# go-distributed/gossip_simulator

Hardware: AMD Instinct MI355X
Metric: gossip messages delivered/sec (node) at N=1e9; rounds-to-coverage parity (higher is better)
Workload: dtype u32

## Files before the change

gossip_simulator_amd/csrc/gs_ctx.cpp:

```cpp
#include "gs_ctx.h"

namespace gs {

namespace {

uint32_t ring_slots(const gs_params& p) { return p.delay_high > 2 ? (uint32_t)p.delay_high : 2u; }

uint32_t ceil_log2(uint64_t x) {
  uint32_t b = 0;
  while ((1ull << b) < x) ++b;
  return b;
}

int check_params(const gs_params* p, bool rumor_trials, bool median_trials, std::string& why) {
  if (!p) { why = "params is NULL"; return GS_EINVAL; }
  if (p->n == 0) { why = "n must be >= 1 (simulator.go:240 panics on rand.Intn(0))"; return GS_EINVAL; }
  if (p->n > 0x7FFFFFFFull) { why = "n must be < 2^31"; return GS_EINVAL; }
  if (p->delay_high <= p->delay_low) {
    why = "delayhigh must exceed delaylow (simulator.go:167 panics on rand.Intn(<=0))";
    return GS_EINVAL;
  }
  if (p->fanout < 0 || p->fanin < 0 || p->fanout > 255 || p->fanin > 255) {
    why = "fanout/fanin must be in [0, 255]";
    return GS_EINVAL;
  }
  if (ring_slots(*p) > 4096) { why = "delayhigh must be <= 4096"; return GS_EINVAL; }
  if (p->model > GS_MODEL_MEDIAN) {
    why = "model must be GS_MODEL_FLOOD, GS_MODEL_PUSHPULL, GS_MODEL_RUMOR or GS_MODEL_MEDIAN";
    return GS_EINVAL;
  }
  if (p->model == GS_MODEL_MEDIAN && (p->rumor_k < 1 || p->rumor_k > 127)) {
    why = "GS_MODEL_MEDIAN needs 1 <= rumor_k <= 127, not " + std::to_string(p->rumor_k);
    return GS_EINVAL;
  }
  if (p->model == GS_MODEL_MEDIAN && p->trials > 1 && !median_trials) {
    why = "GS_MODEL_MEDIAN with trials > 1: the median-counter model runs one trial per context";
    return GS_EINVAL;
  }
  if (p->model == GS_MODEL_RUMOR && (p->rumor_k < 1 || p->rumor_k > 255)) {
    why = "GS_MODEL_RUMOR needs 1 <= rumor_k <= 255, not " + std::to_string(p->rumor_k);
    return GS_EINVAL;
  }
  if (p->model == GS_MODEL_RUMOR && (p->rumor_mode & ~(GS_RUMOR_BLIND | GS_RUMOR_COIN | GS_RUMOR_PULL))) {
    why = "GS_MODEL_RUMOR: rumor_mode " + std::to_string(p->rumor_mode) +
          " has a bit that is none of GS_RUMOR_BLIND, GS_RUMOR_COIN, GS_RUMOR_PULL";
    return GS_EINVAL;
  }
  if (p->model == GS_MODEL_RUMOR && p->trials > 1 && !rumor_trials) {
    why = "GS_MODEL_RUMOR with trials > 1: the rumor model runs one trial per context (gs_create_trials makes a batch)";
    return GS_EINVAL;
  }
  if (p->trials > 1 && ((uint64_t)p->trials << std::max<uint32_t>(kFineLog, ceil_log2(p->n))) > 0x7FFFFFFFull) {
    why = "trials x 2^ceil(log2 n) must be < 2^31 (batch fewer trials per context)";
    return GS_EINVAL;
  }
  return GS_OK;
}

bool alloc_trial_rows(gs_ctx* c, size_t tb, size_t cb) {
  return dev_malloc((void**)&c->bt.d_tstat, tb) == hipSuccess &&
         hipHostMalloc((void**)&c->bt.h_tstat, tb) == hipSuccess && grow(c->bt.chk, cb);
}

void release_trials(gs_ctx* c) {
  if (c->bt.d_tstat) (void)dev_free(c->bt.d_tstat);
  if (c->bt.h_tstat) (void)hipHostFree(c->bt.h_tstat);
  release(c->bt.chk);
}

int alloc_window(gs_ctx* c) {
  const DevState& s = c->st;
  WinState& w = c->ws;
  w.n = s.n;
  w.W = s.W;
  w.nfine = (uint32_t)((s.n + kFineNodes - 1) >> kFineLog);
  w.ncoarse = (w.nfine + 255) / 256;
  w.R = s.R;
  w.delay_low = s.delay_low;
  w.delay_span = s.delay_span;
  w.kd = s.kd;
  w.kc = s.kc;
  w.key = s.key;
  w.base = (uint32_t)c->lo;
  w.tlog = c->tlog;
  w.tmask = c->tlog >= 32 ? ~0u : (1u << c->tlog) - 1;
  w.tnodes = c->trials > 1 && c->tlog <= kCoarseShift && !c->shard ? (uint32_t)c->p.n : 0u;
  w.G = c->G;
  w.rank = c->rank;
  w.seg_per = (uint32_t)c->seg_per;
  w.csub = kCoarseSub;
  w.noxcd = getenv("GS_PART2_NOXCD") ? 1u : 0u;
  {
    const char* xp = getenv("GS_XPAIR");
    w.nopair = xp && atoi(xp) == 0 ? 1u : 0u;
  }
  w.ccap_end = nullptr;
  w.csrc = nullptr;
  if (c->shard) {
    w.owner = 1;
    w.obins = 256 / c->G;
    w.oseg_q = (uint32_t)(c->seg_per >> kFineLog);
    w.oseg_magic = 0xFFFFFFFFu / w.oseg_q;
    if (dev_malloc(&c->wn.d_rtab, kRtabWords * 8) != hipSuccess ||
        hipHostMalloc((void**)&c->wn.h_rtab, kRtabWords * 8) != hipSuccess)
      return fail(c, GS_ENOMEM, "cannot allocate the shard's receive layout");
  }
  auto al = [](size_t b) { return (b + 255) & ~(size_t)255; };
  const size_t units = (size_t)kMaxWindow * w.nfine + 1;
  const size_t b_fc = al((size_t)w.R * w.nfine * 4), b_units = al(units * 8),
               b_small = al(kRegions * 8) * 2 + al((kRegions + 1) * 8) + al((kRegions + 1) * 4) + al(kMaxWindow * 8),
               b_fhist = al(((size_t)w.ncoarse * 256 + 1) * 8), b_fbase = al(((size_t)w.nfine + 1) * 8),
               b_ffill = al((size_t)w.nfine * 8),
               b_sst = al((size_t)kStatShards * kMaxWindow * kStatFields * 8),
               b_rlcnt = al((size_t)w.nfine * 4) + al(((size_t)w.nfine + 2) * 4),
               b_tsum = al((size_t)w.ncoarse * kMaxWindow * 8) + al(((size_t)w.ncoarse + 1) * 8);
  const size_t total = b_fc + 2 * b_units + b_small + b_fhist + b_fbase + b_ffill + b_sst + b_rlcnt + b_tsum;
  if (dev_malloc(&c->wn.d_win, total) != hipSuccess)
    return fail(c, GS_ENOMEM, "cannot allocate window-engine buffers");
  const size_t flist = (size_t)w.R * w.nfine * kFineNodes * 2;
  if (dev_malloc(&c->wn.d_flist, flist) != hipSuccess)
    return fail(c, GS_ENOMEM, "cannot allocate " + std::to_string(flist >> 20) + " MiB of fire lists");
  char* q = (char*)c->wn.d_win;
  w.fcount = (uint32_t*)q; q += b_fc;
  w.usize = (unsigned long long*)q; q += b_units;
  w.unit_off = (unsigned long long*)q; q += b_units;
  w.chist = (unsigned long long*)q; q += al(kRegions * 8);
  w.cfill = (unsigned long long*)q; q += al(kRegions * 8);
  w.ccap = (unsigned long long*)q; q += al((kRegions + 1) * 8);
  w.tprefix = (uint32_t*)q; q += al((kRegions + 1) * 4);
  w.tfires = (unsigned long long*)q;
  q = (char*)c->wn.d_win + b_fc + 2 * b_units + b_small;
  w.fhist = (unsigned long long*)q; q += b_fhist;
  w.fstart = (unsigned long long*)q; q += b_fbase;
  w.ffill = (unsigned long long*)q; q += b_ffill;
  w.sstats = (unsigned long long*)q; q += b_sst;
  w.rlcnt = (uint32_t*)q; q += al((size_t)w.nfine * 4);
  w.lgl = (uint32_t*)q; q += al(((size_t)w.nfine + 2) * 4);
  w.tsum = (unsigned long long*)q; q += al((size_t)w.ncoarse * kMaxWindow * 8);
  w.toff = (unsigned long long*)q; q += al(((size_t)w.ncoarse + 1) * 8);
  if (dev_malloc(&c->wn.d_rlmsg, (size_t)w.nfine * kRolledCap * 4) != hipSuccess)
    return fail(c, GS_ENOMEM, "cannot allocate the rolled-receipt lists");
  w.rlmsg = (uint32_t*)c->wn.d_rlmsg;
  w.dbg = nullptr;
  if (getenv("GS_STAMPS") && dev_malloc(&w.dbg, kDbgWords * 8) == hipSuccess)
    (void)hipMemset(w.dbg, 0, kDbgWords * 8);
  w.flist = (uint16_t*)c->wn.d_flist;
  c->wn.fcount_bytes = (size_t)w.R * w.nfine * 4;
  if (hipMemsetAsync(c->wn.d_win, 0, total, c->stream) != hipSuccess)
    return fail(c, GS_EDEVICE, "memset of window buffers failed");
  c->wn.misc_words = std::max<size_t>(4096, (size_t)c->G * kMaxWindow + 64);
  if (hipHostMalloc((void**)&c->wn.h_cap, (kRegions + 1) * 8) != hipSuccess ||
      hipHostMalloc((void**)&c->wn.h_misc, c->wn.misc_words * 8) != hipSuccess ||
      hipHostMalloc((void**)&c->wn.h_err, 64) != hipSuccess)
    return fail(c, GS_ENOMEM, "cannot allocate pinned window buffers");
  if (c->trials > 1) {
    if (!alloc_trial_rows(c, (size_t)c->trials * kMaxWindow * kTStatFields * 4, 0))
      return fail(c, GS_ENOMEM, "cannot allocate per-trial counters");
    w.tstat = c->bt.d_tstat;
  }
  return GS_OK;
}

void release_window(gs_ctx* c) {
  WinEngine& e = c->wn;
  for (void* p : {e.d_win, e.d_flist, e.d_rlmsg, (void*)e.d_rtab, (void*)c->ws.dbg})
    if (p) (void)dev_free(p);
  for (Buf* b : {&e.gmap, &e.cmsg, &e.fmsg, &e.tmp}) release(*b);
  for (void* p : {(void*)e.h_cap, (void*)e.h_misc, (void*)e.h_err, (void*)e.h_rtab})
    if (p) (void)hipHostFree(p);
}

int ctx_setup(gs_ctx* c, const gs_params* params, int device, bool shard, uint32_t G, uint32_t rank,
              std::string& why) {
  c->p = *params;
  c->p.device = device;
  c->dev = device;
  int ndev = 0;
  if (hipGetDeviceCount(&ndev) != hipSuccess || ndev <= 0) {
    why = "no HIP device visible (libgossip_hip needs an MI355X)";
    return GS_EDEVICE;
  }
  if (c->dev < 0 || c->dev >= ndev) {
    why = "device " + std::to_string(c->dev) + " out of range (" + std::to_string(ndev) + " visible)";
    return GS_EDEVICE;
  }
  hipDeviceProp_t prop;
  if (hipSetDevice(c->dev) != hipSuccess || hipGetDeviceProperties(&prop, c->dev) != hipSuccess ||
      strncmp(prop.gcnArchName, "gfx950", 6) != 0) {
    why = "device " + std::to_string(c->dev) + " is not gfx950";
    return GS_EDEVICE;
  }
  if (hipStreamCreateWithFlags(&c->own, hipStreamNonBlocking) != hipSuccess) {
    why = "cannot create a stream";
    return GS_EDEVICE;
  }
  c->stream = c->own;
  DevState& s = c->st;
  const uint32_t stride0 = (uint32_t)std::max(c->p.fanout, c->p.fanin);
  c->pp = c->p.model == GS_MODEL_PUSHPULL && !c->rset;
  c->rumor = c->p.model == GS_MODEL_RUMOR;
  c->median = c->p.model == GS_MODEL_MEDIAN;
  c->pp_l2_only = (c->p.flags & GS_FLAG_PP_L2_ONLY) != 0;
  c->trials = std::max<uint32_t>(1, c->p.trials);
  c->ntot = c->p.n;
  if (c->trials > 1) {
    c->tlog = std::max<uint32_t>(kFineLog, ceil_log2(c->p.n));
    c->ntot = (uint64_t)c->trials << c->tlog;
  }
  c->shard = shard;
  c->G = G;
  c->rank = rank;
  if (shard && c->rumor) {
    why = "GS_MODEL_RUMOR runs on one device: no node-range shards";
    return GS_EINVAL;
  }
  if (shard && c->median) {
    why = "GS_MODEL_MEDIAN runs on one device: no node-range shards";
    return GS_EINVAL;
  }
  if (shard) {
    if (c->pp && !pp_rslot_packed(stride0)) {
      why = "push-pull node-range shards need rows of at most 16 slots (bottom-up rounds)";
      return GS_EINVAL;
    }
    c->seg_per = (((c->p.n + G - 1) / G) + kFineNodes - 1) & ~(uint64_t)(kFineNodes - 1);
    if ((uint64_t)(G - 1) * c->seg_per >= c->p.n) {
      why = "n = " + std::to_string(c->p.n) + " is too small for " + std::to_string(G) +
            " shards of whole 16384-node buckets";
      return GS_EINVAL;
    }
    c->pp_shard = c->pp;
    c->rs.segw = c->seg_per / 64;
    c->lo = rank * c->seg_per;
    c->hi = std::min<uint64_t>(c->lo + c->seg_per, c->p.n);
    c->ntot = c->hi - c->lo;
  }
  s.lo = 0;
  s.hi = (uint32_t)c->ntot;
  s.n = c->ntot;
  s.W = (s.n + 63) / 64;
  s.C = (uint32_t)((s.n + (1ull << kChunkNodesLog) - 1) >> kChunkNodesLog);
  s.CS = (s.C + kShards - 1) / kShards;
  s.chunk_lo = 0;
  s.chunk_hi = s.C;
  s.sharded = 0;
  s.R = ring_slots(c->p);
  s.delay_low = c->p.delay_low;
  s.delay_span = (uint32_t)(c->p.delay_high - c->p.delay_low);
  s.kd = gs_threshold(c->p.drop_rate);
  s.kc = gs_threshold(c->p.crash_rate);
  s.key = Key{(uint32_t)c->p.seed, (uint32_t)(c->p.seed >> 32), c->p.trial};
  c->win = !c->pp && !c->rumor && !c->median && !c->rset && s.R <= kWinMaxRing && !(c->p.flags & GS_FLAG_TICK_ENGINE) && stride0 <= kWinMaxStride &&
           s.n <= (1ull << (kCoarseShift + 8));
  if (((c->trials > 1 && !c->ppt && !c->rmt && !c->mdt) || (shard && !c->pp)) && !c->win) {
    why = "batched trials and node-range shards run on the window engine (delayhigh <= 256, "
          "fanout/fanin <= 32, no GS_FLAG_TICK_ENGINE, at most 2^30 nodes per context or shard)";
    return GS_EINVAL;
  }
  static_assert(kSrcShift + 8 == 64, "8-bit source index in the receive layout");
  if (shard && !c->pp && (G > 255 || ((c->seg_per + (1ull << kCoarseShift) - 1) >> kCoarseShift) > 256 / G)) {
    why = "flood node-range shards: each of the G <= 255 shards' ranges must fit 256 / G bins of 2^22 nodes "
          "(n up to about 2^30)";
    return GS_EINVAL;
  }
  auto al = [](size_t b) { return (b + 255) & ~(size_t)255; };
  const bool tick = !c->win && !c->pp && !c->rumor && !c->median && !c->rset;
  const size_t b_sum = c->pp && !c->ppt ? al(pp_summary_total_words(s.W) * 8) : 0;
  const size_t b_next = (c->pp && !c->ppt) || (c->rumor && !c->rmt) ? al(s.W * 8) + b_sum : 0;
  const size_t b_bits = al(s.W * 8), b_ring = tick ? al((size_t)s.R * s.W * 8) : 0,
               b_cflag = tick ? al((size_t)s.R * s.C * 4) : 0,
               b_clist = tick ? al((size_t)s.R * kShards * s.CS * 4) : 0,
               b_ccount = tick ? al((size_t)s.R * kShards * kCounterStride * 4) : 0,
               b_stats = al((size_t)kStatSlots * kStatFields * 8);
  const size_t b_roll = c->win ? b_bits : 0;
  const size_t total = 2 * b_bits + b_roll + b_next + b_ring + b_cflag + b_clist + b_ccount + b_stats + 256;
  c->state_bytes = total;
  if (dev_malloc(&c->d_state, total) != hipSuccess) {
    why = "cannot allocate " + std::to_string(total) + " bytes of device state";
    return GS_ENOMEM;
  }
  char* q = (char*)c->d_state;
  s.recv = (unsigned long long*)q; q += b_bits;
  s.crash = (unsigned long long*)q; q += b_bits;
  s.rollw = b_roll ? (uint32_t*)q : nullptr; q += b_roll;
  c->d_next = b_next ? (unsigned long long*)q : nullptr;
  c->d_ppsum = b_sum ? (unsigned long long*)(q + al(s.W * 8)) : nullptr;
  q += b_next;
  s.ring = (unsigned long long*)q; q += b_ring;
  s.cflag = (uint32_t*)q; q += b_cflag;
  s.clist = (uint32_t*)q; q += b_clist;
  s.ccount = (uint32_t*)q; q += b_ccount;
  s.stats = (unsigned long long*)q; q += b_stats;
  c->d_err = (uint32_t*)q;
  c->d_flag = c->d_err + 1;
  s.err = c->d_err;
  s.grecv = s.recv;
  s.gcrash = s.crash;
  s.gbase = 0;
  if (tick && s.kc > 0 && dev_malloc(&c->d_cnt, s.n * 4) != hipSuccess) {
    why = "cannot allocate arrival counters";
// ... 430 lines not shown
```

gossip_simulator_amd/csrc/gs_internal.h:

```cpp
#pragma once
#include <stdint.h>
#include <hip/hip_runtime.h>

#include <algorithm>
#include <vector>

#include "gs_devmem.h"
#include "gs_rng.h"

namespace gs {

inline uint32_t grid_for(uint64_t items, uint32_t per_block, uint32_t cap) {
  return (uint32_t)std::min<uint64_t>((items + per_block - 1) / per_block, cap);
}

constexpr uint32_t kWave = 64;
constexpr uint32_t kChunkNodesLog = 12;
constexpr uint32_t kChunkWords = 64;
constexpr uint32_t kShards = 32;
constexpr uint32_t kCounterStride = 16;
constexpr uint32_t kStatFields = 8;
constexpr uint32_t kStatSlots = 4096;
constexpr uint32_t kListCap = 1024;
constexpr uint32_t kTickBlock = 256;
constexpr uint32_t kTickGridMax = 2048;

enum Stat : uint32_t {
  ST_FIRED = 0, ST_SENT = 1, ST_MSGS = 2, ST_RECV = 3, ST_CRASH = 4, ST_SCHED = 5,
  ST_ERR = 6, ST_RSVD = 7
};

enum Mode : int {
  MODE_FLOOD = 0,
  MODE_COUNT = 1,
  MODE_RESOLVE = 2
};

struct DevState {
  const uint8_t* deg;
  const uint32_t* ids;
  unsigned long long* recv;
  unsigned long long* crash;
  uint32_t* rollw;
  uint32_t* cnt;
  unsigned long long* ring;
  uint32_t* cflag;
  uint32_t* clist;
  uint32_t* ccount;
  unsigned long long* stats;
  uint32_t* err;
  unsigned long long* grecv;
  unsigned long long* gcrash;
  uint64_t gbase;
  uint64_t n, W;
  uint32_t C, CS, R, stride;
  uint32_t stride_magic;
  int32_t delay_low;
  uint32_t delay_span;
  int32_t kd, kc;
  int32_t check_crashed;
  int32_t sharded;
  uint32_t lo, hi;
  uint32_t chunk_lo, chunk_hi;
  Key key;
};

constexpr uint32_t kFineLog = 14;
constexpr uint32_t kFineNodes = 1u << kFineLog;
constexpr uint32_t kCoarseShift = kFineLog + 8;
constexpr uint32_t kMaxWindow = 16;
constexpr uint32_t kCoarseSub = 8;
constexpr uint32_t kRegions = 256 * kCoarseSub;
constexpr uint32_t kWinMaxRing = 256;
constexpr uint32_t kWinMaxStride = 32;
constexpr uint32_t kEmptyMsg = 0xFFFFFFFFu;
constexpr uint32_t kSrcShift = 56;
constexpr unsigned long long kSrcMask = (1ull << kSrcShift) - 1;
#ifndef GS_PART_TILE
#define GS_PART_TILE 16384
#endif
constexpr uint32_t kPartTile = GS_PART_TILE;
constexpr uint32_t kRolledCap = 1024;
constexpr uint32_t kBitTicks = 10;
constexpr uint32_t kXRoundNodes = 2048;
constexpr uint32_t kWinSlotsPerBucket = 1u << 16;

struct WinCtl {
  uint32_t t, L, tnext, tend;
  uint32_t poll, pbase, stop, lmax;
  unsigned long long Tn, T;
  unsigned long long recv, crashed, pending, cover, max_ticks;
  unsigned long long cmsg_cap, fmsg_cap;
  unsigned long long xs_cap, xr_cap;
};
constexpr uint32_t kStageWords = 8 + 16 * 8;

struct WinState {
  const uint8_t* deg;
  const uint32_t* ids;
  unsigned long long* recv;
  unsigned long long* crash;
  uint32_t* rollw;
  uint32_t* rlmsg;
  uint32_t* rlcnt;
  uint32_t* lgl;
  unsigned long long* stats;
  uint32_t* err;
  uint32_t* fcount;
  uint16_t* flist;
  unsigned long long* usize;
  unsigned long long* unit_off;
  unsigned long long* tfires;
  uint32_t* gmap;
  const uint32_t* pk;
  uint32_t noxcd;
  uint32_t nopair;
  uint32_t* cmsg;
  uint32_t* fmsg;
  unsigned long long* chist;
  unsigned long long* ccap;
  const unsigned long long* ccap_end;
  unsigned long long* cfill;
  uint32_t* tprefix;
  unsigned long long* fhist;
  unsigned long long* fstart;
  unsigned long long* ffill;
  unsigned long long* tsum;
  unsigned long long* toff;
  unsigned long long* sstats;
  unsigned long long* dbg;
  uint32_t* tstat;
  uint32_t tofs;
  WinCtl* ctl;
  unsigned long long* stage;
  uint32_t lstride;
  uint32_t slots;
  uint32_t csub;
  const uint32_t* const* csrc;
  uint32_t owner;
  uint32_t obins;
  uint32_t oseg_q, oseg_magic;
  uint32_t abort_on_err;
  uint32_t G, rank;
  uint32_t seg_per;
  uint32_t dd;
  uint32_t guard;
  uint32_t solo;
  unsigned long long* gcnt;
  unsigned long long* glay;
  unsigned long long* wstat;
  uint64_t nglob;
  uint64_t n, W;
  uint32_t nfine, ncoarse, R, stride, stride_magic;
  int32_t delay_low;
  uint32_t delay_span;
  int32_t kd, kc;
  uint32_t base;
  uint32_t tlog, tmask;
  uint32_t tnodes;
  Key key;
};
constexpr uint32_t kStatShards = 32;
constexpr uint32_t kStampPhases = 10;
constexpr uint32_t kXStamp0 = 2 * kStampPhases;
constexpr uint32_t kDbgWords = kXStamp0 + 8;
enum TStat : uint32_t { TS_FIRED = 0, TS_SENT = 1, TS_DEAD = 2, TS_RECV = 3, TS_CRASH = 4, TS_HOT = 5, TS_MSGS = 6 };
constexpr uint32_t kTStatFields = 8;

__host__ __device__ __forceinline__ void node_key(uint32_t tlog, uint32_t tmask, const Key& key,
                                                  uint64_t g, uint32_t kind, uint32_t& node,
                                                  uint32_t& c3) {
  node = (uint32_t)(g & tmask);
  c3 = ctr3(kind, key.trial + (uint32_t)(g >> tlog));
}

constexpr uint32_t kErrArrivals = 4;
constexpr uint32_t kErrCoarse = 8;
constexpr uint32_t kErrFine = 16;
constexpr uint32_t kErrAbort = 32;
constexpr uint32_t kErrNoMem = 64;
constexpr uint32_t kDDRow = kRegions + 4;
constexpr uint32_t kDDWStat = kMaxWindow * kStatFields + 8;
constexpr size_t kRtabWords = 4 * (kRegions + 1) + 260;
constexpr size_t kRtabTotal = kRtabWords - 1;

hipError_t win_units(const WinState& w, uint32_t t0, uint32_t L, hipStream_t s);
hipError_t win_cut(const WinState& w, unsigned long long budget, hipStream_t s);
hipError_t win_unitscan(const WinState& w, hipStream_t s);
hipError_t win_close(const WinState& w, uint32_t slot, hipStream_t s);
hipError_t win_scan_units(const WinState& w, uint32_t L, void* tmp, size_t& tmp_bytes, hipStream_t s);
hipError_t win_groupmap(const WinState& w, uint32_t L, hipStream_t s);
hipError_t win_expand(const WinState& w, uint32_t t0, uint32_t L, uint64_t Tn, int mode,
                      hipStream_t s);
uint32_t win_expand_geometry(const WinState& w, uint64_t Tn, uint32_t* per_round, uint32_t* bsz,
                             uint32_t* npt);
hipError_t win_plan(const WinState& w, bool exact, hipStream_t s);
hipError_t win_scan_fine(const WinState& w, void* tmp, size_t& tmp_bytes, hipStream_t s);
hipError_t win_part2(const WinState& w, uint64_t T, bool scatter, hipStream_t s);
hipError_t win_resolve(const WinState& w, uint32_t t0, uint32_t L, hipStream_t s);
hipError_t win_pack_rows(const uint32_t* ids, uint64_t n, uint32_t* pk, hipStream_t s);
hipError_t win_seal_rows(const uint8_t* deg, uint32_t* ids, uint64_t n, uint32_t stride,
                         hipStream_t s);
hipError_t win_stats_reduce(const WinState& w, uint32_t t0, uint32_t L, hipStream_t s);
hipError_t win_consume_sh(const WinState& w, uint32_t t0, uint32_t L, hipStream_t s);
hipError_t win_rtab(const WinState& w, unsigned long long* rtab, const unsigned long long* const* ccaps,
                    const uint32_t* const* src, uint32_t nsrc, uint32_t travels, hipStream_t s);
hipError_t win_fine_redo(const WinState& w, uint64_t T, hipStream_t s);
hipError_t win_stats_dd(const WinState& w, uint32_t slot, hipStream_t s);
struct WinGroup {
  const WinState* ws;
  const WinState* wr;
  const WinState* wg;
  uint32_t M;
  uint32_t nfine_max;
  uint32_t ncoarse_max;
  uint32_t slots_max;
};
hipError_t win_units_g(const WinGroup& g, uint32_t L, hipStream_t s);
hipError_t win_cut_g(const WinGroup& g, unsigned long long budget, hipStream_t s);
hipError_t win_unitscan_g(const WinGroup& g, hipStream_t s);
hipError_t win_rtab_g(const WinGroup& g, const unsigned long long* const* ccaps, const uint32_t* const* src,
                      uint32_t nsrc, hipStream_t s);
hipError_t win_recv_g(const WinGroup& g, uint64_t T, hipStream_t s);
hipError_t win_stats_dd_g(const WinGroup& g, uint32_t slot, hipStream_t s);
hipError_t win_expand_g(const WinGroup& g, uint32_t L, hipStream_t s);
hipError_t win_resolve_g(const WinGroup& g, uint32_t L, hipStream_t s);
hipError_t win_close_dd(const WinState& w, const unsigned long long* const* wstats, WinCtl* const* ctls,
                        uint32_t n, uint32_t slot, hipStream_t s);
hipError_t win_pack(const WinState& w, const unsigned long long* poff, uint32_t nreg, uint32_t* out, hipStream_t s);
hipError_t win_schedule(const WinState& w, uint32_t node, uint32_t tick, uint32_t trials, uint32_t n,
                        hipStream_t s, uint32_t* started = nullptr);

inline uint64_t pp_summary_words(uint64_t W) { return (W + 63) / 64; }
inline uint64_t pp_summary2_words(uint64_t W) { return (pp_summary_words(W) + 63) / 64; }
inline uint64_t pp_summary_total_words(uint64_t W) { return 2 * pp_summary_words(W) + 2 * pp_summary2_words(W); }
enum PPMode : uint32_t { PP_DENSE = 0, PP_EARLY = 1, PP_BOTTOM = 2, PP_ANSWER = 3 };
__host__ __device__ inline bool pp_rslot_packed(uint32_t stride) { return stride <= 16; }
constexpr uint32_t kPPSegs = 256;
struct PPCtl {
  unsigned long long ninf;
  unsigned long long thr;
  unsigned long long bthr;
  unsigned long long athr;
  unsigned long long ncallers;
  unsigned long long nlive0;
  unsigned long long seg_cap;
  uint32_t nseg;
  uint32_t mode;
  uint32_t early_ok;
  uint32_t ovf;
  uint32_t nearly, nbottom;
  uint32_t nanswer, pad_;
  unsigned long long segcnt[kPPSegs];
  unsigned long long seglen[kPPSegs];
  unsigned long long segpre[kPPSegs + 1];
};
struct PPSparse {
  PPCtl* ctl;
  uint32_t* ilist;
  const unsigned long long* rend;
  const uint16_t* rend16;
  const unsigned long long* rbase;
  const uint32_t* rsrc;
  const uint8_t* rslot;
  const uint8_t* fmask;
  const unsigned long long* fany;
  const uint32_t* rfail;
  uint32_t* dset;
  unsigned long long* dcnt;
  uint64_t dcap, ccap, fcap;
  uint32_t nodeg;
  uint32_t pullfirst;
  uint32_t word_maxi;
  uint32_t word_maxu;
  uint32_t words;
};
constexpr uint32_t kPPDLists = 512;
constexpr uint32_t kPPDRegions = 2048;
hipError_t pp_round(const DevState& s, unsigned long long* next, unsigned long long* sum, uint32_t t,
                    bool l2_only, const PPSparse& sp, hipStream_t st);
hipError_t pp_live_edges(const DevState& s, uint32_t* out, hipStream_t st);
hipError_t pp_commit(const DevState& s, const unsigned long long* next, uint32_t t, const PPSparse& sp,
                     hipStream_t st);
hipError_t pp_seed(const DevState& s, unsigned long long* next, uint32_t node, uint32_t* flag,
                   const PPSparse& sp, unsigned long long thr, unsigned long long bthr, unsigned long long athr,
                   const unsigned long long* callers, hipStream_t st);
size_t pp_rev_scan_bytes(uint64_t n);
hipError_t pp_rev_build(const DevState& s, unsigned long long* rend, uint32_t* rsrc, uint8_t* rslot, void* tmp,
                        size_t tmp_bytes, hipStream_t st);
hipError_t pp_rev_compact(const unsigned long long* rend, uint64_t n, uint16_t* rend16, unsigned long long* rbase,
                          uint32_t* ovf, hipStream_t st);
hipError_t pp_rev_build_part(const DevState& s, unsigned long long* rend, uint32_t* rsrc, uint8_t* rslot,
                             hipStream_t st, uint32_t* passes_out);
hipError_t pp_fmask_build(const DevState& s, const unsigned long long* rend, const uint32_t* rsrc,
                          const uint8_t* rslot, uint8_t* fmask, hipStream_t st);
size_t pp_rev_range_scan_bytes(uint64_t n);
hipError_t pp_rev_count_range(const uint8_t* deg, const uint32_t* ids, uint64_t nfull, uint32_t stride, uint64_t lo,
                              uint64_t hi, unsigned long long* rend, void* tmp, size_t tmp_bytes, hipStream_t st);
hipError_t pp_rev_fill_range(const uint8_t* deg, const uint32_t* ids, uint64_t nfull, uint32_t stride, uint64_t lo,
                             uint64_t hi, unsigned long long* rend, uint32_t* rsrc, uint8_t* rslot, hipStream_t st);
hipError_t pp_fmask_rows(const DevState& s, uint8_t* fmask, hipStream_t st);
hipError_t pp_fmask_any(const uint8_t* fmask, uint64_t n, unsigned long long* fany, hipStream_t st);
hipError_t pp_rfail_build(const DevState& s, const unsigned long long* rend, const uint32_t* rsrc,
                          const uint8_t* rslot, uint32_t* rfail, hipStream_t st);
hipError_t pp_round_shard(const DevState& s, unsigned long long* next, unsigned long long* gnext, uint32_t t,
                          const PPSparse& sp, uint32_t mode, hipStream_t st);
hipError_t pp_count(const unsigned long long* words, uint64_t nwords, unsigned long long* out, hipStream_t st);
hipError_t pp_or_slices(unsigned long long* dst, const unsigned long long* src, uint32_t nslices, uint64_t words,
                        hipStream_t st);

struct PptState {
  const uint8_t* deg;
  const uint32_t* ids;
  unsigned long long* recv;
  const unsigned long long* crash;
  uint32_t* tstat;
  uint32_t n, trials, tlog, stride;
  uint32_t block, lds_bytes;
  uint32_t lds_masked;
  int32_t kd;
  Key key;
};
hipError_t ppt_lds_limit(int device, bool masked, uint64_t* limit, const char** where = nullptr);
hipError_t ppt_prepare(int device, bool masked, uint32_t lds_bytes);
hipError_t ppt_seed(const PptState& s, uint32_t node, uint32_t* started, hipStream_t st);
hipError_t ppt_rounds(const PptState& s, uint32_t t0, uint32_t rounds, hipStream_t st);
hipError_t ppt_stalled(const PptState& s, const uint8_t* need, uint32_t* live, hipStream_t st);

enum RumorAcc : uint32_t { RA_FIRED = 0, RA_SENT = 1, RA_MSGS = 2, RA_NEW = 3 };
constexpr uint32_t kRumorCovered = 1, kRumorQuiescent = 2;
constexpr uint32_t kRumorBlind = 1, kRumorCoin = 2, kRumorPull = 4;
struct RumorCtl {
  unsigned long long wlen;
  unsigned long long pad0_[31];
  unsigned long long acc[4];
  unsigned long long pad1_[28];
  unsigned long long rlen;
  unsigned long long received;
  unsigned long long cover;
  unsigned long long peak;
  uint32_t stop, pad2_;
  unsigned long long pad3_[27];
};
static_assert(sizeof(RumorCtl) == 3 * 256, "RumorCtl: three 256-byte blocks");
struct RumorState {
  RumorCtl* ctl;
  unsigned long long* next;
  uint8_t* miss;
  uint32_t k;
  uint32_t mode;
  unsigned long long* hot;
  unsigned long long* served;
  unsigned long long* vain;
};
uint32_t rumor_grid(uint64_t n, uint32_t want);
hipError_t rumor_seed(const DevState& s, const RumorState& r, uint32_t* list0, uint32_t node, unsigned long long cover,
                      hipStream_t st);
hipError_t rumor_round(const DevState& s, const RumorState& r, const uint32_t* rlist, uint32_t* wlist, uint32_t t,
                       uint32_t grid, hipStream_t st);
hipError_t rumor_commit(const DevState& s, const RumorState& r, uint32_t t, hipStream_t st);
hipError_t rumor_removed(const RumorState& r, const uint32_t* rlist, unsigned long long* out, uint32_t grid,
                         hipStream_t st);
hipError_t rumor_pull_seed(const DevState& s, const RumorState& r, uint32_t node, unsigned long long cover,
                           hipStream_t st);
hipError_t rumor_pull_round(const DevState& s, const RumorState& r, uint32_t t, uint32_t grid, hipStream_t st);
hipError_t rumor_pull_commit(const DevState& s, const RumorState& r, uint32_t t, hipStream_t st);
hipError_t rumor_pull_removed(const DevState& s, const RumorState& r, unsigned long long* out, hipStream_t st);

struct RmtState {
// ... 69 lines not shown
```

gossip_simulator_amd/csrc/gs_shards.cpp:

```cpp
#include "gs_ctx.h"

namespace gs {

namespace {

int sync_all(const std::vector<gs_ctx*>& ms) {
  for (gs_ctx* m : ms) {
    CK(m, hipSetDevice(m->dev));
    CK(m, hipStreamSynchronize(m->stream));
  }
  return GS_OK;
}

int mark_nomem(gs_ctx* m, const std::string& what) {
  uint32_t e = 0;
  CK(m, hipMemcpyAsync(&e, m->d_err, 4, hipMemcpyDeviceToHost, m->stream));
  CK(m, hipStreamSynchronize(m->stream));
  e |= kErrNoMem;
  CK(m, hipMemcpyAsync(m->d_err, &e, 4, hipMemcpyHostToDevice, m->stream));
  CK(m, hipStreamSynchronize(m->stream));
  m->err = what;
  return GS_OK;
}

// ... 575 lines not shown
  CK(c, hipMemcpyAsync(dbuf, c->xc.h_xbuf, count * 8, hipMemcpyHostToDevice, c->stream));
  CK(c, hipStreamSynchronize(c->stream));
  return GS_OK;
}

int rank_sum(gs_ctx* c, unsigned long long* v) {
  unsigned long long* d = c->xc.d_gcounts;
  CK(c, hipMemcpyAsync(d, v, 8, hipMemcpyHostToDevice, c->stream));
  if (int rc = x_all_reduce(c, d, 1)) return abort_rank(c, rc);
  CK(c, hipMemcpyAsync(v, d, 8, hipMemcpyDeviceToHost, c->stream));
  CK(c, hipStreamSynchronize(c->stream));
  return GS_OK;
}

int abort_rank(gs_ctx* c, int rc) {
  if (rc && is_rank(c)) c->aborted = true;
  if (rc && c->xc.comm && rccl().ok && rccl().comm_abort) {
    (void)rccl().comm_abort(c->xc.comm);
    c->xc.comm = nullptr;
  }
  return rc;
}

bool dd_ok(const gs_ctx* acc, const std::vector<gs_ctx*>& ms) {
  if ((acc->p.flags & GS_FLAG_TIMING) || getenv("GS_SYNC_WINDOWS") || shard_serial()) return false;
  const gs_ctx* m0 = ms[0];
  if (m0->pp || !m0->win || !m0->shard) return false;
  if (acc->group) return !acc->gtrials && acc->gr.devs.size() == 1;
  return is_rank(acc);
}

int dd_run(gs_ctx* acc, const std::vector<gs_ctx*>& ms, uint64_t tend, uint32_t poll, uint64_t max_ticks,
           const OnTick& on_tick, uint32_t* stop, bool* fallback) {
  *stop = 0;
  *fallback = false;
  RC(dd_setup(acc, ms));
  gs_ctx* m0 = ms[0];
  const uint32_t G = m0->G, M = (uint32_t)ms.size();
  const bool rank = is_rank(m0), travel = rank && G > 1;
  const bool solo = !rank && G == 1 && M == 1;
  const size_t K1 = kRegions + 1;
  hipStream_t st = m0->stream;
  CK(acc, hipSetDevice(m0->dev));
  for (gs_ctx* m : ms)
    if (m != m0) CK(acc, hipStreamSynchronize(m->stream));
  const uint32_t Lmax = std::min<uint32_t>(std::max<int32_t>(m0->p.delay_low, 1), kBitTicks);
  const uint64_t N = m0->p.n;
  const unsigned long long budget = ((N + kFineNodes - 1) >> kFineLog) * (unsigned long long)kWinSlotsPerBucket;
  const uint32_t B8 = m0->ws.obins * kCoarseSub, nreg = G * B8;
  bool ok = true;
  for (gs_ctx* m : ms)
    ok = ok && grow(m->wn.gmap, ((m->ntot + 1 + 63) / 64 + 1) * 4) && grow(m->wn.cmsg, 64) && grow(m->wn.fmsg, 64);
  if (rank) RC(agree_ok(m0, ok, "cannot allocate the window message buffers"));
  else if (!ok) return fail(acc, GS_ENOMEM, "cannot allocate the window message buffers");
  void** hp = acc->dd.h_ptrs;
  const uint32_t nsrc = rank ? 2u : M + 1;
  void** d_ccaps = acc->dd.ptrs;
  void** d_src = acc->dd.ptrs + M;
  void** d_wst = acc->dd.ptrs + 2 * M + 1;
  void** d_ctls = acc->dd.ptrs + 3 * M + 1;
  for (uint32_t i = 0; i < M; ++i) {
    hp[i] = ms[i]->ws.ccap;
    hp[2 * M + 1 + i] = acc->dd.wstat + (size_t)i * kDDWStat;
    hp[3 * M + 1 + i] = acc->dd.ctl + i;
  }
  if (rank) {
    hp[M] = m0->xc.xrecv.p;
    hp[M + 1] = m0->wn.cmsg.p;
  } else {
    for (uint32_t i = 0; i < M; ++i) hp[M + i] = ms[i]->wn.cmsg.p;
    hp[2 * M] = nullptr;
  }
  CK(acc, hipMemcpyAsync(acc->dd.ptrs, hp, (size_t)(4 * M + 2) * sizeof(void*), hipMemcpyHostToDevice, st));
  std::vector<WinCtl> hc(M);
  for (uint32_t i = 0; i < M; ++i) {
    WinCtl& h = hc[i];
    h = WinCtl{};
    h.tnext = (uint32_t)(acc->t + 1);
    h.tend = (uint32_t)std::min<uint64_t>(tend, 0xFFFFFFFFull);
    h.poll = poll;
    h.pbase = (uint32_t)acc->t;
    h.lmax = Lmax;
    h.recv = acc->recv;
    h.crashed = acc->crashed;
    h.pending = acc->pending;
    h.cover = cover_threshold(N);
    h.max_ticks = max_ticks;
    h.cmsg_cap = buf_cap(ms[i]->wn.cmsg);
    h.fmsg_cap = buf_cap(ms[i]->wn.fmsg);
    h.xs_cap = buf_cap(ms[i]->xc.xsend);
    h.xr_cap = buf_cap(ms[i]->xc.xrecv);
  }
  CK(acc, hipMemcpyAsync(acc->dd.ctl, hc.data(), (size_t)M * sizeof(WinCtl), hipMemcpyHostToDevice, st));
  CK(acc, hipMemsetAsync(acc->dd.gcnt, 0, (size_t)G * kMaxWindow * 8, st));
  std::vector<WinState> ws(M), wr(M);
  std::vector<uint64_t> tn_bound(M);
  for (uint32_t i = 0; i < M; ++i) {
    gs_ctx* m = ms[i];
    WinState w = m->ws;
    w.ctl = acc->dd.ctl + i;
    w.stage = acc->aw.d_stage;
    w.lstride = Lmax;
    w.dd = 1;
    w.guard = 0;
    w.abort_on_err = 0;
    w.gcnt = acc->dd.gcnt;
    w.glay = acc->dd.glay;
    w.tfires = acc->dd.gcnt + (size_t)m->rank * kMaxWindow;
    w.cfill = acc->dd.glay + (size_t)m->rank * kDDRow;
    w.wstat = acc->dd.wstat + (size_t)i * kDDWStat;
    w.nglob = N;
    w.solo = solo ? 1u : 0u;
    w.gmap = (uint32_t*)m->wn.gmap.p;
    w.cmsg = (uint32_t*)m->wn.cmsg.p;
    w.fmsg = (uint32_t*)m->wn.fmsg.p;
    ws[i] = w;
    if (solo) {
      wr[i] = w;
      tn_bound[i] = std::min<uint64_t>(m->ntot + 1, 4096ull * 1024);
      continue;
    }
    WinState r = w;
    r.cmsg = nullptr;
    r.csrc = (const uint32_t* const*)(m->wn.d_rtab + 4 * K1);
    r.ccap = m->wn.d_rtab;
    r.ccap_end = m->wn.d_rtab + K1;
    r.cfill = m->wn.d_rtab + 2 * K1;
    r.csub = G * kCoarseSub;
    wr[i] = r;
    tn_bound[i] = std::min<uint64_t>(m->ntot + 1, 4096ull * 1024);
  }
  const uint64_t T_bound = 2048ull * 16384;
  static const bool group_env = [] { const char* e = getenv("GS_DD_GROUP"); return !(e && atoi(e) == 0); }();
  const bool grouped = !rank && M > 1 && group_env;
  std::vector<WinState> wall;
  WinGroup grp{};
  if (grouped) {
    wall.reserve(3 * M);
    wall.insert(wall.end(), ws.begin(), ws.end());
    wall.insert(wall.end(), wr.begin(), wr.end());
    for (uint32_t i = 0; i < M; ++i) {
      wall.push_back(wr[i]);
      wall.back().guard = 1;
    }
    CK(acc, hipMemcpyAsync(acc->dd.wsm, wall.data(), wall.size() * sizeof(WinState), hipMemcpyHostToDevice, st));
    grp.ws = acc->dd.wsm;
    grp.wr = acc->dd.wsm + M;
    grp.wg = acc->dd.wsm + 2 * M;
    grp.M = M;
    for (uint32_t i = 0; i < M; ++i) {
      grp.nfine_max = std::max(grp.nfine_max, ws[i].nfine);
      grp.ncoarse_max = std::max(grp.ncoarse_max, ws[i].ncoarse);
      grp.slots_max = std::max(grp.slots_max, ws[i].slots);
    }
  }
  auto bsize = [&](uint32_t s, uint32_t d) {
    unsigned long long a = 0;
    for (uint32_t r = d * B8; r < (d + 1) * B8; ++r) a += acc->dd.h_lay[(size_t)s * kDDRow + r];
    return a;
  };
  auto enqueue = [&](uint32_t slot, bool* aborted) -> int {
    *aborted = false;
    if (grouped) {
      CK(acc, win_units_g(grp, Lmax, st));
      CK(acc, win_cut_g(grp, budget, st));
      CK(acc, win_unitscan_g(grp, st));
    } else {
      for (uint32_t i = 0; i < M; ++i) CK(acc, win_units(ws[i], 0, Lmax, st));
      if (rank) RC(x_all_gather(m0, acc->dd.gcnt, kMaxWindow * 8));
      for (uint32_t i = 0; i < M; ++i) CK(acc, win_cut(ws[i], budget, st));
      for (uint32_t i = 0; i < M; ++i) CK(acc, win_unitscan(ws[i], st));
    }
    if (grouped) CK(acc, win_expand_g(grp, Lmax, st));
    for (uint32_t i = 0; i < M && !grouped; ++i) CK(acc, win_expand(ws[i], 0, Lmax, tn_bound[i], 1, st));
    if (rank) RC(x_all_gather(m0, acc->dd.glay, kDDRow * 8));
    if (grouped)
      CK(acc, win_rtab_g(grp, (const unsigned long long* const*)d_ccaps, (const uint32_t* const*)d_src, nsrc, st));
    for (uint32_t i = 0; i < M && !solo && !grouped; ++i)
      CK(acc, win_rtab(ws[i], ms[i]->wn.d_rtab, (const unsigned long long* const*)d_ccaps, (const uint32_t* const*)d_src,
                       nsrc, rank ? 1u : 0u, st));
    if (travel) {
      gs_ctx* m = m0;
      const uint32_t me = m->rank;
      CK(acc, hipMemcpyAsync(acc->dd.h_lay, acc->dd.glay, (size_t)G * kDDRow * 8, hipMemcpyDeviceToHost, st));
      CK(acc, hipMemcpyAsync(m->wn.h_err, m->d_err, 4, hipMemcpyDeviceToHost, st));
      CK(acc, hipMemcpyAsync(m->wn.h_misc, acc->dd.ctl, 32, hipMemcpyDeviceToHost, st));
      CK(acc, hipStreamSynchronize(st));
      const uint32_t* hc0 = (const uint32_t*)m->wn.h_misc;
      if (*m->wn.h_err & kErrAbort) { *aborted = true; return 1; }
      if (hc0[1] == 0 || hc0[6]) return 1;
      std::vector<unsigned long long> ptot(G, 0), rsum(G, 0);
      for (uint32_t s = 0; s < G; ++s)
        for (uint32_t d = 0; d < G; ++d)
          if (s != d) {
            const unsigned long long b = bsize(s, d);
            ptot[s] += b;
            rsum[d] += b;
          }
      bool any_grow = false;
      for (uint32_t s = 0; s < G; ++s) {
        const unsigned long long* row = acc->dd.h_lay + (size_t)s * kDDRow;
        if (ptot[s] > row[kRegions + 2] || rsum[s] > row[kRegions + 3]) any_grow = true;
      }
      if (any_grow) {
        const void* old_recv = m->xc.xrecv.p;
        const bool ok = grow(m->xc.xsend, (ptot[me] + 16) * 4) && grow(m->xc.xrecv, (rsum[me] + 16) * 4);
        unsigned long long* d = m->xc.d_gcounts + (size_t)G * kMaxWindow;
        m->wn.h_misc[8] = ok ? 0ull : 1ull;
        CK(acc, hipMemcpyAsync(d, &m->wn.h_misc[8], 8, hipMemcpyHostToDevice, st));
        RC(x_all_reduce(m, d, 1));
        CK(acc, hipMemcpyAsync(&m->wn.h_misc[9], d, 8, hipMemcpyDeviceToHost, st));
        CK(acc, hipStreamSynchronize(st));
        if (m->wn.h_misc[9]) return fail(acc, GS_ENOMEM, "a rank cannot allocate its exchange buffers");
        WinCtl* c = acc->dd.ctl;
        m->wn.h_misc[10] = buf_cap(m->xc.xsend);
        m->wn.h_misc[11] = buf_cap(m->xc.xrecv);
        CK(acc, hipMemcpyAsync(&c->xs_cap, &m->wn.h_misc[10], 16, hipMemcpyHostToDevice, st));
        if (m->xc.xrecv.p != old_recv) {
          m->wn.h_misc[12] = (unsigned long long)(uintptr_t)m->xc.xrecv.p;
          CK(acc, hipMemcpyAsync(m->wn.d_rtab + 4 * K1, &m->wn.h_misc[12], 8, hipMemcpyHostToDevice, st));
          hp[M] = m->xc.xrecv.p;
          CK(acc, hipMemcpyAsync(&d_src[0], &hp[M], sizeof(void*), hipMemcpyHostToDevice, st));
        }
        CK(acc, hipStreamSynchronize(st));
      }
      CK(acc, win_pack(ws[0], m->wn.d_rtab + 3 * K1, nreg, (uint32_t*)m->xc.xsend.p, st));
      auto bstart = [&](uint32_t s, uint32_t d) {
        unsigned long long a = 0;
        for (uint32_t d2 = 0; d2 < d; ++d2)
          if (d2 != s) a += bsize(s, d2);
        return a;
      };
      std::vector<unsigned long long> in(G, 0);
      unsigned long long rs = 0;
      for (uint32_t s = 0; s < G; ++s)
        if (s != me) { in[s] = rs; rs += bsize(s, me); }
      uint32_t* xs = (uint32_t*)m->xc.xsend.p;
      uint32_t* xr = (uint32_t*)m->xc.xrecv.p;
      if (m->xc.comm) {
        const Rccl& r = rccl();
        NCK(acc, r.group_start());
        for (uint32_t p = 0; p < G; ++p) {
          if (p == me) continue;
          if (bsize(me, p)) NCK(acc, r.send(xs + bstart(me, p), bsize(me, p), ncclUint32, (int)p, m->xc.comm, st));
          if (bsize(p, me)) NCK(acc, r.recv(xr + in[p], bsize(p, me), ncclUint32, (int)p, m->xc.comm, st));
        }
        NCK(acc, r.group_end());
      } else {
        std::vector<size_t> sb(G, 0), rb(G, 0);
        for (uint32_t p = 0; p < G; ++p)
          if (p != me) { sb[p] = bsize(me, p) * 4; rb[p] = bsize(p, me) * 4; }
        RC(agree_ok(m, grow_pinned(m, (ptot[me] + rs) * 4 + 16), "cannot allocate exchange staging"));
        char* hs = m->xc.h_xbuf;
        char* hr = m->xc.h_xbuf + ptot[me] * 4;
        CK(acc, hipMemcpyAsync(hs, xs, ptot[me] * 4, hipMemcpyDeviceToHost, st));
        CK(acc, hipStreamSynchronize(st));
        if (m->xc.hx.all_to_allv(m->xc.hx.user, hs, sb.data(), hr, rb.data()))
          return fail(acc, GS_EDEVICE, "the exchange's all_to_allv callback failed");
        CK(acc, hipMemcpyAsync(xr, hr, rs * 4, hipMemcpyHostToDevice, st));
        CK(acc, hipStreamSynchronize(st));
      }
    }
    if (grouped) {
      CK(acc, win_recv_g(grp, T_bound, st));
      CK(acc, win_resolve_g(grp, Lmax, st));
      CK(acc, win_stats_dd_g(grp, slot, st));
    } else {
      for (uint32_t i = 0; i < M; ++i) {
        CK(acc, win_plan(wr[i], false, st));
        CK(acc, win_part2(wr[i], T_bound, true, st));
        if (!solo) CK(acc, win_fine_redo(wr[i], T_bound, st));
        CK(acc, win_resolve(wr[i], 0, Lmax, st));
        CK(acc, win_stats_dd(ws[i], slot, st));
      }
    }
    if (rank) RC(x_all_reduce(m0, acc->dd.wstat, kDDWStat));
    if (!solo)
      CK(acc, win_close_dd(ws[0], (const unsigned long long* const*)d_wst, (WinCtl* const*)d_ctls, M, slot, st));
    CK(acc, hipEventRecord(acc->aw.wev[slot], st));
    return 0;
  };
  bool eoverflow = false;
  auto absorb = [&](uint32_t slot, int* what) -> int {
    CK(acc, hipEventSynchronize(acc->aw.wev[slot]));
    const unsigned long long* sg = acc->aw.h_stage + (size_t)slot * kStageWords;
    const uint32_t t0 = (uint32_t)sg[0], L = (uint32_t)sg[1];
    *what = 0;
    if (sg[3] & kErrAbort) {
      if (dd_log()) fprintf(stderr, "[dd] window at t0=%u aborted: redone host-driven\n", t0);
      ++m0->timing.dd_fallbacks;
      *fallback = true;
      *what = 1;
      return GS_OK;
    }
    if (dd_log()) fprintf(stderr, "[dd] t0=%u L=%u stop=%llu redos=%llu\n", t0, L, sg[2], sg[4]);
    m0->timing.exact_redos += sg[4];
    for (uint32_t k = 0; k < L; ++k) on_tick((uint64_t)t0 + k, sg + 8 + (size_t)k * kStatFields);
    if (sg[3] & kErrArrivals) eoverflow = true;
    if (sg[2]) *stop = (uint32_t)sg[2];
    if (sg[2] || L == 0 || (uint64_t)t0 + L >= tend || eoverflow) *what = 1;
    return GS_OK;
  };
  bool ab = false;
  int e0 = 0;
  RC((e0 = enqueue(0, &ab), e0 < 0 ? e0 : 0));
  if (e0 == 1) {
// ... 79 lines not shown
```

gossip_simulator_amd/csrc/gs_win_dev.h:

```cpp
#pragma once
#include <cstdlib>

#include "gossip.h"
#include "gs_internal.h"
#include "gs_wave.h"

namespace gs {
namespace {

constexpr uint32_t kExpandBlock = 256;
constexpr uint32_t kExpandBlock6 = 512;
constexpr uint32_t kExpandNpt = 4;
constexpr uint32_t kResolveBlock = 512;
#ifndef GS_RESOLVE_WAVES
#define GS_RESOLVE_WAVES 4
#endif
constexpr uint32_t kRoll0Coarse = kCoarseShift + 4;
constexpr uint32_t kRoll0Fine = kFineLog + 4;

inline uint32_t device_cus() {
  static const uint32_t cus = [] {
    int dev = 0, v = 0;
    if (hipGetDevice(&dev) == hipSuccess &&
        hipDeviceGetAttribute(&v, hipDeviceAttributeMultiprocessorCount, dev) == hipSuccess && v > 0)
      return (uint32_t)v;
    return 256u;
  }();
  return cus;
}

__device__ __forceinline__ uint32_t stop_bits(const WinState& w) {
  return w.dd && !w.solo ? kErrAbort : (kErrCoarse | kErrFine | kErrAbort);
}
__device__ __forceinline__ bool win_abort(const WinState& w) {
  return (*w.err & stop_bits(w)) != 0;
}
struct CtlView {
  uint32_t t, L, tnext, tend, poll, pbase, stop, lmax, err;
};
__device__ __forceinline__ CtlView ctl_view(const WinState& w) {
  static_assert(offsetof(WinCtl, t) == 0 && offsetof(WinCtl, lmax) == 28, "WinCtl's first 32 bytes");
  const uint4* p = reinterpret_cast<const uint4*>(w.ctl);
  const uint4 a = p[0], b = p[1];
  const uint32_t e = *w.err;
  return CtlView{a.x, a.y, a.z, a.w, b.x, b.y, b.z, b.w, e};
}
__device__ __forceinline__ uint32_t win_open(const WinState& w, uint32_t& t) {
  const CtlView c = ctl_view(w);
  t = c.tnext;
  const bool dead = (c.err & stop_bits(w)) || c.stop || t >= c.tend;
  uint32_t Lw = min(c.lmax, c.tend - t);
  if (c.poll) {
    const uint32_t P = c.pbase + c.poll * ((t - c.pbase + c.poll - 1) / c.poll);
    Lw = min(Lw, P - t + 1);
  }
  return dead ? 0u : Lw;
}
__device__ __forceinline__ uint32_t win_live(const WinState& w, uint32_t& t0, uint32_t L) {
  if (!w.ctl) return w.abort_on_err && win_abort(w) ? 0u : L;
  const CtlView c = ctl_view(w);
  t0 = c.t;
  const bool off = (c.err & stop_bits(w)) || (w.guard && !(c.err & kErrFine));
  return off ? 0u : c.L;
}

__device__ __forceinline__ unsigned long long* shard_row(const WinState& w, uint32_t k) {
  return w.sstats + ((size_t)(blockIdx.x & (kStatShards - 1)) * kMaxWindow + k) * kStatFields;
}

constexpr uint32_t kCloseLanes = 8;
__device__ __forceinline__ unsigned long long stat_shard_sum(const WinState& w, uint32_t i, uint32_t part) {
  constexpr uint32_t kPer = kStatShards / kCloseLanes;
  unsigned long long x[kPer], sum = 0;
#pragma unroll
  for (uint32_t j = 0; j < kPer; ++j) x[j] = w.sstats[(size_t)(j * kCloseLanes + part) * kMaxWindow * kStatFields + i];
#pragma unroll
  for (uint32_t j = 0; j < kPer; ++j) {
    sum += x[j];
    if (x[j]) w.sstats[(size_t)(j * kCloseLanes + part) * kMaxWindow * kStatFields + i] = 0;
  }
#pragma unroll
  for (uint32_t o = 1; o < kCloseLanes; o <<= 1) sum += __shfl_xor(sum, o, 64);
  return sum;
}

__device__ __forceinline__ void block_scan256(uint32_t* cnt, uint32_t* off) {
  if (threadIdx.x < 64) {
    const uint32_t l = threadIdx.x;
    const uint32_t a = cnt[4 * l], b = cnt[4 * l + 1], c = cnt[4 * l + 2], d = cnt[4 * l + 3];
    const uint32_t sum = a + b + c + d;
    const uint32_t x = wave_inscan(sum);
    const uint32_t ex = x - sum;
    off[4 * l] = ex;
    off[4 * l + 1] = ex + a;
    off[4 * l + 2] = ex + a + b;
    off[4 * l + 3] = ex + a + b + c;
    if (l == 63) off[256] = x;
  }
}

__device__ __forceinline__ unsigned long long region_end(const WinState& w, uint32_t r) {
  return w.ccap_end ? w.ccap_end[r] : w.ccap[r + 1];
}
__device__ __forceinline__ unsigned long long region_fill(const WinState& w, uint32_t r) {
  const unsigned long long room = region_end(w, r) - w.ccap[r];
  return w.cfill[r] < room ? w.cfill[r] : room;
}

__device__ __forceinline__ bool tiles_by_xcd(const WinState& w) {
  return w.csub == kCoarseSub && !w.csrc && !w.noxcd;
}
__device__ __forceinline__ uint32_t xcd_bin_pos(uint32_t c) { return (c & 7) * 32 + (c >> 3); }
__device__ __forceinline__ uint32_t xcd_bin_of(uint32_t pc) { return (pc & 31) * 8 + (pc >> 5); }

__device__ __forceinline__ uint32_t msg_loc(uint32_t m) { return m & (kFineNodes - 1); }
__device__ __forceinline__ uint32_t msg_tick(uint32_t m) { return (m >> kFineLog) & (kMaxWindow - 1); }

}
}
```

gossip_simulator_amd/csrc/gs_win_expand.hip:

```cpp
#include <algorithm>

#include "gs_win_dev.h"

namespace gs {
namespace {

__device__ __forceinline__ uint32_t unit_of_wave(const WinState& w, unsigned long long g0, unsigned long long g,
                                                 unsigned long long Tn, uint32_t units) {
  const unsigned long long q = g0 >> 6;
  uint32_t lo = w.gmap[q];
  uint32_t hi = ((q + 1) << 6) < Tn ? w.gmap[q + 1] : units - 1;
  if (lo == hi) return lo;
  while (lo < hi) {
    const uint32_t mid = (lo + hi + 1) >> 1;
    if (w.unit_off[mid] <= g) lo = mid; else hi = mid - 1;
  }
  return lo;
}

#ifdef GS_XSTAMPS
__device__ __forceinline__ void xstamp(const WinState& w, unsigned long long& last, uint32_t i) {
  if (w.dbg && threadIdx.x < 64) {
    __builtin_amdgcn_s_waitcnt(0);
    const unsigned long long t = __builtin_amdgcn_s_memtime();
// ... 18 lines not shown
  uint32_t ovf;
  unsigned long long acc[kMaxWindow][2];
};

__device__ __forceinline__ void tstat_add(uint32_t* tstat, uint32_t key, uint32_t fa, uint32_t a,
                                          uint32_t fb, uint32_t b) {
  bool pend = key != ~0u;
  for (unsigned long long bal = __ballot(pend); bal; bal = __ballot(pend)) {
    const uint32_t lead = (uint32_t)__builtin_ctzll(bal);
    const uint32_t k0 = __shfl(key, lead, 64);
    const bool mine = pend && key == k0;
    const uint32_t sa = wave_sum(mine ? a : 0u), sb = wave_sum(mine ? b : 0u);
    if ((threadIdx.x & 63) == lead) {
      if (sa) atomicAdd(&tstat[(size_t)k0 * kTStatFields + fa], sa);
      if (sb) atomicAdd(&tstat[(size_t)k0 * kTStatFields + fb], sb);
    }
    pend = pend && !mine;
  }
}

__device__ __forceinline__ uint64_t pk_byte(uint32_t v) {
  const uint32_t line = (uint32_t)(((uint64_t)v * 0xCCCCCCCDull) >> 34);
  return (uint64_t)line * 128 + (v - line * 5) * 24;
}

__device__ __forceinline__ uint32_t dpp_swap_pair(uint32_t v) {
  return (uint32_t)__builtin_amdgcn_mov_dpp((int)v, 0xB1, 0xF, 0xF, false);
}
template <uint32_t MAXS>
__device__ __forceinline__ void decode_pk_row(uint4 x, uint4 y, bool o8, uint32_t (&mm)[MAXS]) {
  mm[0] = o8 ? x.z : x.x;
  mm[1] = o8 ? x.w : x.y;
  mm[2] = o8 ? y.x : x.z;
  mm[3] = o8 ? y.y : x.w;
  mm[4 % MAXS] = o8 ? y.z : y.x;
  if (MAXS > 5) mm[5 % MAXS] = o8 ? y.w : y.y;
}
template <uint32_t MAXS, uint32_t NPT>
__device__ __forceinline__ void load_rows_pk_pairs(const WinState& w, const uint32_t (&vv)[NPT], const bool (&wlive)[NPT],
                                                   uint32_t (&mm)[NPT][MAXS]) {
  const uint32_t odd = threadIdx.x & 1;
  const uint4* pk = reinterpret_cast<const uint4*>(w.pk);
  uint4 s0[NPT], s1[NPT];
  uint32_t o8[NPT];
#pragma unroll
  for (uint32_t q = 0; q < NPT; ++q) {
    if (!wlive[q]) continue;
    const uint64_t b = vv[q] != ~0u ? pk_byte(vv[q]) : 0ull;
    o8[q] = (uint32_t)b & 8u;
    const uint32_t mine = (uint32_t)(b >> 4), other = dpp_swap_pair(mine);
    const uint32_t ev = odd ? other : mine, od = odd ? mine : other;
    s0[q] = pk[(size_t)ev + odd];
    s1[q] = pk[(size_t)od + odd];
  }
#pragma unroll
  for (uint32_t q = 0; q < NPT; ++q) {
    if (!wlive[q]) continue;
    const uint4 send = odd ? s0[q] : s1[q];
    uint4 got;
    got.x = dpp_swap_pair(send.x);
    got.y = dpp_swap_pair(send.y);
    got.z = dpp_swap_pair(send.z);
    got.w = dpp_swap_pair(send.w);
    if (vv[q] != ~0u) decode_pk_row<MAXS>(odd ? got : s0[q], odd ? s1[q] : got, o8[q] != 0, mm[q]);
  }
}

template <uint32_t MAXS>
__device__ __forceinline__ void load_row(const WinState& w, uint32_t v, uint32_t (&mm)[MAXS]) {
  const uint32_t S = w.stride;
  if (MAXS >= 5 && MAXS <= 6 && w.pk) {
    const uint64_t b = pk_byte(v);
    const uint4* p = reinterpret_cast<const uint4*>(reinterpret_cast<const char*>(w.pk) + (b & ~15ull));
    decode_pk_row<MAXS>(p[0], p[1], (b & 8) != 0, mm);
    return;
  }
  if ((S & 3) == 0 && S >= 8 && MAXS >= 5 && MAXS <= 8) {
    const uint4 a = reinterpret_cast<const uint4*>(w.ids + (size_t)v * S)[0];
    mm[0] = a.x; mm[1] = a.y; mm[2] = a.z; mm[3] = a.w;
    if (MAXS > 4 && MAXS <= 6) {
      const uint2 b = reinterpret_cast<const uint2*>(w.ids + (size_t)v * S)[2];
      mm[4 % MAXS] = b.x;
      if (MAXS > 5) mm[5 % MAXS] = b.y;
    } else if (MAXS > 6) {
      const uint4 b = reinterpret_cast<const uint4*>(w.ids + (size_t)v * S)[1];
      mm[4 % MAXS] = b.x; mm[5 % MAXS] = b.y; mm[6 % MAXS] = b.z; mm[7 % MAXS] = b.w;
    }
  } else if ((S & 3) == 0 && MAXS > 8) {
    const uint4* row = reinterpret_cast<const uint4*>(w.ids + (size_t)v * S);
#pragma unroll
    for (uint32_t j = 0; j < MAXS; j += 4) {
      const uint4 x = j < S ? row[j / 4] : make_uint4(kEmptyMsg, kEmptyMsg, kEmptyMsg, kEmptyMsg);
      mm[j] = x.x;
      if (j + 1 < MAXS) mm[j + 1] = x.y;
      if (j + 2 < MAXS) mm[j + 2] = x.z;
      if (j + 3 < MAXS) mm[j + 3] = x.w;
    }
  } else if ((S & 1) == 0) {
    const uint2* row = reinterpret_cast<const uint2*>(w.ids + (size_t)v * S);
#pragma unroll
    for (uint32_t j = 0; j < MAXS; j += 2) {
      const uint2 x = 2 * j < 2 * S ? row[j / 2] : make_uint2(kEmptyMsg, kEmptyMsg);
      mm[j] = x.x;
      if (j + 1 < MAXS) mm[j + 1] = x.y;
    }
  } else {
    const uint32_t* row = w.ids + (size_t)v * S;
#pragma unroll
    for (uint32_t j = 0; j < MAXS; ++j) mm[j] = j < S ? row[j] : kEmptyMsg;
  }
}

__device__ __forceinline__ uint32_t coarse_bin(const WinState& w, uint32_t& t) {
  if (!w.owner) {
    const uint32_t b = t >> kCoarseShift;
    t &= (1u << kCoarseShift) - 1;
    return b;
  }
  const uint32_t q = t >> kFineLog;
  uint32_t d = __umulhi(q, w.oseg_magic);
  if ((d + 1) * w.oseg_q <= q) ++d;
  const uint32_t off = t - d * w.seg_per;
  t = off & ((1u << kCoarseShift) - 1);
  return d * w.obins + (off >> kCoarseShift);
}

__device__ __forceinline__ void xcd_rounds(unsigned long long rounds, unsigned long long& beg,
                                           unsigned long long& end, unsigned long long& step) {
  const uint32_t B = gridDim.x;
  if ((B & 7) == 0) {
    const unsigned long long per = (rounds + 7) >> 3, x = blockIdx.x & 7;
    beg = x * per + (blockIdx.x >> 3);
    end = (x + 1) * per < rounds ? (x + 1) * per : rounds;
    step = B >> 3;
  } else {
    beg = blockIdx.x;
    end = rounds;
    step = B;
  }
}

template <bool WRITE, uint32_t MAXS, uint32_t NPT, uint32_t B>
__device__ __forceinline__ void expand_body(const WinState& w, uint32_t t0, uint32_t L, unsigned long long Tn,
                                            int add_stats) {
  __shared__ ExpandLds<B * NPT * MAXS> sm;
  const uint32_t tid = threadIdx.x;
  uint32_t Ls = L;
  if (w.ctl) {
    L = win_live(w, t0, 0);
    if (!L) return;
    Tn = w.ctl->Tn;
    Ls = w.lstride;
  }
  const uint32_t units = Ls * w.nfine;
  constexpr uint32_t per_round = B * NPT;
  if (tid < kMaxWindow * 2) (&sm.acc[0][0])[tid] = 0;
  static_assert(B % 256 == 0, "thread b < 256 owns coarse bin b");
  const bool binner = tid < 256;
  const uint32_t reg = (tid & 255) * kCoarseSub + (blockIdx.x & (kCoarseSub - 1));
  const unsigned long long cbase = w.ccap[reg], cend = w.ccap[reg + 1];
  if (binner) sm.cend[tid] = cend;
  const unsigned long long rounds = (Tn + per_round - 1) / per_round;
  unsigned long long rbeg, rend, rstep;
  xcd_rounds(rounds, rbeg, rend, rstep);
  uint32_t accp[kBitTicks];
#pragma unroll
  for (uint32_t kx = 0; kx < kBitTicks; ++kx) accp[kx] = 0;
#ifdef GS_XSTAMPS
  unsigned long long xlast = 0;
  XSTAMP(0);
#endif
  for (unsigned long long rd = rbeg; rd < rend; rd += rstep) {
    if (binner) sm.cnt[tid] = 0;
    __syncthreads();
    if (tid == 0) sm.ovf = 0;
    XSTAMP(6);
    uint32_t mm[NPT][MAXS], mt[NPT][MAXS];
    uint32_t vv[NPT], kk[NPT];
    bool wlive[NPT];
#pragma unroll
    for (uint32_t q = 0; q < NPT; ++q) {
      const unsigned long long g0 = rd * per_round + q * B + __builtin_amdgcn_readfirstlane(tid & ~63u);
      const unsigned long long g = g0 + (tid & 63);
      vv[q] = ~0u;
      kk[q] = 0;
      wlive[q] = g0 < Tn;
      if (g0 < Tn) {
        const uint32_t u = unit_of_wave(w, g0, g < Tn ? g : Tn - 1, Tn, units);
        if (g < Tn) {
        const uint32_t f = u / Ls, k = u - f * Ls;
        const uint32_t s = (t0 + k) % w.R;
        const uint32_t i = (uint32_t)(g - w.unit_off[u]);
        vv[q] = (f << kFineLog) + w.flist[((size_t)s * w.nfine + f) * kFineNodes + i];
        kk[q] = k;
        }
      }
    }
    XSTAMP(1);
#pragma unroll
    for (uint32_t q = 0; q < NPT; ++q) {
#pragma unroll
      for (uint32_t j = 0; j < MAXS; ++j) { mm[q][j] = kEmptyMsg; mt[q][j] = ~0u; }
    }
    if (MAXS >= 5 && MAXS <= 6 && w.pk && !w.nopair) {
      load_rows_pk_pairs<MAXS, NPT>(w, vv, wlive, mm);
    } else {
#pragma unroll
      for (uint32_t q = 0; q < NPT; ++q)
        if (vv[q] != ~0u) load_row<MAXS>(w, vv[q], mm[q]);
    }
    XSTAMP(2);
    uint32_t sentq[NPT];
#pragma unroll
    for (uint32_t q = 0; q < NPT; ++q) {
      sentq[q] = 0;
      if (vv[q] == ~0u) continue;
      const uint32_t v = vv[q], k = kk[q], t = t0 + k;
      uint32_t vn, c3drop;
      node_key(w.tlog, w.tmask, w.key, (uint64_t)w.base + v, K_DROP, vn, c3drop);
      uint32_t sent = 0;
#pragma unroll
      for (uint32_t jg = 0; jg < (MAXS + 3) / 4; ++jg) {
        if (mm[q][jg * 4] == kEmptyMsg) break;
        const u32x4 r = philox(vn, t, jg, c3drop, w.key.k0, w.key.k1);
#pragma unroll
        for (uint32_t jj = 0; jj < 4; ++jj) {
          const uint32_t j = jg * 4 + jj;
          if (j >= MAXS) break;
          uint32_t dropd, crashd;
          drop_crash(lane_of(r, jj), dropd, crashd);
          if (mm[q][j] != kEmptyMsg && (int32_t)dropd >= w.kd) {
            uint32_t loc = mm[q][j];
            const uint32_t bin = coarse_bin(w, loc);
            const uint32_t roll0 = (int32_t)crashd < w.kc;
            mt[q][j] = bin | (atomicAdd(&sm.cnt[bin], 1u) << 8);
            mm[q][j] = loc | (k << kCoarseShift) | (roll0 << kRoll0Coarse);
            ++sent;
          }
        }
      }
      sentq[q] = sent;
#pragma unroll
      for (uint32_t kx = 0; kx < kBitTicks; ++kx)
        if (kx == k) accp[kx] += 1u | (sent << 16);
    }
    if (WRITE && add_stats && w.tstat) {
#pragma unroll
      for (uint32_t q = 0; q < NPT; ++q) {
        const uint32_t key = vv[q] == ~0u ? ~0u : (uint32_t)((uint64_t)vv[q] >> w.tlog) * kMaxWindow + w.tofs + kk[q];
        tstat_add(w.tstat, key, TS_FIRED, 1u, TS_SENT, sentq[q]);
      }
    }
    XSTAMP(3);
    __syncthreads();
    if (!WRITE) {
      if (binner && sm.cnt[tid]) atomicAdd(&w.chist[reg], (unsigned long long)sm.cnt[tid]);
      continue;
    }
    block_scan256(sm.cnt, sm.off);
    const uint32_t mycnt = binner ? sm.cnt[tid] : 0u;
    unsigned long long at = 0;
    if (mycnt) at = atomicAdd(&w.cfill[reg], (unsigned long long)mycnt);
    __syncthreads();
#pragma unroll
    for (uint32_t q = 0; q < NPT; ++q)
#pragma unroll
      for (uint32_t j = 0; j < MAXS; ++j)
        if (mt[q][j] != ~0u) {
          const uint32_t bin = mt[q][j] & 255, p = sm.off[bin] + (mt[q][j] >> 8);
          sm.sorted[p] = mm[q][j];
          sm.sbin[p] = (uint8_t)bin;
        }
    if (mycnt) {
      if (at + mycnt > cend - cbase) {
        atomicOr(w.err, kErrCoarse);
        if (w.dd) atomicOr(reinterpret_cast<unsigned int*>(&w.cfill[kRegions]), kErrCoarse);
        sm.ovf = 1;
      }
      sm.gbase[tid] = cbase + at - sm.off[tid];
    }
    XSTAMP(4);
    __syncthreads();
    XSTAMP(5);
    const uint32_t total = sm.off[256];
    if (!sm.ovf) {
      for (uint32_t p = tid; p < total; p += B) w.cmsg[sm.gbase[sm.sbin[p]] + p] = sm.sorted[p];
    } else {
      for (uint32_t p = tid; p < total; p += B) {
        const uint32_t b = sm.sbin[p];
        const unsigned long long pos = sm.gbase[b] + p;
        if (pos < sm.cend[b]) w.cmsg[pos] = sm.sorted[p];
      }
    }
  }
  if (!WRITE || !add_stats) return;
#pragma unroll
  for (uint32_t kx = 0; kx < kBitTicks; ++kx) {
    if (kx >= L) continue;
    const uint32_t fired = wave_sum(accp[kx] & 0xFFFFu), sent = wave_sum(accp[kx] >> 16);
    if ((tid & 63) == 0) {
      if (fired) atomicAdd(&sm.acc[kx][0], (unsigned long long)fired);
      if (sent) atomicAdd(&sm.acc[kx][1], (unsigned long long)sent);
    }
  }
  __syncthreads();
  if (tid < L * 2) {
    const uint32_t k = tid >> 1, fld = tid & 1;
    const unsigned long long v = sm.acc[k][fld];
    unsigned long long* row = shard_row(w, k);
    if (v) atomicAdd(&row[fld ? ST_SENT : ST_FIRED], v);
    if (v && fld) atomicAdd(&row[ST_MSGS], v);
  }
}
template <bool WRITE, uint32_t MAXS, uint32_t NPT, uint32_t B = kExpandBlock>
__global__ __launch_bounds__(B) void k_expand(const WinState w, uint32_t t0, uint32_t L, unsigned long long Tn,
                                              int add_stats) {
  expand_body<WRITE, MAXS, NPT, B>(w, t0, L, Tn, add_stats);
}
template <bool WRITE, uint32_t MAXS, uint32_t NPT, uint32_t B = kExpandBlock>
__global__ __launch_bounds__(B) void k_expand_m(const WinState* __restrict__ ws, uint32_t L, int add_stats) {
  expand_body<WRITE, MAXS, NPT, B>(ws[blockIdx.y], 0u, L, 0ull, add_stats);
}

__global__ void k_pack_rows(const uint32_t* ids, uint64_t n, uint32_t* pk) {
  for (uint64_t v = (uint64_t)blockIdx.x * blockDim.x + threadIdx.x; v < n;
       v += (uint64_t)gridDim.x * blockDim.x) {
    const uint4 a = reinterpret_cast<const uint4*>(ids + v * 8)[0];
    const uint2 b = reinterpret_cast<const uint2*>(ids + v * 8)[2];
    uint2* d = reinterpret_cast<uint2*>(reinterpret_cast<char*>(pk) + pk_byte((uint32_t)v));
    d[0] = make_uint2(a.x, a.y);
    d[1] = make_uint2(a.z, a.w);
    d[2] = b;
  }
}

__global__ void k_seal_rows(const uint8_t* deg, uint32_t* ids, uint64_t n, uint32_t stride) {
  for (uint64_t v = (uint64_t)blockIdx.x * blockDim.x + threadIdx.x; v < n;
       v += (uint64_t)gridDim.x * blockDim.x) {
    const uint32_t d = deg[v];
    for (uint32_t j = d; j < stride; ++j) ids[v * stride + j] = kEmptyMsg;
  }
}

}

uint32_t win_expand_geometry(const WinState& w, uint64_t Tn, uint32_t* per_round_out, uint32_t* bsz_out,
// ... 71 lines not shown
```

gossip_simulator_amd/csrc/gs_win_resolve.hip:

```cpp
#include <algorithm>

#include "gs_win_dev.h"

namespace gs {
namespace {

constexpr uint32_t kResolveMaxBuckets = 256;
constexpr uint32_t kSmallMax = 256;
#ifndef GS_SMALL_BLOCK
#define GS_SMALL_BLOCK 512
#endif
constexpr uint32_t kSmallBlock = GS_SMALL_BLOCK;
#ifndef GS_ROLLED_BLOCK
#define GS_ROLLED_BLOCK 256
#endif
constexpr uint32_t kRolledBlock = GS_ROLLED_BLOCK;

constexpr uint32_t kBitWords = kFineNodes / 32;
struct ResolveLds {
  union {
    struct {
      uint32_t b1[kBitTicks][kBitWords];
      uint2 cr0[kBitWords];
    };
    struct {
      uint32_t cnt[kFineNodes];
      uint32_t recv[kBitWords];
      uint32_t crash[kBitWords];
      uint32_t nrecv[kBitWords];
      uint32_t ncrash[kBitWords];
    };
  };
  uint32_t fc[kWinMaxRing];
  uint32_t st[kMaxWindow][4];
  uint32_t dead[kMaxWindow];
  uint32_t blist[kResolveMaxBuckets];
  unsigned long long bstart[kResolveMaxBuckets];
  uint32_t bcnt[kResolveMaxBuckets];
  uint32_t ndup;
  uint32_t ninf;
  uint32_t err;
  uint32_t nb;
  uint32_t cls;
  unsigned long long stamp[2][kStampPhases];
  unsigned long long tlast;
};
static_assert(kBitTicks <= kMaxWindow, "window ticks fit the message format");
static_assert(sizeof(uint32_t) * kFineNodes <= sizeof(((ResolveLds*)0)->cnt), "the infection list fits");

template <class Lds>
__device__ __forceinline__ void stamp(const WinState& w, Lds& sm, uint32_t i) {
  if (w.dbg && threadIdx.x == 0) {
    const unsigned long long t = __builtin_amdgcn_s_memtime();
    if (i) sm.stamp[sm.cls][i] += t - sm.tlast;
    sm.tlast = t;
  }
}

#if defined(GS_RESOLVE_PROBE) && GS_RESOLVE_PROBE == 1
#define GS_RESOLVE_CR0(loc) make_uint2(0u, 0u)
#else
#define GS_RESOLVE_CR0(loc) sm.cr0[(loc) >> 5]
#endif


__device__ __forceinline__ void resolve_node(const WinState& w, ResolveLds& sm, uint32_t f,
                                             uint32_t loc, uint32_t kk, uint32_t ones, uint32_t t,
                                             uint32_t& cm, uint32_t& cr, uint32_t& cc, uint32_t& cs) {
  const uint32_t bit = 1u << (loc & 31), wi = loc >> 5;
  if (sm.crash[wi] & bit) return;
  const uint64_t g = (uint64_t)w.base + (f << kFineLog) + loc;
  uint32_t u, c3order;
  node_key(w.tlog, w.tmask, w.key, g, K_ORDER, u, c3order);
  const uint32_t pos = ones ? first_crash(u, t, kk, ones, c3order, w.key.k0, w.key.k1) : kk + 1;
  cm += pos <= kk ? pos : kk;
  if (pos > 1 && !(sm.recv[wi] & bit)) {
    atomicOr(&sm.recv[wi], bit);
    ++cr;
    uint32_t c3delay;
    node_key(w.tlog, w.tmask, w.key, g, K_DELAY, u, c3delay);
    const uint32_t off = fire_offset(w.delay_low, w.delay_span,
                                     philox(u, t, 0, c3delay, w.key.k0, w.key.k1).x);
    const uint32_t s = (t + off) % w.R;
    const uint32_t at = atomicAdd(&sm.fc[s], 1u);
    w.flist[((size_t)s * w.nfine + f) * kFineNodes + at] = (uint16_t)loc;
    ++cs;
  }
  if (pos <= kk) {
    atomicOr(&sm.crash[wi], bit);
    ++cc;
  }
}

template <class Src>
__device__ __forceinline__ void resolve_tick(const WinState& w, ResolveLds& sm, uint32_t f,
                                             const Src& src, uint32_t lo, uint32_t hi, uint32_t k,
                                             uint32_t t) {
  const uint32_t tid = threadIdx.x;
  for (uint32_t p = lo + tid; p < hi; p += kResolveBlock) {
    const uint32_t m = src[p];
    if (msg_tick(m) != k) continue;
    const uint32_t old = atomicAdd(&sm.cnt[msg_loc(m)], 1u + (((m >> kRoll0Fine) & 1u) << 16));
    if ((old & 0xFFFFu) == 0xFFFFu) sm.err = 1;
  }
  __syncthreads();
  uint32_t arr = 0, cm = 0, cr = 0, cc = 0, cs = 0;
  for (uint32_t p = lo + tid; p < hi; p += kResolveBlock) {
    const uint32_t m = src[p];
    if (msg_tick(m) != k) continue;
    const uint32_t loc = msg_loc(m);
    const uint32_t kk = atomicExch(&sm.cnt[loc], 0u);
    arr += kk & 0xFFFFu;
    if (kk) resolve_node(w, sm, f, loc, kk & 0xFFFFu, kk >> 16, t, cm, cr, cc, cs);
  }
  if (arr != cm) atomicAdd(&sm.st[k][0], arr - cm);
  if (cr) atomicAdd(&sm.st[k][1], cr);
  if (cc) atomicAdd(&sm.st[k][2], cc);
  (void)cs;
  __syncthreads();
}

template <class Lds>
__device__ __forceinline__ void flush_counts(const WinState& w, Lds& sm, uint32_t (&acc_ni)[kBitTicks / 2],
                                             uint32_t L, uint32_t trial) {
#pragma unroll
  for (uint32_t k = 0; k < kBitTicks; ++k) {
    if (k >= L) continue;
    const uint32_t sr = wave_sum((acc_ni[k / 2] >> (16 * (k & 1))) & 0xFFFFu);
    if (lane_id() == 0 && sr) atomicAdd(&sm.st[k][1], sr);
  }
#pragma unroll
  for (uint32_t k = 0; k < kBitTicks / 2; ++k) acc_ni[k] = 0;
  __syncthreads();
  const uint32_t tid = threadIdx.x;
  if (tid < L * 3) {
    const uint32_t k = tid / 3, fld = tid - k * 3;
    const uint32_t v = sm.st[k][fld];
    unsigned long long* row = shard_row(w, k);
    if (v && fld == 0) atomicAdd(&row[ST_MSGS], 0ull - (unsigned long long)v);
    if (v && fld == 1) {
      atomicAdd(&row[ST_RECV], (unsigned long long)v);
      atomicAdd(&row[ST_SCHED], (unsigned long long)v);
    }
    if (v && fld == 2) atomicAdd(&row[ST_CRASH], (unsigned long long)v);
    if (v && trial != ~0u) atomicAdd(&w.tstat[((size_t)trial * kMaxWindow + w.tofs + k) * kTStatFields + TS_DEAD + fld], v);
    sm.st[k][fld] = 0;
  }
  __syncthreads();
}

__device__ __forceinline__ void resolve_body(const WinState& w, uint32_t t0, uint32_t L) {
  __shared__ ResolveLds sm;
  const uint32_t tid = threadIdx.x, G = gridDim.x;
  L = win_live(w, t0, L);
  if (!L) return;
  static_assert(kBitWords == kResolveBlock, "one bit word per thread");
  static_assert(kWinMaxRing <= kResolveBlock, "one ring slot per thread");
  if (tid < kMaxWindow * 4) (&sm.st[0][0])[tid] = 0;
  if (tid == 0) { sm.nb = 0; sm.cls = 0; }
  if (tid < 2 * kStampPhases) (&sm.stamp[0][0])[tid] = 0;
  __syncthreads();
  {
    const uint32_t f = blockIdx.x + tid * G;
    const unsigned long long fl = tid < kResolveMaxBuckets && f < w.nfine ? w.ffill[f] : 0ull;
    const bool ne = fl > kSmallMax;
    const uint32_t at = wave_append(&sm.nb, ne);
    if (ne) {
      sm.blist[at] = f;
      sm.bstart[at] = w.fstart[f];
      sm.bcnt[at] = (uint32_t)fl;
    }
  }
  __syncthreads();
  const uint32_t nb = sm.nb;
  stamp(w, sm, 0);
  uint32_t fB = 0, MB = 0;
  unsigned long long mbB = 0;
  auto next_bucket = [&](uint32_t j) { fB = sm.blist[j]; mbB = sm.bstart[j]; MB = sm.bcnt[j]; };
  if (nb > 0) next_bucket(0);
  uint32_t* rwg = (uint32_t*)w.recv;
  uint32_t* cwg = (uint32_t*)w.crash;
  uint32_t acc_ni[kBitTicks / 2];
#pragma unroll
  for (uint32_t k = 0; k < kBitTicks / 2; ++k) acc_ni[k] = 0;
  static_assert(kBitTicks % 2 == 0 && 32 * kResolveMaxBuckets < 65536, "two 16-bit counts per register");
  constexpr uint32_t kU = 8;
  constexpr uint32_t kBatch = kResolveBlock * kU;
  auto ld = [&](const uint32_t* gm, uint32_t M, uint32_t p0, uint32_t (&m)[kU]) {
#pragma unroll
    for (uint32_t u = 0; u < kU; ++u) {
      const uint32_t p = p0 + u * kResolveBlock + tid;
      m[u] = *reinterpret_cast<const uint32_t*>(reinterpret_cast<const char*>(gm) + ((p < M ? p : M - 1) << 2));
    }
  };
  uint32_t pm[kU], p_recv0 = 0, p_crash0 = 0, p_roll0 = 0, p_fcv = 0;
  bool p_in = false;
  auto prefetch = [&](uint32_t f, uint32_t M, unsigned long long mb) {
    const uint64_t wi = ((uint64_t)(f << kFineLog) >> 5) + tid;
    const bool in = wi < w.W * 2;
    const uint64_t wc = in ? wi : w.W * 2 - 1;
    p_in = in;
    p_recv0 = rwg[wc];
    p_crash0 = cwg[wc];
    p_roll0 = w.rollw[wc];
    p_fcv = w.fcount[(size_t)(tid < w.R ? tid : 0u) * w.nfine + f];
    ld(w.fmsg + mb, M, 0, pm);
  };
  if (nb > 0) prefetch(fB, MB, mbB);
  for (uint32_t i = 0; i < nb; ++i) {
    const uint32_t f = fB, M = MB;
    const unsigned long long mb = mbB;
    const uint32_t node0 = f << kFineLog;
    const uint64_t wi = ((uint64_t)node0 >> 5) + tid;
    uint32_t knode0, c3order;
    node_key(w.tlog, w.tmask, w.key, (uint64_t)w.base + node0, K_ORDER, knode0, c3order);
    const uint32_t c3delay = (c3order & 0xFFFFFFu) | (K_DELAY << 24);
    const bool in = wi < w.W * 2;
    const uint32_t recv0 = p_in ? p_recv0 : 0u, crash0 = p_in ? p_crash0 : 0u, roll0 = p_in ? p_roll0 : 0u;
    const uint32_t fcv = tid < w.R ? p_fcv : 0u;
    if (i + 1 < nb) next_bucket(i + 1);
    if (roll0) w.rollw[wi] = 0u;
    const uint32_t rollw = roll0 & ~crash0;
#pragma unroll
    for (uint32_t k = 0; k < kBitTicks; ++k)
      if (k < L) sm.b1[k][tid] = 0;
    sm.cr0[tid] = make_uint2(crash0, rollw);
    if (tid < w.R) sm.fc[tid] = fcv;
    if (tid < kMaxWindow) sm.dead[tid] = 0;
    if (tid == 0) { sm.ndup = 0; sm.ninf = 0; sm.err = M >= (1u << 28) ? 3 : 0; sm.cls = M >= 1024 ? 1 : 0; }
    __syncthreads();
    stamp(w, sm, 1);
    const uint32_t* gm = w.fmsg + mb;
    unsigned long long dlo = 0, dhi = 0;
    auto flush_dead = [&]() {
      while (dlo) {
        const uint32_t b = __builtin_ctzll(dlo) >> 3;
        atomicAdd(&sm.dead[b], (uint32_t)(dlo >> (8 * b)) & 255u);
        dlo &= ~(255ull << (8 * b));
      }
      while (dhi) {
        const uint32_t b = __builtin_ctzll(dhi) >> 3;
        atomicAdd(&sm.dead[8 + b], (uint32_t)(dhi >> (8 * b)) & 255u);
        dhi &= ~(255ull << (8 * b));
      }
    };
#define GS_RESOLVE_BATCH(m, VALID)                                                                \
    {                                                                                             \
      uint2 sp[kU];                                                                               \
      _Pragma("unroll") for (uint32_t u = 0; u < kU; ++u) {                                       \
        sp[u] = make_uint2(0, 0);                                                                 \
        if (VALID) {                                                                              \
          const uint32_t loc = msg_loc(m[u]);                                                     \
          atomicOr(&sm.b1[msg_tick(m[u])][loc >> 5], 1u << (loc & 31));          \
          sp[u] = GS_RESOLVE_CR0(loc);                                                            \
        }                                                                                         \
      }                                                                                           \
      uint32_t dm = 0;                                  \
      _Pragma("unroll") for (uint32_t u = 0; u < kU; ++u) {                                       \
        const uint32_t sh = msg_loc(m[u]) & 31, k = msg_tick(m[u]);                               \
        if ((sp[u].x >> sh) & 1u) {            \
          if (k < 8) dlo += 1ull << (8 * k);                                                      \
          else dhi += 1ull << (8 * (k - 8));                                                      \
        }                                                                                         \
        if ((sp[u].y >> sh) & 1u) dm |= 1u << u;                                                  \
      }                                                                                           \
      if (nbat % 31 == 30) flush_dead();                                                          \
      const uint32_t nd = __popc(dm);                                                             \
      if (__ballot(nd != 0)) {                                                                    \
        uint32_t pre = 0, tot = 0;                                  \
        _Pragma("unroll") for (uint32_t bb = 0; bb < 4; ++bb) {                                   \
          const unsigned long long bal = __ballot((nd >> bb) & 1u);                               \
          pre += lanes_below(bal) << bb;                                                                \
          tot += (uint32_t)__popcll(bal) << bb;                                                   \
        }                                                                                         \
        uint32_t base = 0;                                                                        \
        if (lane_id() == 0) base = atomicAdd(&sm.ndup, tot);                                      \
        uint32_t at = __builtin_amdgcn_readfirstlane(base) + pre;                                 \
        _Pragma("unroll") for (uint32_t u = 0; u < kU; ++u) if ((dm >> u) & 1u) {                 \
          if (at < kRolledCap) w.rlmsg[(size_t)f * kRolledCap + at] = m[u] & ((1u << 19) - 1);    \
          else sm.err = 3;                                                                        \
          ++at;                                                                                   \
        }                                                                                         \
      }                                                                                           \
    }
    {
      uint32_t m[kU];
#pragma unroll
      for (uint32_t u = 0; u < kU; ++u) m[u] = pm[u];
      for (uint32_t p0 = 0, nbat = 0; p0 < (sm.err == 3 ? 0u : M); p0 += kBatch, ++nbat) {
        uint32_t mn[kU];
        if (p0 + kBatch < M) ld(gm, M, p0 + kBatch, mn);
        GS_RESOLVE_BATCH(m, p0 + u * kResolveBlock + tid < M)
#pragma unroll
        for (uint32_t u = 0; u < kU; ++u) m[u] = mn[u];
      }
    }
#undef GS_RESOLVE_BATCH
    flush_dead();
    stamp(w, sm, 2);
    __syncthreads();
    if (i + 1 < nb) prefetch(fB, MB, mbB);
    if (tid == 0) w.rlcnt[f] = sm.err == 3 ? 0u : min(sm.ndup, kRolledCap);
    stamp(w, sm, 3);
    uint32_t rw = recv0, cw = crash0;
    if (sm.err != 3) {
      if (tid < L && sm.dead[tid]) atomicAdd(&sm.st[tid][0], sm.dead[tid]);
      uint32_t infk[kBitTicks], ninf = 0;
      const uint32_t plain = ~(crash0 | rollw);
#pragma unroll
      for (uint32_t k = 0; k < kBitTicks; ++k) {
        infk[k] = 0;
        if (k >= L) continue;
        const uint32_t infS = sm.b1[k][tid] & plain & ~rw;
        rw |= infS;
        infk[k] = infS;
      }
      stamp(w, sm, 4);
#pragma unroll
      for (uint32_t k = 0; k < kBitTicks; ++k) {
        const uint32_t ni = __popc(infk[k]);
        acc_ni[k / 2] += ni << (16 * (k & 1));
        ninf += ni;
      }
      stamp(w, sm, 5);
      __syncthreads();
      stamp(w, sm, 6);
      auto bcast = [&](uint32_t x) {
        const uint32_t loc = msg_loc(x), t = t0 + msg_tick(x);
        const uint32_t off = fire_offset(w.delay_low, w.delay_span,
                                         philox(knode0 + loc, t, 0, c3delay, w.key.k0, w.key.k1).x);
        const uint32_t slot = (t + off) % w.R;
        const uint32_t pos = atomicAdd(&sm.fc[slot], 1u);
        w.flist[((size_t)slot * w.nfine + f) * kFineNodes + pos] = (uint16_t)loc;
      };
      uint32_t* inf = &sm.cnt[0];
      {
        uint32_t pre = 0, tot = 0;
#pragma unroll
        for (uint32_t b = 0; b < 9; ++b) {
          const unsigned long long bal = __ballot((ninf >> b) & 1u);
          pre += lanes_below(bal) << b;
          tot += (uint32_t)__popcll(bal) << b;
        }
        uint32_t base = 0;
        if (tot && lane_id() == 0) base = atomicAdd(&sm.ninf, tot);
        uint32_t at = __builtin_amdgcn_readfirstlane(base) + pre;
#pragma unroll
        for (uint32_t k = 0; k < kBitTicks; ++k)
          for (uint32_t x = k < L ? infk[k] : 0u; x; x &= x - 1)
            inf[at++] = (tid * 32 + __builtin_ctz(x)) | (k << kFineLog);
      }
      __syncthreads();
      stamp(w, sm, 7);
      const uint32_t ni_all = sm.ninf;
      for (uint32_t q = tid; q < ni_all; q += kResolveBlock) bcast(inf[q]);
    } else {
      __syncthreads();
      uint4* c4 = reinterpret_cast<uint4*>(sm.cnt);
      for (uint32_t q = tid; q < kFineNodes / 4; q += kResolveBlock) c4[q] = make_uint4(0, 0, 0, 0);
      sm.recv[tid] = recv0;
      sm.crash[tid] = crash0;
      sm.nrecv[tid] = 0;
      sm.ncrash[tid] = 0;
      __syncthreads();
      for (uint32_t k = 0; k < L; ++k) resolve_tick(w, sm, f, gm, 0, M, k, t0 + k);
      rw = sm.recv[tid] | sm.nrecv[tid];
      cw = sm.crash[tid] | sm.ncrash[tid];
      if (tid == 0 && sm.err == 1) atomicOr(w.err, kErrArrivals);
    }
    __syncthreads();
    stamp(w, sm, 8);
    if (in) {
      if (rw != recv0) rwg[wi] = rw;
      if (cw != crash0) cwg[wi] = cw;
    }
    if (tid < w.R) w.fcount[(size_t)tid * w.nfine + f] = sm.fc[tid];
    stamp(w, sm, 9);
    if (w.dbg && tid == 0) sm.stamp[sm.cls][0] += 1;
    if (w.tstat) flush_counts(w, sm, acc_ni, L, (uint32_t)(((uint64_t)w.base + node0) >> w.tlog));
  }
  if (w.dbg && tid < 2 * kStampPhases) atomicAdd(&w.dbg[tid], (&sm.stamp[0][0])[tid]);
  if (!w.tstat) flush_counts(w, sm, acc_ni, L, ~0u);
}
__global__ __launch_bounds__(kResolveBlock, GS_RESOLVE_WAVES) void k_resolve2(const WinState w, uint32_t t0, uint32_t L) {
  resolve_body(w, t0, L);
}
__global__ __launch_bounds__(kResolveBlock, GS_RESOLVE_WAVES) void k_resolve2_m(const WinState* __restrict__ ws,
                                                                                 uint32_t L) {
  resolve_body(ws[blockIdx.y], 0u, L);
}

constexpr uint32_t kInfCap = 6656;
constexpr uint32_t kResolveWaves3 = 6;
struct ResolveLds3 {
  uint32_t b1[kBitTicks][kBitWords];
  union {
    uint2 cr0[kBitWords];
    uint32_t inf[kInfCap];
  };
  uint32_t fc[kWinMaxRing];
  uint32_t st[kMaxWindow][4];
  uint32_t dead[kMaxWindow];
  uint32_t blist[kResolveMaxBuckets];
  unsigned long long bstart[kResolveMaxBuckets];
  uint32_t bcnt[kResolveMaxBuckets];
  uint32_t ndup;
  uint32_t ninf;
  uint32_t err;
  uint32_t nb;
  uint32_t cls;
  unsigned long long stamp[2][kStampPhases];
  unsigned long long tlast;
};
static_assert(sizeof(ResolveLds3) <= 53 * 1024, "three workgroups per CU");
static_assert(kBitTicks * 6 <= 64, "6-bit dead counts per tick in one register pair");

__device__ __forceinline__ void resolve3_body(const WinState& w, uint32_t t0, uint32_t L) {
  __shared__ ResolveLds3 sm;
  const uint32_t tid = threadIdx.x, G = gridDim.x;
  L = win_live(w, t0, L);
  if (!L) return;
  if (tid < kMaxWindow * 4) (&sm.st[0][0])[tid] = 0;
  if (tid == 0) { sm.nb = 0; sm.cls = 0; }
  if (tid < 2 * kStampPhases) (&sm.stamp[0][0])[tid] = 0;
  __syncthreads();
  {
    const uint32_t f = blockIdx.x + tid * G;
    const unsigned long long fl = tid < kResolveMaxBuckets && f < w.nfine ? w.ffill[f] : 0ull;
    const bool ne = fl > kSmallMax;
    const uint32_t at = wave_append(&sm.nb, ne);
    if (ne) {
      sm.blist[at] = f;
      sm.bstart[at] = w.fstart[f];
      sm.bcnt[at] = (uint32_t)fl;
    }
  }
  __syncthreads();
  const uint32_t nb = sm.nb;
  stamp(w, sm, 0);
  uint32_t* rwg = (uint32_t*)w.recv;
  uint32_t* cwg = (uint32_t*)w.crash;
  uint32_t acc_ni[kBitTicks / 2];
#pragma unroll
  for (uint32_t k = 0; k < kBitTicks / 2; ++k) acc_ni[k] = 0;
  constexpr uint32_t kU = 4;
  constexpr uint32_t kBatch = kResolveBlock * kU;
  auto ld = [&](const uint32_t* gm, uint32_t M, uint32_t p0, uint32_t (&m)[kU]) {
#pragma unroll
    for (uint32_t u = 0; u < kU; ++u) {
      const uint32_t p = p0 + u * kResolveBlock + tid;
      m[u] = *reinterpret_cast<const uint32_t*>(reinterpret_cast<const char*>(gm) + ((p < M ? p : M - 1) << 2));
    }
  };
  uint32_t pm[kU], p_recv0 = 0, p_crash0 = 0, p_roll0 = 0, p_fcv = 0;
  bool p_in = false;
  auto prefetch = [&](uint32_t j) {
    const uint32_t f = sm.blist[j];
    const uint64_t wi = ((uint64_t)(f << kFineLog) >> 5) + tid;
    const bool in = wi < w.W * 2;
    const uint64_t wc = in ? wi : w.W * 2 - 1;
    p_in = in;
    p_recv0 = rwg[wc];
    p_crash0 = cwg[wc];
    p_roll0 = w.rollw[wc];
    p_fcv = w.fcount[(size_t)(tid < w.R ? tid : 0u) * w.nfine + f];
    ld(w.fmsg + sm.bstart[j], sm.bcnt[j], 0, pm);
  };
  if (nb > 0) prefetch(0);
  for (uint32_t i = 0; i < nb; ++i) {
    const uint32_t f = sm.blist[i], M = sm.bcnt[i];
    const uint32_t* gm = w.fmsg + sm.bstart[i];
    uint32_t m[kU];
#pragma unroll
    for (uint32_t u = 0; u < kU; ++u) m[u] = pm[u];
    const uint32_t node0 = f << kFineLog;
    const uint64_t wi = ((uint64_t)node0 >> 5) + tid;
    const bool in = p_in;
    const uint32_t recv0 = in ? p_recv0 : 0u, crash0 = in ? p_crash0 : 0u, roll0 = in ? p_roll0 : 0u;
    if (roll0) w.rollw[wi] = 0u;
    const uint32_t rollw = roll0 & ~crash0;
#pragma unroll
    for (uint32_t k = 0; k < kBitTicks; ++k)
      if (k < L) sm.b1[k][tid] = 0;
    sm.cr0[tid] = make_uint2(crash0, rollw);
    if (tid < w.R) sm.fc[tid] = p_fcv;
    if (tid < kMaxWindow) sm.dead[tid] = 0;
    if (tid == 0) { sm.ndup = 0; sm.ninf = 0; sm.err = M >= (1u << 28) ? 3 : 0; sm.cls = M >= 1024 ? 1 : 0; }
    __syncthreads();
    stamp(w, sm, 1);
    unsigned long long dd = 0;
    auto flush_dead = [&]() {
      while (dd) {
        const uint32_t b = (uint32_t)__builtin_ctzll(dd) / 6;
        atomicAdd(&sm.dead[b], (uint32_t)(dd >> (6 * b)) & 63u);
        dd &= ~(63ull << (6 * b));
      }
    };
    for (uint32_t p0 = 0, nbat = 0; p0 < (sm.err == 3 ? 0u : M); p0 += kBatch, ++nbat) {
      uint32_t mn[kU];
      if (p0 + kBatch < M) ld(gm, M, p0 + kBatch, mn);
      uint2 sp[kU];
#pragma unroll
      for (uint32_t u = 0; u < kU; ++u) {
        const uint32_t loc = msg_loc(m[u]);
        atomicOr(&sm.b1[msg_tick(m[u])][loc >> 5], 1u << (loc & 31));
        sp[u] = GS_RESOLVE_CR0(loc);
      }
      uint32_t dm = 0;
#pragma unroll
      for (uint32_t u = 0; u < kU; ++u) {
        const uint32_t sh = msg_loc(m[u]) & 31, k = msg_tick(m[u]);
        const uint32_t valid = p0 + u * kResolveBlock + tid < M ? 1u : 0u;
        dd += (unsigned long long)((sp[u].x >> sh) & valid) << (6 * k);
        dm |= ((sp[u].y >> sh) & valid) << u;
      }
      if (nbat % 15 == 14) flush_dead();
      if (__ballot(dm != 0)) {
        const uint32_t nd = __popc(dm);
        uint32_t pre = 0, tot = 0;
#pragma unroll
        for (uint32_t bb = 0; bb < 3; ++bb) {
          const unsigned long long bal = __ballot((nd >> bb) & 1u);
          pre += lanes_below(bal) << bb;
          tot += (uint32_t)__popcll(bal) << bb;
        }
        uint32_t base = 0;
        if (lane_id() == 0) base = atomicAdd(&sm.ndup, tot);
        uint32_t at = __builtin_amdgcn_readfirstlane(base) + pre;
#pragma unroll
        for (uint32_t u = 0; u < kU; ++u) if ((dm >> u) & 1u) {
          if (at < kRolledCap) w.rlmsg[(size_t)f * kRolledCap + at] = m[u] & ((1u << 19) - 1);
          else sm.err = 3;
          ++at;
        }
      }
#pragma unroll
      for (uint32_t u = 0; u < kU; ++u) m[u] = mn[u];
    }
    flush_dead();
    stamp(w, sm, 2);
    __syncthreads();
    if (i + 1 < nb) prefetch(i + 1);
    const bool large = sm.err == 3;
    if (tid == 0) {
      w.rlcnt[f] = large ? 0u : sm.ndup;
      if (large) w.lgl[2 + atomicAdd(&w.lgl[0], 1u)] = f;
    }
    stamp(w, sm, 3);
    if (!large) {
      if (tid < L && sm.dead[tid]) atomicAdd(&sm.st[tid][0], sm.dead[tid]);
      const uint32_t plain = ~(crash0 | rollw);
      uint32_t rw = recv0, ninf = 0;
#pragma unroll
      for (uint32_t k = 0; k < kBitTicks; ++k) {
        if (k >= L) continue;
        const uint32_t infS = sm.b1[k][tid] & plain & ~rw;
        rw |= infS;
        const uint32_t ni = __popc(infS);
        acc_ni[k / 2] += ni << (16 * (k & 1));
        ninf += ni;
      }
      stamp(w, sm, 4);
      stamp(w, sm, 5);
      stamp(w, sm, 6);
      if (in && rw != recv0) rwg[wi] = rw;
      uint32_t at0;
      {
        uint32_t pre = 0, tot = 0;
#pragma unroll
        for (uint32_t b = 0; b < 9; ++b) {
          const unsigned long long bal = __ballot((ninf >> b) & 1u);
          pre += lanes_below(bal) << b;
          tot += (uint32_t)__popcll(bal) << b;
        }
        uint32_t base = 0;
        if (tot && lane_id() == 0) base = atomicAdd(&sm.ninf, tot);
        at0 = __builtin_amdgcn_readfirstlane(base) + pre;
      }
      for (uint32_t r0 = 0;; r0 += kInfCap) {
        uint32_t at = at0 - r0, r = recv0;
#pragma unroll
        for (uint32_t k = 0; k < kBitTicks; ++k) {
          if (k >= L) continue;
          uint32_t x = sm.b1[k][tid] & plain & ~r;
          r |= x;
          for (; x; x &= x - 1, ++at)
            if (at < kInfCap) sm.inf[at] = (tid * 32 + __builtin_ctz(x)) | (k << kFineLog);
        }
        __syncthreads();
        stamp(w, sm, 7);
        const uint32_t left = sm.ninf - r0;
        for (uint32_t q = tid; q < min(left, kInfCap); q += kResolveBlock) {
          const uint32_t x = sm.inf[q];
          const uint32_t loc = msg_loc(x), t = t0 + msg_tick(x);
          uint32_t knode0, c3order;
          node_key(w.tlog, w.tmask, w.key, (uint64_t)w.base + node0, K_ORDER, knode0, c3order);
          const uint32_t c3delay = (c3order & 0xFFFFFFu) | (K_DELAY << 24);
          const uint32_t off = fire_offset(w.delay_low, w.delay_span,
                                           philox(knode0 + loc, t, 0, c3delay, w.key.k0, w.key.k1).x);
          const uint32_t slot = (t + off) % w.R;
          const uint32_t pos = atomicAdd(&sm.fc[slot], 1u);
          w.flist[((size_t)slot * w.nfine + f) * kFineNodes + pos] = (uint16_t)loc;
        }
        if (left <= kInfCap) break;
        __syncthreads();
      }
    }
    __syncthreads();
    stamp(w, sm, 8);
    if (!large && tid < w.R) w.fcount[(size_t)tid * w.nfine + f] = sm.fc[tid];
    stamp(w, sm, 9);
    if (w.dbg && tid == 0) sm.stamp[sm.cls][0] += 1;
    if (w.tstat) flush_counts(w, sm, acc_ni, L, (uint32_t)(((uint64_t)w.base + node0) >> w.tlog));
  }
  if (w.dbg && tid < 2 * kStampPhases) atomicAdd(&w.dbg[tid], (&sm.stamp[0][0])[tid]);
  if (!w.tstat) flush_counts(w, sm, acc_ni, L, ~0u);
}
__global__ __launch_bounds__(kResolveBlock, kResolveWaves3) void k_resolve(const WinState w, uint32_t t0, uint32_t L) {
  resolve3_body(w, t0, L);
}
__global__ __launch_bounds__(kResolveBlock, kResolveWaves3) void k_resolve_m(const WinState* __restrict__ ws,
                                                                             uint32_t L) {
  resolve3_body(ws[blockIdx.y], 0u, L);
}

__device__ __forceinline__ void resolve_large_body(const WinState& w, uint32_t t0, uint32_t L) {
  __shared__ ResolveLds sm;
  const uint32_t n = w.lgl[0];
  if (!n) return;
  const uint32_t tid = threadIdx.x;
  L = win_live(w, t0, L);
  if (L) {
    if (tid < kMaxWindow * 4) (&sm.st[0][0])[tid] = 0;
    uint32_t acc_ni[kBitTicks / 2];
#pragma unroll
    for (uint32_t k = 0; k < kBitTicks / 2; ++k) acc_ni[k] = 0;
    uint32_t* rwg = (uint32_t*)w.recv;
    uint32_t* cwg = (uint32_t*)w.crash;
    for (uint32_t j = blockIdx.x; j < n; j += gridDim.x) {
      const uint32_t f = w.lgl[2 + j], M = (uint32_t)w.ffill[f];
      const uint32_t* gm = w.fmsg + w.fstart[f];
      const uint32_t node0 = f << kFineLog;
      const uint64_t wi = ((uint64_t)node0 >> 5) + tid;
      const bool in = wi < w.W * 2;
      const uint32_t recv0 = in ? rwg[wi] : 0u, crash0 = in ? cwg[wi] : 0u;
      uint4* c4 = reinterpret_cast<uint4*>(sm.cnt);
      for (uint32_t q = tid; q < kFineNodes / 4; q += kResolveBlock) c4[q] = make_uint4(0, 0, 0, 0);
      sm.recv[tid] = recv0;
      sm.crash[tid] = crash0;
      if (tid < w.R) sm.fc[tid] = w.fcount[(size_t)tid * w.nfine + f];
      if (tid == 0) sm.err = 0;
      __syncthreads();
      for (uint32_t k = 0; k < L; ++k) resolve_tick(w, sm, f, gm, 0, M, k, t0 + k);
      const uint32_t rw = sm.recv[tid], cw = sm.crash[tid];
      if (in) {
        if (rw != recv0) rwg[wi] = rw;
        if (cw != crash0) cwg[wi] = cw;
      }
      if (tid < w.R) w.fcount[(size_t)tid * w.nfine + f] = sm.fc[tid];
      if (tid == 0 && sm.err == 1) atomicOr(w.err, kErrArrivals);
      if (w.tstat) flush_counts(w, sm, acc_ni, L, (uint32_t)(((uint64_t)w.base + node0) >> w.tlog));
      else __syncthreads();
    }
    if (!w.tstat) flush_counts(w, sm, acc_ni, L, ~0u);
  }
  __syncthreads();
  if (tid == 0 && atomicAdd(&w.lgl[1], 1u) == gridDim.x - 1) {
    w.lgl[0] = 0;
    w.lgl[1] = 0;
  }
}
__global__ __launch_bounds__(kResolveBlock) void k_resolve_large(const WinState w, uint32_t t0, uint32_t L) {
  resolve_large_body(w, t0, L);
}
__global__ __launch_bounds__(kResolveBlock) void k_resolve_large_m(const WinState* __restrict__ ws, uint32_t L) {
  resolve_large_body(ws[blockIdx.y], 0u, L);
}

template <uint32_t E, bool ROLLED>
__device__ __forceinline__ void resolve_small_bucket(const WinState& w, uint32_t t0, uint32_t L, uint32_t f,
                                                     const uint32_t* gm, unsigned long long M,
                                                     uint32_t (*st)[kMaxWindow][4], uint32_t* skw,
                                                     uint32_t* fcw) {
  constexpr uint32_t N = 64 * E;
  const uint32_t lane = threadIdx.x & 63, wv = threadIdx.x >> 6;
  {
    const bool consume = !ROLLED && w.ctl;
    const uint32_t s0 = t0 % w.R;
    for (uint32_t s = lane; s < w.R; s += 64)
      fcw[s] = consume && (s + w.R - s0) % w.R < L ? 0u : w.fcount[(size_t)s * w.nfine + f];
    uint32_t knode0, c3order;
    node_key(w.tlog, w.tmask, w.key, (uint64_t)w.base + (f << kFineLog), K_ORDER, knode0, c3order);
    const uint32_t c3delay = (c3order & 0xFFFFFFu) | (K_DELAY << 24);
    uint32_t key[E];
#pragma unroll
    for (uint32_t r = 0; r < E; ++r) {
      const uint32_t i = lane * E + r;
      key[r] = ~0u;
      if (i < M) {
        const uint32_t m = gm[i];
        key[r] = (msg_loc(m) << 5) | (msg_tick(m) << 1) | ((m >> kRoll0Fine) & 1u);
        if (!ROLLED && ((m >> kRoll0Fine) & 1u)) w.rollw[((f << kFineLog) + msg_loc(m)) >> 5] = 0u;
      }
    }
#pragma unroll
    for (uint32_t k = 2; k <= N; k <<= 1)
#pragma unroll
      for (uint32_t j = k >> 1; j > 0; j >>= 1) {
        if (j >= E) {
#pragma unroll
          for (uint32_t r = 0; r < E; ++r) {
            const uint32_t i = lane * E + r;
            const uint32_t o = __shfl_xor(key[r], j / E, 64);
            const bool keep_min = ((i & j) == 0) == ((i & k) == 0);
            key[r] = keep_min ? min(key[r], o) : max(key[r], o);
          }
        } else {
#pragma unroll
          for (uint32_t r = 0; r < E; ++r) {
            if (r & j) continue;
            const bool up = ((lane * E + r) & k) == 0;
            const uint32_t a = key[r], b = key[r | j];
            key[r] = up ? min(a, b) : max(a, b);
            key[r | j] = up ? max(a, b) : min(a, b);
          }
        }
      }
#pragma unroll
    for (uint32_t r = 0; r < E; ++r) skw[lane * E + r] = key[r];
    wave_lds_sync();
    uint32_t* rwg = (uint32_t*)w.recv;
    uint32_t* cwg = (uint32_t*)w.crash;
    bool any_inf = false;
    uint32_t head = 0;
#pragma unroll
    for (uint32_t r = 0; r < E; ++r) {
      const uint32_t i = lane * E + r;
      if (key[r] != ~0u && !(i > 0 && (skw[i - 1] >> 5) == (key[r] >> 5))) head |= 1u << r;
    }
#pragma unroll 1
    for (uint32_t r = 0; r < E; ++r) {
      if (!((head >> r) & 1u)) continue;
      const uint32_t i = lane * E + r;
      const uint32_t loc = skw[i] >> 5;
      const uint32_t wi = ((f << kFineLog) + loc) >> 5, bit = 1u << (loc & 31), u = knode0 + loc;
      const uint32_t cw = cwg[wi];
      bool rv = (rwg[wi] & bit) != 0, cr = (cw & bit) != 0, inf = false;
      uint32_t tinf = 0;
      for (uint32_t q = i; q < N;) {
        const uint32_t e = skw[q];
        if ((e >> 5) != loc) break;
        const uint32_t k = (e >> 1) & (kMaxWindow - 1), t = t0 + k;
        uint32_t c = 0, ones = 0;
        for (; q < N && (skw[q] >> 1) == (e >> 1); ++q) {
          ++c;
          ones += skw[q] & 1u;
        }
        if (cr) {
          atomicAdd(&st[wv][k][0], c);
          continue;
        }
        const uint32_t g = ones ? first_crash(u, t, c, ones, c3order, w.key.k0, w.key.k1) : c + 1;
        if (g > 1 && !rv) {
          rv = inf = true;
          tinf = t;
          atomicAdd(&st[wv][k][1], 1u);
        }
        if (g <= c) {
          cr = true;
          atomicAdd(&st[wv][k][2], 1u);
          if (c > g) atomicAdd(&st[wv][k][0], c - g);
        }
      }
      if (cr && !(cw & bit)) atomicOr(&cwg[wi], bit);
      if (inf) {
        any_inf = true;
        atomicOr(&rwg[wi], bit);
        const uint32_t off = fire_offset(w.delay_low, w.delay_span,
                                         philox(u, tinf, 0, c3delay, w.key.k0, w.key.k1).x);
        const uint32_t slot = (tinf + off) % w.R;
        const uint32_t pos = atomicAdd(&fcw[slot], 1u);
        w.flist[((size_t)slot * w.nfine + f) * kFineNodes + pos] = (uint16_t)loc;
      }
    }
    wave_lds_sync();
    if (__ballot(any_inf)) {
      for (uint32_t s = lane; s < w.R; s += 64) w.fcount[(size_t)s * w.nfine + f] = fcw[s];
    } else if (consume && lane < L) {
      w.fcount[(size_t)((t0 + lane) % w.R) * w.nfine + f] = 0;
    }
    if (w.tstat) {
      wave_lds_sync();
      if (lane < L * 3) {
        const uint32_t k = lane / 3, fld = lane - k * 3;
        const uint32_t v = st[wv][k][fld];
        const uint32_t trial = (uint32_t)(((uint64_t)w.base + (f << kFineLog)) >> w.tlog);
        if (v) atomicAdd(&w.tstat[((size_t)trial * kMaxWindow + w.tofs + k) * kTStatFields + TS_DEAD + fld], v);
      }
    }
  }
}

template <bool ROLLED>
__device__ __forceinline__ void resolve_small_body(const WinState& w, uint32_t t0, uint32_t L) {
  constexpr uint32_t kWaves = (ROLLED ? kRolledBlock : kSmallBlock) / 64;
  constexpr uint32_t kEmax = ROLLED ? 16 : 4;
  __shared__ uint32_t st[kWaves][kMaxWindow][4];
  __shared__ uint32_t sk[kWaves][64 * kEmax];
  __shared__ uint32_t fcw[kWaves][kWinMaxRing];
  const uint32_t tid = threadIdx.x, wv = tid >> 6;
  static_assert(kWaves * kMaxWindow * 4 == kWaves * 64, "one counter per thread");
  static_assert(kRolledCap == 64 * 16, "the rolled bodies cover 1..kRolledCap");
  const uint32_t f = __builtin_amdgcn_readfirstlane(blockIdx.x * kWaves + wv);
  unsigned long long M = 0;
  const uint32_t* gm = nullptr;
  if (f < w.nfine) {
    if (ROLLED) {
      M = w.rlcnt[f];
      gm = w.rlmsg + (size_t)f * kRolledCap;
    } else {
      M = w.ffill[f];
      gm = w.fmsg + w.fstart[f];
    }
  }
  L = win_live(w, t0, L);
  if (!L) return;
  (&st[0][0][0])[tid] = 0;
  __syncthreads();
  if (M > 0 && M <= 64) resolve_small_bucket<1, ROLLED>(w, t0, L, f, gm, M, st, sk[wv], fcw[wv]);
  else if (M > 64 && M <= 256) resolve_small_bucket<4, ROLLED>(w, t0, L, f, gm, M, st, sk[wv], fcw[wv]);
  else if (ROLLED && M > 256 && M <= 512)
    resolve_small_bucket<ROLLED ? 8 : 1, ROLLED>(w, t0, L, f, gm, M, st, sk[wv], fcw[wv]);
  else if (ROLLED && M > 512 && M <= kRolledCap)
    resolve_small_bucket<ROLLED ? 16 : 1, ROLLED>(w, t0, L, f, gm, M, st, sk[wv], fcw[wv]);
  if (ROLLED && M && (threadIdx.x & 63) == 0) w.rlcnt[f] = 0;
  if (!ROLLED && w.ctl && !(M > 0 && M <= 256) && f < w.nfine && (threadIdx.x & 63) < L)
    w.fcount[(size_t)((t0 + (threadIdx.x & 63)) % w.R) * w.nfine + f] = 0;
  __syncthreads();
  if (tid < L * 3) {
    const uint32_t k = tid / 3, fld = tid - k * 3;
    uint32_t v = 0;
    for (uint32_t q = 0; q < kWaves; ++q) v += st[q][k][fld];
    unsigned long long* row = shard_row(w, k);
    if (v && fld == 0) atomicAdd(&row[ST_MSGS], 0ull - (unsigned long long)v);
    if (v && fld == 1) {
      atomicAdd(&row[ST_RECV], (unsigned long long)v);
      atomicAdd(&row[ST_SCHED], (unsigned long long)v);
    }
    if (v && fld == 2) atomicAdd(&row[ST_CRASH], (unsigned long long)v);
  }
}
template <bool ROLLED>
__global__ __launch_bounds__(ROLLED ? kRolledBlock : kSmallBlock) void k_resolve_small(const WinState w, uint32_t t0,
                                                                                       uint32_t L) {
  resolve_small_body<ROLLED>(w, t0, L);
}
template <bool ROLLED>
__global__ __launch_bounds__(ROLLED ? kRolledBlock : kSmallBlock) void k_resolve_small_m(
    const WinState* __restrict__ ws, uint32_t L) {
  resolve_small_body<ROLLED>(ws[blockIdx.y], 0u, L);
}

}

static bool resolve_occ3() {
  static const bool on = [] { const char* e = getenv("GS_RESOLVE_OCC3"); return !e || atoi(e) != 0; }();
  return on;
}

static uint32_t resolve_grid_env() {
  static const uint32_t g = [] { const char* e = getenv("GS_RESOLVE_GRID"); return e ? (uint32_t)std::max(atoi(e), 1) : 0u; }();
  return g;
}

hipError_t win_resolve(const WinState& w, uint32_t t0, uint32_t L, hipStream_t s) {
  const uint32_t cus = device_cus();
  const bool occ3 = resolve_occ3();
  static const uint32_t per_cu_env = [] { const char* e = getenv("GS_RESOLVE_PER_CU"); return e ? (uint32_t)std::max(atoi(e), 1) : 0u; }();
  const uint32_t per_cu = per_cu_env ? per_cu_env : occ3 ? 6u : 2u;
  uint32_t G = std::min<uint32_t>(w.nfine, resolve_grid_env() ? resolve_grid_env() : per_cu * cus);
  G = std::max<uint32_t>(G, (w.nfine + kResolveMaxBuckets - 1) / kResolveMaxBuckets);
  const uint32_t gs = (w.nfine + kSmallBlock / 64 - 1) / (kSmallBlock / 64);
  hipLaunchKernelGGL(k_resolve_small<false>, dim3(gs), dim3(kSmallBlock), 0, s, w, t0, L);
  static_assert(kSmallMax == 64 * 4, "the two bodies cover 1..kSmallMax");
  if (occ3) {
    hipLaunchKernelGGL(k_resolve, dim3(G), dim3(kResolveBlock), 0, s, w, t0, L);
    hipLaunchKernelGGL(k_resolve_large, dim3(std::min<uint32_t>(w.nfine, cus)), dim3(kResolveBlock), 0, s, w, t0, L);
  } else {
    hipLaunchKernelGGL(k_resolve2, dim3(G), dim3(kResolveBlock), 0, s, w, t0, L);
  }
  hipLaunchKernelGGL(k_resolve_small<true>, dim3((w.nfine + kRolledBlock / 64 - 1) / (kRolledBlock / 64)),
                     dim3(kRolledBlock), 0, s, w, t0, L);
  return hipGetLastError();
}

hipError_t win_resolve_g(const WinGroup& g, uint32_t L, hipStream_t s) {
  const uint32_t cus = device_cus();
  const bool occ3 = resolve_occ3();
  uint32_t G = std::min<uint32_t>(g.nfine_max,
                                  resolve_grid_env() ? resolve_grid_env() : ((occ3 ? 3 : 2) * cus + g.M - 1) / g.M);
  G = std::max<uint32_t>(G, (g.nfine_max + kResolveMaxBuckets - 1) / kResolveMaxBuckets);
  const uint32_t gs = (g.nfine_max + kSmallBlock / 64 - 1) / (kSmallBlock / 64);
  hipLaunchKernelGGL(k_resolve_small_m<false>, dim3(gs, g.M), dim3(kSmallBlock), 0, s, g.wr, L);
  if (occ3) {
    hipLaunchKernelGGL(k_resolve_m, dim3(G, g.M), dim3(kResolveBlock), 0, s, g.wr, L);
    hipLaunchKernelGGL(k_resolve_large_m, dim3(std::min<uint32_t>(g.nfine_max, (cus + g.M - 1) / g.M), g.M),
                       dim3(kResolveBlock), 0, s, g.wr, L);
  } else {
    hipLaunchKernelGGL(k_resolve2_m, dim3(G, g.M), dim3(kResolveBlock), 0, s, g.wr, L);
  }
  hipLaunchKernelGGL(k_resolve_small_m<true>, dim3((g.nfine_max + kRolledBlock / 64 - 1) / (kRolledBlock / 64), g.M),
                     dim3(kRolledBlock), 0, s, g.wr, L);
  return hipGetLastError();
}

}
```

gossip_simulator_amd/csrc/gs_win_shard.hip:

```cpp
#include "gs_win_dev.h"

namespace gs {
namespace {

__global__ void k_pack(const WinState w, const unsigned long long* poff, uint32_t nreg, uint32_t* out) {
  const uint32_t r = blockIdx.x;
  if (r >= nreg || poff[r] == ~0ull) return;
  if (w.dd && (*w.err & kErrAbort)) return;
  const unsigned long long f = region_fill(w, r);
  const uint32_t* src = w.cmsg + w.ccap[r];
  uint32_t* dst = out + poff[r];
  for (unsigned long long i = (unsigned long long)blockIdx.y * blockDim.x + threadIdx.x; i < f;
       i += (unsigned long long)gridDim.y * blockDim.x)
    dst[i] = src[i];
}

__global__ void k_consume_sh(const WinState w, uint32_t t0, uint32_t L) {
  for (uint32_t i = blockIdx.x * blockDim.x + threadIdx.x; i < L * w.nfine; i += gridDim.x * blockDim.x) {
    const uint32_t k = i / w.nfine, f = i - k * w.nfine;
    w.fcount[(size_t)((t0 + k) % w.R) * w.nfine + f] = 0;
  }
}


__device__ __forceinline__ void rtab_body(const WinState& w, unsigned long long* rtab,
                                          const unsigned long long* const* ccaps, const uint32_t* const* src,
                                          uint32_t nsrc, uint32_t travels) {
  __shared__ unsigned long long s_x[4];
  __shared__ unsigned long long s_R[256];
  __shared__ uint32_t s_abort;
  const uint32_t tid = threadIdx.x;
  uint32_t t0;
  if (!win_live(w, t0, 0)) return;
  const uint32_t G = w.G, me = w.rank, B8 = w.obins * kCoarseSub, nreg = G * B8;
  constexpr size_t K1 = kRegions + 1;
  static_assert(kRegions == 8 * 256, "eight regions per thread");
  if (nreg > kRegions) {
    if (tid == 0) atomicOr(w.err, kErrAbort);
    return;
  }
  unsigned long long *rcap = rtab, *rend = rtab + K1, *rfill = rtab + 2 * K1, *mypoff = rtab + 3 * K1;
  s_R[tid] = 0;
  if (tid == 0) s_abort = 0;
  __syncthreads();
  uint32_t fl = 0;
  for (uint32_t s = tid; s < G; s += 256) fl |= (uint32_t)w.glay[(size_t)s * kDDRow + kRegions];
  if (fl & (kErrCoarse | kErrAbort)) atomicOr(&s_abort, 1u);
  for (uint32_t s = 0; s < G; ++s) {
    const unsigned long long* row = w.glay + (size_t)s * kDDRow;
    for (uint32_t r = tid; r < nreg; r += 256) {
      const unsigned long long f = row[r];
      if (f) atomicAdd(&s_R[r / B8], f);
    }
  }
  __syncthreads();
  for (uint32_t d = tid; d < G; d += 256) {
    const unsigned long long lo = (unsigned long long)d * w.seg_per;
    const unsigned long long nd = min((unsigned long long)w.seg_per, (unsigned long long)w.nglob - lo);
    const unsigned long long ncd = (((nd + kFineNodes - 1) >> kFineLog) + 255) / 256;
    const unsigned long long R = s_R[d];
    if (R + R / 8 + ncd * 256 * 513 + 16 > w.glay[(size_t)d * kDDRow + kRegions + 1]) atomicOr(&s_abort, 2u);
  }
  __syncthreads();
  if (s_abort) {
    if (tid == 0) atomicOr(w.err, kErrAbort);
    return;
  }
  for (uint32_t rr = tid; rr < K1; rr += 256) {
    rcap[rr] = rend[rr] = rfill[rr] = 0;
    mypoff[rr] = ~0ull;
  }
  __syncthreads();
  const uint32_t in_src = travels ? 0u : G;
  const uint32_t per = (B8 + 255) / 256;
  unsigned long long in_s = 0, tot = 0;
  for (uint32_t s = 0; s < G; ++s) {
    const bool tr = travels && s != me;
    const unsigned long long* row = w.glay + (size_t)s * kDDRow + (size_t)me * B8;
    const unsigned long long* cc = ccaps[travels ? 0u : s] + (size_t)me * B8;
    unsigned long long f[8], sum = 0;
#pragma unroll
    for (uint32_t j = 0; j < 8; ++j) {
      const uint32_t i = tid * per + j;
      f[j] = j < per && i < B8 ? row[i] : 0ull;
      sum += f[j];
    }
    unsigned long long btot;
    unsigned long long off = block_exscan_u64<4>(sum, s_x, &btot);
#pragma unroll
    for (uint32_t j = 0; j < 8; ++j) {
      const uint32_t i = tid * per + j;
      if (j >= per || i >= B8) continue;
      const uint32_t c = i / kCoarseSub, x = i % kCoarseSub;
      const size_t rr = ((size_t)c * G + s) * kCoarseSub + x;
      const unsigned long long at = tr ? ((unsigned long long)in_src << kSrcShift) | (in_s + off)
                                       : ((unsigned long long)(travels ? 1u : s) << kSrcShift) | cc[i];
      rcap[rr] = at;
      rend[rr] = at + f[j];
      rfill[rr] = f[j];
      off += f[j];
    }
    if (tr) in_s += btot;
    tot += btot;
  }
  if (travels) {
    const unsigned long long* row = w.glay + (size_t)me * kDDRow;
    const uint32_t per2 = (nreg + 255) / 256;
    unsigned long long f[8], sum = 0;
#pragma unroll
    for (uint32_t j = 0; j < 8; ++j) {
      const uint32_t r = tid * per2 + j;
      f[j] = j < per2 && r < nreg && r / B8 != me ? row[r] : 0ull;
      sum += f[j];
    }
    unsigned long long btot;
    unsigned long long off = block_exscan_u64<4>(sum, s_x, &btot);
#pragma unroll
    for (uint32_t j = 0; j < 8; ++j) {
      const uint32_t r = tid * per2 + j;
      if (j >= per2 || r >= nreg || r / B8 == me) continue;
      mypoff[r] = off;
      off += f[j];
    }
  }
  if (tid < nsrc) rtab[4 * K1 + tid] = (unsigned long long)(uintptr_t)src[tid];
  if (tid == 0) rtab[kRtabTotal] = tot;
}
__global__ __launch_bounds__(256) void k_rtab(const WinState w, unsigned long long* rtab,
                                              const unsigned long long* const* ccaps, const uint32_t* const* src,
                                              uint32_t nsrc, uint32_t travels) {
  rtab_body(w, rtab, ccaps, src, nsrc, travels);
}
__global__ __launch_bounds__(256) void k_rtab_m(const WinState* __restrict__ ws, const WinState* __restrict__ wr,
                                                const unsigned long long* const* ccaps, const uint32_t* const* src,
                                                uint32_t nsrc) {
  rtab_body(ws[blockIdx.x], const_cast<unsigned long long*>(wr[blockIdx.x].ccap), ccaps, src, nsrc, 0u);
}

__device__ void close_rows(const WinState& w, const unsigned long long* rows, WinCtl* const* ctls, uint32_t n,
                           uint32_t slot) {
  const uint32_t tid = threadIdx.x;
  constexpr uint32_t F = kMaxWindow * kStatFields;
  const WinCtl* c0 = ctls[0];
  const bool dead = rows[F + 2] != 0;
  const uint32_t t0 = c0->t, L = dead || c0->stop ? 0u : c0->L;
  unsigned long long* st = w.stage + (size_t)slot * kStageWords;
  for (uint32_t i = tid; i < F; i += blockDim.x) st[8 + i] = i / kStatFields < L ? rows[i] : 0ull;
  if (tid != 0) return;
  uint32_t stop = c0->stop;
  if (L) {
    unsigned long long recv = c0->recv, crashed = c0->crashed, pending = c0->pending;
    for (uint32_t j = 0; j < L; ++j) {
      recv += rows[j * kStatFields + ST_RECV];
      crashed += rows[j * kStatFields + ST_CRASH];
      pending += rows[j * kStatFields + ST_SCHED] - rows[j * kStatFields + ST_FIRED];
    }
    const uint32_t tl = t0 + L - 1;
    if (c0->poll && (tl - c0->pbase) % c0->poll == 0 && !stop) {
      if (recv >= c0->cover) stop = 1 + GS_RUN_COVERED;
      else if (pending == 0) stop = 1 + GS_RUN_QUIESCENT;
      else if (tl >= c0->max_ticks) stop = 1 + GS_RUN_MAX_TICKS;
    }
    for (uint32_t q = 0; q < n; ++q) {
      WinCtl* c = ctls[q];
      c->recv = recv;
      c->crashed = crashed;
      c->pending = pending;
      c->stop = stop;
    }
  }
  st[0] = t0;
  st[1] = L;
  st[2] = stop;
  st[3] = (dead ? kErrAbort : 0u) | (rows[F] ? kErrArrivals : 0u);
  st[4] = rows[F + 1];
}

__device__ __forceinline__ void stats_dd_body(const WinState& w, uint32_t slot) {
  __shared__ unsigned long long rows[kDDWStat];
  const uint32_t tid = threadIdx.x;
  const CtlView c = ctl_view(w);
  const bool dead = (c.err & stop_bits(w)) != 0;
  const uint32_t L = dead || c.stop ? 0u : c.L;
  const uint32_t i = tid / kCloseLanes, part = tid % kCloseLanes, k = i / kStatFields;
  unsigned long long sum = 0;
  if (k < L) sum = stat_shard_sum(w, i, part);
  if (part == 0) {
    w.wstat[i] = sum;
    rows[i] = sum;
  }
  if (tid < 8) {
    constexpr uint32_t F = kMaxWindow * kStatFields;
    unsigned long long v = 0;
    if (tid == 0) v = (c.err & kErrArrivals) ? 1 : 0;
    if (tid == 1) v = !w.solo && (c.err & kErrFine) ? 1 : 0;
    if (tid == 2) v = dead ? 1 : 0;
    w.wstat[F + tid] = v;
    rows[F + tid] = v;
  }
  if (tid == 0 && !w.solo && (c.err & kErrFine)) atomicAnd(w.err, ~kErrFine);
  if (!w.solo) return;
  __syncthreads();
  WinCtl* const one[1] = {w.ctl};
  close_rows(w, rows, one, 1, slot);
}
__global__ void k_stats_dd(const WinState w, uint32_t slot) { stats_dd_body(w, slot); }
__global__ void k_stats_dd_m(const WinState* __restrict__ ws, uint32_t slot) { stats_dd_body(ws[blockIdx.x], slot); }

__global__ __launch_bounds__(128) void k_close_dd(const WinState w, const unsigned long long* const* wstats,
                                                  WinCtl* const* ctls, uint32_t n, uint32_t slot) {
  __shared__ unsigned long long rows[kDDWStat];
  const uint32_t tid = threadIdx.x;
  for (uint32_t i = tid; i < kDDWStat; i += blockDim.x) {
    unsigned long long v = 0;
    for (uint32_t q = 0; q < n; ++q) v += wstats[q][i];
    rows[i] = v;
  }
  __syncthreads();
  close_rows(w, rows, ctls, n, slot);
}

}

hipError_t win_rtab(const WinState& w, unsigned long long* rtab, const unsigned long long* const* ccaps,
                    const uint32_t* const* src, uint32_t nsrc, uint32_t travels, hipStream_t s) {
  hipLaunchKernelGGL(k_rtab, dim3(1), dim3(256), 0, s, w, rtab, ccaps, src, nsrc, travels);
  return hipGetLastError();
}

hipError_t win_stats_dd(const WinState& w, uint32_t slot, hipStream_t s) {
  hipLaunchKernelGGL(k_stats_dd, dim3(1), dim3(kMaxWindow * kStatFields * kCloseLanes), 0, s, w, slot);
  return hipGetLastError();
}

hipError_t win_close_dd(const WinState& w, const unsigned long long* const* wstats, WinCtl* const* ctls,
                        uint32_t n, uint32_t slot, hipStream_t s) {
  hipLaunchKernelGGL(k_close_dd, dim3(1), dim3(128), 0, s, w, wstats, ctls, n, slot);
  return hipGetLastError();
}

hipError_t win_rtab_g(const WinGroup& g, const unsigned long long* const* ccaps, const uint32_t* const* src,
                      uint32_t nsrc, hipStream_t s) {
  hipLaunchKernelGGL(k_rtab_m, dim3(g.M), dim3(256), 0, s, g.ws, g.wr, ccaps, src, nsrc);
  return hipGetLastError();
}

hipError_t win_stats_dd_g(const WinGroup& g, uint32_t slot, hipStream_t s) {
  hipLaunchKernelGGL(k_stats_dd_m, dim3(g.M), dim3(kMaxWindow * kStatFields * kCloseLanes), 0, s, g.ws, slot);
  return hipGetLastError();
}

hipError_t win_consume_sh(const WinState& w, uint32_t t0, uint32_t L, hipStream_t s) {
  const uint32_t blocks = std::min<uint32_t>((L * w.nfine + 255) / 256, 2048);
  hipLaunchKernelGGL(k_consume_sh, dim3(blocks ? blocks : 1), dim3(256), 0, s, w, t0, L);
  return hipGetLastError();
}

hipError_t win_pack(const WinState& w, const unsigned long long* poff, uint32_t nreg, uint32_t* out, hipStream_t s) {
  if (!nreg) return hipSuccess;
  hipLaunchKernelGGL(k_pack, dim3(nreg, 8), dim3(256), 0, s, w, poff, nreg, out);
  return hipGetLastError();
}

}
```

gossip_simulator_amd/csrc/gs_win_units.hip:

```cpp
#include <hipcub/hipcub.hpp>

#include "gs_win_dev.h"

namespace gs {
namespace {

__device__ __forceinline__ void units_body(const WinState& w, uint32_t t0, uint32_t L) {
  __shared__ uint32_t s_t[kMaxWindow];
  uint32_t Ls = L;
  if (w.ctl) {
    L = win_open(w, t0);
    if (!L) return;
    Ls = w.lstride;
  }
  const uint32_t units = Ls * w.nfine;
  const uint32_t tid = blockIdx.x * blockDim.x + threadIdx.x, nth = gridDim.x * blockDim.x;
  __shared__ uint32_t s_tile[256 * (kMaxWindow + 1)];
  uint32_t acc[kMaxWindow];
#pragma unroll
  for (uint32_t k = 0; k < kMaxWindow; ++k) acc[k] = 0;
  if (threadIdx.x < kMaxWindow) s_t[threadIdx.x] = 0;
  if (tid == 0) w.usize[units] = 0;
  __syncthreads();
  __shared__ uint32_t s_ts[kMaxWindow];
  uint32_t slot[kMaxWindow];
#pragma unroll
  for (uint32_t k = 0; k < kMaxWindow; ++k) slot[k] = k < L ? (t0 + k) % w.R : 0u;
  for (uint32_t f0 = blockIdx.x * 256; f0 < w.nfine; f0 += gridDim.x * 256) {
    const uint32_t f = f0 + threadIdx.x;
    if (threadIdx.x < kMaxWindow) s_ts[threadIdx.x] = 0;
    uint32_t cv[kMaxWindow];
#pragma unroll
    for (uint32_t k = 0; k < kMaxWindow; ++k)
      cv[k] = k < L && k < Ls && f < w.nfine ? w.fcount[(size_t)slot[k] * w.nfine + f] : 0u;
#pragma unroll
    for (uint32_t k = 0; k < kMaxWindow; ++k) {
      if (k < Ls) {
        s_tile[threadIdx.x * (kMaxWindow + 1) + k] = cv[k];
        acc[k] += cv[k];
      }
    }
    __syncthreads();
#pragma unroll
    for (uint32_t k = 0; k < kMaxWindow; ++k) {
      if (k < Ls) {
        const uint32_t c = wave_sum(s_tile[threadIdx.x * (kMaxWindow + 1) + k]);
        if ((threadIdx.x & 63) == 0 && c) atomicAdd(&s_ts[k], c);
      }
    }
    __syncthreads();
    if (threadIdx.x < Ls) w.tsum[(size_t)(f0 >> 8) * kMaxWindow + threadIdx.x] = s_ts[threadIdx.x];
    const uint32_t nb = min(256u, w.nfine - f0), base = f0 * Ls;
    for (uint32_t i = threadIdx.x; i < nb * Ls; i += 256) {
      const uint32_t b = i / Ls, k = i - b * Ls;
      w.usize[base + i] = s_tile[b * (kMaxWindow + 1) + k];
    }
    __syncthreads();
  }
#pragma unroll
  for (uint32_t k = 0; k < kMaxWindow; ++k)
    if (acc[k]) atomicAdd(&s_t[k], acc[k]);
  __syncthreads();
  if (threadIdx.x < L && s_t[threadIdx.x]) atomicAdd(&w.tfires[threadIdx.x], (unsigned long long)s_t[threadIdx.x]);
  for (uint32_t i = tid; i < kRegions; i += nth) { w.chist[i] = 0; w.cfill[i] = 0; }
  for (uint32_t i = tid; i < w.nfine; i += nth) w.ffill[i] = 0;
  if (w.dd && tid == 0) {
    w.cfill[kRegions] = 0;
    w.cfill[kRegions + 1] = w.ctl->fmsg_cap;
    w.cfill[kRegions + 2] = w.ctl->xs_cap;
    w.cfill[kRegions + 3] = w.ctl->xr_cap;
  }
  if (tid == 0 && !w.ctl && !w.abort_on_err) *w.err &= ~(kErrCoarse | kErrFine);
}
__global__ __launch_bounds__(256) void k_units(const WinState w, uint32_t t0, uint32_t L) { units_body(w, t0, L); }

__global__ __launch_bounds__(256) void k_units_m(const WinState* __restrict__ ws, uint32_t t0, uint32_t L) {
  units_body(ws[blockIdx.y], t0, L);
}

__device__ __forceinline__ void cut_body(const WinState& w, unsigned long long budget) {
  __shared__ unsigned long long s_sz[256];
  __shared__ unsigned long long s_T;
  __shared__ uint32_t s_go, s_L;
  WinCtl* c = w.ctl;
  const uint32_t b = threadIdx.x;
  __shared__ unsigned long long s_tf[kMaxWindow];
  if (win_abort(w)) return;
  uint32_t t = 0;
  const uint32_t Lw = win_open(w, t);
  const unsigned long long cap = c->cmsg_cap;
  __shared__ unsigned long long s_own[kMaxWindow];
  if (b < kMaxWindow) {
    if (w.dd) {
      unsigned long long g = 0;
      for (uint32_t r = 0; r < w.G; ++r) g += w.gcnt[(size_t)r * kMaxWindow + b];
      s_tf[b] = g;
      s_own[b] = w.tfires[b];
    } else {
      s_tf[b] = w.tfires[b];
    }
  }
  unsigned long long ts[4][kMaxWindow];
#pragma unroll
  for (uint32_t j = 0; j < 4; ++j)
#pragma unroll
    for (uint32_t k = 0; k < kMaxWindow; ++k)
      ts[j][k] = Lw && b * 4 + j < w.ncoarse ? w.tsum[(size_t)(b * 4 + j) * kMaxWindow + k] : 0ull;
  __syncthreads();
  if (b == 0) {
    s_go = Lw != 0;
    if (!Lw) {
      c->L = 0;
      c->Tn = 0;
    } else {
      uint32_t L = 1;
      unsigned long long Tn = s_tf[0];
      while (L < Lw && (Tn + s_tf[L]) * w.stride <= budget) Tn += s_tf[L++];
      if (w.dd) {
        Tn = 0;
        for (uint32_t k = 0; k < L; ++k) Tn += s_own[k];
      } else {
        for (uint32_t k = 0; k < kMaxWindow; ++k) w.tfires[k] = 0;
      }
      c->t = t;
      c->L = L;
      s_L = L;
      c->tnext = t + L;
      c->Tn = Tn;
      c->T = Tn * (w.owner ? w.slots : w.stride);
      s_T = c->T;
    }
  }
  __syncthreads();
  if (!s_go) return;
  {
    const uint32_t L = s_L, nt = w.ncoarse;
    unsigned long long v[4], sum = 0;
#pragma unroll
    for (uint32_t j = 0; j < 4; ++j) {
      v[j] = 0;
#pragma unroll
      for (uint32_t k = 0; k < kMaxWindow; ++k) v[j] += k < L ? ts[j][k] : 0ull;
      sum += v[j];
    }
    unsigned long long tot;
    unsigned long long pre = block_exscan_u64<4>(sum, &s_sz[0], &tot);
#pragma unroll
    for (uint32_t j = 0; j < 4; ++j) {
      const uint32_t tile = b * 4 + j;
      if (tile < nt) w.toff[tile] = pre;
      pre += v[j];
    }
    if (b == 0) w.toff[nt] = tot;
    __syncthreads();
  }
  unsigned long long sub = 0;
  if (!w.owner) {
    const unsigned long long lo = (unsigned long long)b << kCoarseShift;
    const unsigned long long hi = min((unsigned long long)w.n, lo + (1ull << kCoarseShift));
    const double xr = (double)kXRoundNodes * w.stride;
    sub = b < w.ncoarse
              ? (unsigned long long)(((double)s_T / kCoarseSub + xr) * (double)(hi - lo) / (double)w.n) + 512
              : 0ull;
  } else {
    const uint32_t d = b / w.obins, k = b % w.obins;
    unsigned long long cnt = 0;
    if (d < w.G) {
      const unsigned long long dlo = (unsigned long long)d * w.seg_per;
      const unsigned long long dhi = min(dlo + w.seg_per, (unsigned long long)w.nglob);
      const unsigned long long lo = dlo + ((unsigned long long)k << kCoarseShift);
      const unsigned long long hi = min(dhi, lo + (1ull << kCoarseShift));
      cnt = hi > lo ? hi - lo : 0ull;
    }
    const double xr = (double)kXRoundNodes * w.slots;
    sub = cnt ? (unsigned long long)(((double)s_T / kCoarseSub + xr) * (double)cnt / (double)w.nglob) + 512 : 0ull;
  }
  unsigned long long total;
  const unsigned long long base = block_exscan_u64<4>(sub * kCoarseSub, &s_sz[0], &total);
  if (total > cap) {
    for (uint32_t x = 0; x < kCoarseSub; ++x) w.ccap[b * kCoarseSub + x] = 0;
    if (b == 0) {
      w.ccap[kRegions] = 0;
      atomicOr(w.err, kErrCoarse);
      if (w.dd) atomicOr(reinterpret_cast<unsigned int*>(&w.cfill[kRegions]), kErrCoarse);
    }
    return;
  }
  for (uint32_t x = 0; x < kCoarseSub; ++x) w.ccap[b * kCoarseSub + x] = base + x * sub;
  if (b == 255) w.ccap[kRegions] = total;
}
__global__ __launch_bounds__(256) void k_cut(const WinState w, unsigned long long budget) { cut_body(w, budget); }
__global__ __launch_bounds__(256) void k_cut_m(const WinState* __restrict__ ws, unsigned long long budget) {
  cut_body(ws[blockIdx.x], budget);
}

__device__ __forceinline__ void unitscan_body(const WinState& w) {
  __shared__ unsigned long long s_x[4];
  if (blockIdx.x >= w.ncoarse) return;
  uint32_t t0;
  const uint32_t L = win_live(w, t0, 0);
  if (!L) return;
  const uint32_t Ls = w.lstride, tile = blockIdx.x, f = tile * 256 + threadIdx.x;
  if (w.dd && tile == 0 && threadIdx.x < kMaxWindow) w.tfires[threadIdx.x] = 0;
  unsigned long long sz[kMaxWindow], sum = 0;
#pragma unroll
  for (uint32_t k = 0; k < kMaxWindow; ++k)
    sz[k] = k < L && f < w.nfine ? w.usize[(size_t)f * Ls + k] : 0ull;
#pragma unroll
  for (uint32_t k = 0; k < kMaxWindow; ++k) sum += sz[k];
  unsigned long long tot;
  unsigned long long a = w.toff[tile] + block_exscan_u64<4>(sum, s_x, &tot);
  if (f >= w.nfine) return;
#pragma unroll
  for (uint32_t k = 0; k < kMaxWindow; ++k) {
    if (k >= Ls) break;
    const uint32_t u = f * Ls + k;
    w.unit_off[u] = a;
    const unsigned long long b = a + sz[k];
    for (unsigned long long q = (a + 63) >> 6; (q << 6) < b; ++q) w.gmap[q] = u;
    a = b;
  }
  if (f == w.nfine - 1) w.unit_off[(size_t)w.nfine * Ls] = a;
}
__global__ __launch_bounds__(256) void k_unitscan(const WinState w) { unitscan_body(w); }
__global__ __launch_bounds__(256) void k_unitscan_m(const WinState* __restrict__ ws) { unitscan_body(ws[blockIdx.y]); }

__global__ void k_groupmap(const WinState w, uint32_t L) {
  if (w.ctl) {
    uint32_t t0;
    if (!win_live(w, t0, 0)) return;
    L = w.lstride;
  }
  const uint32_t units = L * w.nfine;
  for (uint32_t u = blockIdx.x * blockDim.x + threadIdx.x; u < units; u += gridDim.x * blockDim.x) {
    const unsigned long long a = w.unit_off[u], b = w.unit_off[u + 1];
    for (unsigned long long q = (a + 63) >> 6; (q << 6) < b; ++q) w.gmap[q] = u;
  }
}

__global__ void k_stats_reduce(const WinState w, uint32_t t0, uint32_t L) {
  if (w.abort_on_err && win_abort(w)) return;
  const uint32_t i = threadIdx.x / kCloseLanes, part = threadIdx.x % kCloseLanes;
  const uint32_t k = i / kStatFields, fld = i % kStatFields;
  if (k >= L) return;
  const unsigned long long sum = stat_shard_sum(w, i, part);
  if (part == 0 && sum) w.stats[(size_t)((t0 + k) % kStatSlots) * kStatFields + fld] += sum;
}

__global__ void k_close(const WinState w, uint32_t slot) {
  __shared__ unsigned long long rows[kMaxWindow][kStatFields];
  WinCtl* c = w.ctl;
  unsigned long long* st = w.stage + (size_t)slot * kStageWords;
  uint32_t t0 = 0;
  const uint32_t L = win_live(w, t0, 0);
  const uint32_t i = threadIdx.x / kCloseLanes, part = threadIdx.x % kCloseLanes, tid = threadIdx.x;
  const uint32_t k = i / kStatFields, fld = i % kStatFields;
  if (k < L) {
    const unsigned long long sum = stat_shard_sum(w, i, part);
    if (part == 0) {
      rows[k][fld] = sum;
      w.stats[(size_t)((t0 + k) % kStatSlots) * kStatFields + fld] = sum;
      st[8 + k * kStatFields + fld] = sum;
    }
  }
  __syncthreads();
  if (tid != 0) return;
  uint32_t stop = c->stop;
  if (L) {
    for (uint32_t j = 0; j < L; ++j) {
      c->recv += rows[j][ST_RECV];
      c->crashed += rows[j][ST_CRASH];
      c->pending += rows[j][ST_SCHED] - rows[j][ST_FIRED];
    }
    const uint32_t tl = t0 + L - 1;
    if (c->poll && (tl - c->pbase) % c->poll == 0 && !stop) {
      if (c->recv >= c->cover) stop = 1 + GS_RUN_COVERED;
      else if (c->pending == 0) stop = 1 + GS_RUN_QUIESCENT;
      else if (tl >= c->max_ticks) stop = 1 + GS_RUN_MAX_TICKS;
      c->stop = stop;
    }
  }
  st[0] = t0;
  st[1] = L;
  st[2] = stop;
  st[3] = *w.err;
  st[4] = L ? c->Tn : 0;
}

__global__ void k_schedule_win(const WinState w, uint32_t node, uint32_t t, uint32_t trials, uint32_t n,
                               uint32_t* __restrict__ started) {
  const uint32_t i = blockIdx.x * blockDim.x + threadIdx.x;
  if (i >= trials) return;
  uint32_t local = node;
  if (trials > 1 || node == ~0u) {
    uint32_t v = node;
    if (node == ~0u) v = uniform(philox(0, 0, 0, ctr3(K_SENDER, w.key.trial + i), w.key.k0, w.key.k1).x, n);
    local = (i << w.tlog) | v;
  }
  if (started) {
    const bool dead = (w.crash[local >> 6] >> (local & 63)) & 1;
    started[i] = dead ? 0u : 1u;
    if (dead) return;
  }
  uint32_t kn, c3;
  node_key(w.tlog, w.tmask, w.key, (uint64_t)w.base + local, K_DELAY, kn, c3);
  const uint32_t off = fire_offset(w.delay_low, w.delay_span, philox(kn, t, 0, c3, w.key.k0, w.key.k1).x);
  const uint32_t s = (t + off) % w.R;
  const uint32_t f = local >> kFineLog;
  const uint32_t pos = atomicAdd(&w.fcount[(size_t)s * w.nfine + f], 1u);
  w.flist[((size_t)s * w.nfine + f) * kFineNodes + pos] = (uint16_t)(local & (kFineNodes - 1));
}

}

hipError_t win_units_g(const WinGroup& g, uint32_t L, hipStream_t s) {
  const uint32_t blocks = std::max<uint32_t>(std::min<uint32_t>((g.nfine_max + 255) / 256, 4096), 1);
  hipLaunchKernelGGL(k_units_m, dim3(blocks, g.M), dim3(256), 0, s, g.ws, 0u, L);
  return hipGetLastError();
}

hipError_t win_cut_g(const WinGroup& g, unsigned long long budget, hipStream_t s) {
  hipLaunchKernelGGL(k_cut_m, dim3(g.M), dim3(256), 0, s, g.ws, budget);
  return hipGetLastError();
}

hipError_t win_unitscan_g(const WinGroup& g, hipStream_t s) {
  hipLaunchKernelGGL(k_unitscan_m, dim3(std::max<uint32_t>(g.ncoarse_max, 1), g.M), dim3(256), 0, s, g.ws);
  return hipGetLastError();
}

hipError_t win_units(const WinState& w, uint32_t t0, uint32_t L, hipStream_t s) {
  (void)L;
  const uint32_t blocks = std::max<uint32_t>(std::min<uint32_t>((w.nfine + 255) / 256, 4096), 1);
  hipLaunchKernelGGL(k_units, dim3(blocks), dim3(256), 0, s, w, t0, L);
  return hipGetLastError();
}

hipError_t win_cut(const WinState& w, unsigned long long budget, hipStream_t s) {
  hipLaunchKernelGGL(k_cut, dim3(1), dim3(256), 0, s, w, budget);
  return hipGetLastError();
}

hipError_t win_unitscan(const WinState& w, hipStream_t s) {
  hipLaunchKernelGGL(k_unitscan, dim3(w.ncoarse), dim3(256), 0, s, w);
  return hipGetLastError();
}

hipError_t win_close(const WinState& w, uint32_t slot, hipStream_t s) {
  hipLaunchKernelGGL(k_close, dim3(1), dim3(kMaxWindow * kStatFields * kCloseLanes), 0, s, w, slot);
  return hipGetLastError();
}

hipError_t win_scan_units(const WinState& w, uint32_t L, void* tmp, size_t& tmp_bytes, hipStream_t s) {
  return hipcub::DeviceScan::ExclusiveSum(tmp, tmp_bytes, (const unsigned long long*)w.usize,
                                          w.unit_off, (int)(L * w.nfine + 1), s);
}

hipError_t win_groupmap(const WinState& w, uint32_t L, hipStream_t s) {
  const uint32_t units = L * w.nfine;
  const uint32_t blocks = std::min<uint32_t>((units + 255) / 256, 4096);
  hipLaunchKernelGGL(k_groupmap, dim3(blocks ? blocks : 1), dim3(256), 0, s, w, L);
  return hipGetLastError();
}

hipError_t win_stats_reduce(const WinState& w, uint32_t t0, uint32_t L, hipStream_t s) {
  hipLaunchKernelGGL(k_stats_reduce, dim3(1), dim3(kMaxWindow * kStatFields * kCloseLanes), 0, s, w, t0, L);
  return hipGetLastError();
}

hipError_t win_schedule(const WinState& w, uint32_t node, uint32_t tick, uint32_t trials, uint32_t n,
                        hipStream_t s, uint32_t* started) {
  hipLaunchKernelGGL(k_schedule_win, dim3((trials + 255) / 256), dim3(256), 0, s, w, node, tick, trials, n, started);
  return hipGetLastError();
}

}
```

gossip_simulator_amd/csrc/gs_windows.cpp:

```cpp
#include "gs_ctx.h"

namespace gs {

namespace {

void plan_coarse(gs_ctx* c, uint64_t T, const unsigned long long* exact) {
  const WinState& w = c->ws;
  unsigned long long a = 0;
  for (uint32_t b = 0; b < 256; ++b) {
    const uint64_t lo = (uint64_t)b << kCoarseShift;
    const uint64_t hi = std::min<uint64_t>(w.n, lo + (1ull << kCoarseShift));
    const double xr = (double)kXRoundNodes * w.stride;
    const unsigned long long sub =
        b < w.ncoarse ? (unsigned long long)(((double)T / kCoarseSub + xr) * (double)(hi - lo) / (double)w.n) + 512
                      : 0ull;
    for (uint32_t x = 0; x < kCoarseSub; ++x) {
      const uint32_t r = b * kCoarseSub + x;
      c->wn.h_cap[r] = a;
      if (b >= w.ncoarse) continue;
      a += exact ? exact[r] : sub;
    }
  }
  c->wn.h_cap[kRegions] = a;
}

void plan_coarse_trials(gs_ctx* c, const unsigned long long* fb, unsigned long long Tn) {
  const WinState& w = c->ws;
  uint32_t per_round = 0;
  const uint32_t blocks = win_expand_geometry(w, Tn, &per_round, nullptr, nullptr);
  const unsigned long long rounds = (Tn + per_round - 1) / per_round;
  const bool by_xcd = blocks && (blocks & 7) == 0;
  const unsigned long long per = (rounds + 7) >> 3;
  std::vector<unsigned long long> cap(kRegions, 0);
  for (uint32_t b = 0; b < w.ncoarse; ++b) {
    const unsigned long long lo = fb[b], hi = fb[b + 1];
    for (unsigned long long r = lo / per_round; lo < hi && r * per_round < hi; ++r) {
      const unsigned long long a = std::max(lo, r * per_round), e = std::min(hi, (r + 1) * per_round);
      const uint32_t x = by_xcd ? (uint32_t)std::min<unsigned long long>(r / per, 7) : (uint32_t)((r % blocks) & 7);
      cap[b * kCoarseSub + x] += (e - a) * w.slots;
    }
  }
  unsigned long long a = 0;
  for (uint32_t r = 0; r < kRegions; ++r) {
    c->wn.h_cap[r] = a;
    a += cap[r] ? cap[r] + 16 : 0;
  }
  c->wn.h_cap[kRegions] = a;
}

int run_windows(gs_ctx* c, uint64_t t0, uint32_t n, bool timing, uint64_t tchunk) {
  RC(expand_view(c));
  WinState& w = c->ws;
  const uint32_t Lmax = std::min<uint32_t>(std::max<int32_t>(c->p.delay_low, 1), kBitTicks);
  uint32_t done = 0, widx = 0;
  std::vector<std::pair<uint32_t, uint32_t>> evs;
  const uint64_t slot_budget = (uint64_t)w.nfine * kWinSlotsPerBucket;
  const bool trial_plan = c->trials > 1 && c->tlog <= kCoarseShift && !c->shard;
  while (done < n) {
    const uint32_t Lw = std::min(Lmax, n - done);
    const uint32_t t = (uint32_t)(t0 + done);
    w.tofs = (uint32_t)(t - tchunk);
    auto units = [&](uint32_t Lu) -> int {
      CK(c, hipMemsetAsync(w.tfires, 0, kMaxWindow * 8, c->stream));
      CK(c, win_units(w, t, Lu, c->stream));
      size_t need = 0;
      CK(c, win_scan_units(w, Lu, nullptr, need, c->stream));
      if (!grow(c->wn.tmp, need)) return fail(c, GS_ENOMEM, "cannot allocate scan scratch");
      need = c->wn.tmp.bytes;
      CK(c, win_scan_units(w, Lu, c->wn.tmp.p, need, c->stream));
      CK(c, hipMemcpyAsync(c->wn.h_misc, w.tfires, kMaxWindow * 8, hipMemcpyDeviceToHost, c->stream));
      if (trial_plan)
        CK(c, hipMemcpy2DAsync(c->wn.h_misc + kMaxWindow, 8, w.unit_off, (size_t)256 * Lu * 8, 8, w.ncoarse,
                               hipMemcpyDeviceToHost, c->stream));
      CK(c, hipStreamSynchronize(c->stream));
      return GS_OK;
    };
    RC(units(Lw));
    uint32_t L = 1;
    unsigned long long Tn = c->wn.h_misc[0];
    while (L < Lw && (Tn + c->wn.h_misc[L]) * w.stride <= slot_budget) Tn += c->wn.h_misc[L++];
    if (L < Lw) RC(units(L));
    const unsigned long long T = Tn * w.stride;
    if (trial_plan && Tn) {
      std::vector<unsigned long long> fb(c->wn.h_misc + kMaxWindow, c->wn.h_misc + kMaxWindow + w.ncoarse);
      fb.push_back(Tn);
      plan_coarse_trials(c, fb.data(), Tn);
    } else {
      plan_coarse(c, T, nullptr);
    }
    const uint64_t fcap = T + T / 8 + (uint64_t)w.ncoarse * 256 * 513 + 16;
    if (!grow(c->wn.gmap, ((Tn + 63) / 64 + 1) * 4) || !grow(c->wn.cmsg, (c->wn.h_cap[kRegions] + 16) * 4) ||
        !grow(c->wn.fmsg, (fcap + 16) * 4))
      return fail(c, GS_ENOMEM, "cannot allocate " + std::to_string(T) + " window messages");
    w.gmap = (uint32_t*)c->wn.gmap.p;
    w.cmsg = (uint32_t*)c->wn.cmsg.p;
    w.fmsg = (uint32_t*)c->wn.fmsg.p;
    if (timing)
      while (c->ev.size() < (size_t)(widx + 1) * 5) {
        hipEvent_t ev;
        CK(c, hipEventCreate(&ev));
        c->ev.push_back(ev);
      }
    hipEvent_t* e = timing ? &c->ev[(size_t)widx * 5] : nullptr;
    if (T) {
      CK(c, hipMemcpyAsync(w.ccap, c->wn.h_cap, (kRegions + 1) * 8, hipMemcpyHostToDevice, c->stream));
      CK(c, win_groupmap(w, L, c->stream));
      if (e) CK(c, hipEventRecord(e[0], c->stream));
      CK(c, win_expand(w, t, L, Tn, 1, c->stream));
      if (e) CK(c, hipEventRecord(e[1], c->stream));
      CK(c, win_plan(w, false, c->stream));
      CK(c, win_part2(w, T, true, c->stream));
      if (e) CK(c, hipEventRecord(e[2], c->stream));
      CK(c, hipMemcpyAsync(c->wn.h_misc, c->d_err, 4, hipMemcpyDeviceToHost, c->stream));
      CK(c, hipStreamSynchronize(c->stream));
      uint32_t err = (uint32_t)c->wn.h_misc[0];
      if (err & kErrCoarse) {
        ++c->timing.coarse_redos;
        CK(c, hipMemsetAsync(w.chist, 0, kRegions * 8, c->stream));
        CK(c, win_expand(w, t, L, Tn, 0, c->stream));
        CK(c, hipMemcpyAsync(c->wn.h_misc, w.chist, kRegions * 8, hipMemcpyDeviceToHost, c->stream));
        CK(c, hipStreamSynchronize(c->stream));
        plan_coarse(c, T, c->wn.h_misc);
        CK(c, hipMemcpyAsync(w.ccap, c->wn.h_cap, (kRegions + 1) * 8, hipMemcpyHostToDevice, c->stream));
        CK(c, hipMemsetAsync(w.cfill, 0, kRegions * 8, c->stream));
        CK(c, win_expand(w, t, L, Tn, 2, c->stream));
        CK(c, win_plan(w, false, c->stream));
        err = kErrFine;
      }
      if (err & kErrFine) {
        CK(c, hipMemsetAsync(w.fhist, 0, ((size_t)w.ncoarse * 256 + 1) * 8, c->stream));
        CK(c, win_plan(w, true, c->stream));
        CK(c, win_part2(w, T, false, c->stream));
        size_t need2 = 0;
        CK(c, win_scan_fine(w, nullptr, need2, c->stream));
        if (!grow(c->wn.tmp, need2)) return fail(c, GS_ENOMEM, "cannot allocate scan scratch");
        need2 = c->wn.tmp.bytes;
        CK(c, win_scan_fine(w, c->wn.tmp.p, need2, c->stream));
        CK(c, hipMemsetAsync(w.ffill, 0, (size_t)w.nfine * 8, c->stream));
        CK(c, win_part2(w, T, true, c->stream));
        ++c->timing.exact_redos;
      }
    } else if (e) {
      CK(c, hipEventRecord(e[0], c->stream));
      CK(c, hipEventRecord(e[1], c->stream));
      CK(c, hipEventRecord(e[2], c->stream));
    }
    const uint32_t s0 = t % w.R;
    const uint32_t first = std::min(L, w.R - s0);
    CK(c, hipMemsetAsync(w.fcount + (size_t)s0 * w.nfine, 0, (size_t)first * w.nfine * 4, c->stream));
    if (first < L) CK(c, hipMemsetAsync(w.fcount, 0, (size_t)(L - first) * w.nfine * 4, c->stream));
    if (e) CK(c, hipEventRecord(e[3], c->stream));
    if (T) CK(c, win_resolve(w, t, L, c->stream));
    if (T) CK(c, win_stats_reduce(w, t, L, c->stream));
    if (e) {
      CK(c, hipEventRecord(e[4], c->stream));
      evs.emplace_back(widx * 5, T ? 1u : 0u);
    }
    ++widx;
    done += L;
  }
  if (timing) {
    CK(c, hipStreamSynchronize(c->stream));
    for (auto& pr : evs) {
      hipEvent_t* e = &c->ev[pr.first];
      float ms = 0;
      CK(c, hipEventElapsedTime(&ms, e[0], e[1]));
      c->timing.expand_ms += ms;
      c->timing.deliver_ms += ms;
      CK(c, hipEventElapsedTime(&ms, e[1], e[2]));
      c->timing.part_ms += ms;
      c->timing.deliver_ms += ms;
      CK(c, hipEventElapsedTime(&ms, e[3], e[4]));
      c->timing.resolve_ms += ms;
      c->timing.deliver_launches += pr.second;
      c->timing.resolve_launches += pr.second;
      c->timing.windows += 1;
    }
  }
  uint32_t err = 0;
  CK(c, hipMemcpyAsync(&err, c->d_err, 4, hipMemcpyDeviceToHost, c->stream));
  CK(c, hipStreamSynchronize(c->stream));
  if (err & 4) return fail(c, GS_EOVERFLOW, "too many arrivals at one node in one tick");
  return GS_OK;
}

int async_setup(gs_ctx* c) {
  if (!c->aw.d_ctl) CK(c, dev_malloc(&c->aw.d_ctl, sizeof(WinCtl)));
  RC(alloc_stage(c));
  if (!grow(c->wn.gmap, ((c->ntot + 1 + 63) / 64 + 1) * 4) || !grow(c->wn.cmsg, 64) || !grow(c->wn.fmsg, 64))
    return fail(c, GS_ENOMEM, "cannot allocate the window message buffers");
  return GS_OK;
}

}

int alloc_stage(gs_ctx* c) {
  if (c->aw.h_stage) return GS_OK;
  CK(c, hipHostMalloc((void**)&c->aw.h_stage, (size_t)kSlots * kStageWords * 8,
                      hipHostMallocMapped | hipHostMallocPortable));
  CK(c, hipHostGetDevicePointer((void**)&c->aw.d_stage, c->aw.h_stage, 0));
  for (uint32_t i = 0; i < kSlots; ++i) {
    hipEvent_t e;
    CK(c, hipEventCreateWithFlags(&e, hipEventDisableTiming));
    c->aw.wev.push_back(e);
  }
  return GS_OK;
}

void release_async(gs_ctx* c) {
  if (c->aw.d_ctl) (void)dev_free(c->aw.d_ctl);
  if (c->aw.h_stage) (void)hipHostFree(c->aw.h_stage);
  for (hipEvent_t e : c->aw.wev) (void)hipEventDestroy(e);
}

void refresh_window(gs_ctx* c) {
  WinState& w = c->ws;
  w.deg = c->st.deg;
  w.ids = c->st.ids;
  w.recv = c->st.recv;
  w.crash = c->st.crash;
  w.rollw = c->st.rollw;
  w.stats = c->st.stats;
  w.err = c->d_err;
  w.stride = c->st.stride;
  w.slots = c->row_slots && c->row_slots < c->st.stride ? c->row_slots : c->st.stride;
  w.stride_magic = c->st.stride_magic;
  w.abort_on_err = c->shard ? 1u : 0u;
}

bool async_ok(const gs_ctx* c) {
  return c->win && !c->pp && !c->shard && !c->group && c->trials == 1 && !c->async_off &&
         !(c->p.flags & GS_FLAG_TIMING);
}

uint64_t cover_threshold(uint64_t n) {
  uint64_t lo = 0, hi = n;
  while (lo < hi) {
    const uint64_t mid = (lo + hi) / 2;
    if (covered(mid, n)) hi = mid; else lo = mid + 1;
  }
  return lo;
}

int run_async(gs_ctx* c, uint64_t tend, uint32_t poll, uint64_t max_ticks, const OnTick& on_tick, uint32_t* stop,
              bool* fallback) {
  *stop = 0;
  *fallback = false;
  RC(async_setup(c));
  RC(expand_view(c));
  WinState w = c->ws;
  w.ctl = c->aw.d_ctl;
  w.stage = c->aw.d_stage;
  w.lstride = std::min<uint32_t>(std::max<int32_t>(c->p.delay_low, 1), kBitTicks);
  w.gmap = (uint32_t*)c->wn.gmap.p;
  w.cmsg = (uint32_t*)c->wn.cmsg.p;
  w.fmsg = (uint32_t*)c->wn.fmsg.p;
  WinCtl h{};
  h.tnext = (uint32_t)(c->t + 1);
  h.tend = (uint32_t)std::min<uint64_t>(tend, 0xFFFFFFFFull);
  h.poll = poll;
  h.pbase = (uint32_t)c->t;
  h.lmax = w.lstride;
  h.recv = c->recv;
  h.crashed = c->crashed;
  h.pending = c->pending;
  h.cover = cover_threshold(c->p.n);
  h.max_ticks = max_ticks;
  h.cmsg_cap = c->wn.cmsg.bytes / 4 > 16 ? c->wn.cmsg.bytes / 4 - 16 : 0;
  h.fmsg_cap = c->wn.fmsg.bytes / 4 > 16 ? c->wn.fmsg.bytes / 4 - 16 : 0;
  CK(c, hipMemcpyAsync(c->aw.d_ctl, &h, sizeof h, hipMemcpyHostToDevice, c->stream));
  CK(c, hipMemsetAsync(w.tfires, 0, kMaxWindow * 8, c->stream));
  const uint64_t budget = (uint64_t)w.nfine * kWinSlotsPerBucket;
  const uint64_t Tn_bound = std::min<uint64_t>(c->ntot + 1, 4096ull * 1024),
                 T_bound = std::min<uint64_t>((c->ntot + 1) * w.stride, 2048ull * 16384);
  auto enqueue = [&](uint32_t slot) -> int {
    CK(c, win_units(w, 0, w.lstride, c->stream));
    CK(c, win_cut(w, budget, c->stream));
    CK(c, win_unitscan(w, c->stream));
    CK(c, win_expand(w, 0, w.lstride, Tn_bound, 1, c->stream));
    CK(c, win_plan(w, false, c->stream));
    CK(c, win_part2(w, T_bound, true, c->stream));
    CK(c, win_resolve(w, 0, w.lstride, c->stream));
    CK(c, win_close(w, slot, c->stream));
    CK(c, hipEventRecord(c->aw.wev[slot], c->stream));
    return GS_OK;
  };
  auto absorb = [&](uint32_t slot, int* what) -> int {
    CK(c, hipEventSynchronize(c->aw.wev[slot]));
    const unsigned long long* st = c->aw.h_stage + (size_t)slot * kStageWords;
    const uint32_t t0 = (uint32_t)st[0], L = (uint32_t)st[1];
    *what = 0;
    if (st[3] & (kErrCoarse | kErrFine)) {
      *fallback = true;
      *what = 1;
      return GS_OK;
    }
    if (c->winlog) fprintf(stderr, "[win] t0=%u L=%u Tn=%llu stop=%llu\n", t0, L, st[4], st[2]);
    for (uint32_t k = 0; k < L; ++k) on_tick((uint64_t)t0 + k, st + 8 + (size_t)k * kStatFields);
    if (st[2]) *stop = (uint32_t)st[2];
    if (st[2] || L == 0 || (uint64_t)t0 + L >= tend) *what = 1;
    return GS_OK;
  };
  RC(enqueue(0));
// ... 116 lines not shown
```

Baseline: 86.77 billion.

## Split per-slot fire lists into sub-lists with packed 16-bit counters

Fire-count storage shrinks from 32-bit to 16-bit counters. Each fine region's per-slot fire list can optionally be split into 2 or 4 sub-lists (compile-time GS_FIRE_SUB), whose counters are packed into 32-bit words and bumped with shifted atomics. Unit sizing, tile sums, scans and the expand indexing are rebased from fine regions onto sub-lists, and the per-wave fcw shared buffer becomes dynamically sized by ring length. The intent is to cut counter memory and memset traffic and to shorten the fire lists that one unit walks. The cost is extra packing and shift arithmetic, more units to scan when sub-lists are enabled, and reliance on counts staying below 65536.

```diff
diff --git a/gossip_simulator_amd/csrc/gs_ctx.cpp b/gossip_simulator_amd/csrc/gs_ctx.cpp
--- a/gossip_simulator_amd/csrc/gs_ctx.cpp
+++ b/gossip_simulator_amd/csrc/gs_ctx.cpp
@@ -106,14 +106,17 @@
       return fail(c, GS_ENOMEM, "cannot allocate the shard's receive layout");
   }
   auto al = [](size_t b) { return (b + 255) & ~(size_t)255; };
-  const size_t units = (size_t)kMaxWindow * w.nfine + 1;
-  const size_t b_fc = al((size_t)w.R * w.nfine * 4), b_units = al(units * 8),
+  static const bool one_sub = [] { const char* e = getenv("GS_FIRESUB"); return e && atoi(e) == 1; }();
+  w.fshift = one_sub ? kFineLog : kFineLog - kFireSubLog;
+  const size_t nsub = (size_t)w.nfine * kFireSub, ntile = (nsub + 255) / 256;
+  const size_t units = (size_t)kMaxWindow * nsub + 1;
+  const size_t b_fc = al((size_t)w.R * nsub * sizeof *w.fcount), b_units = al(units * 8),
                b_small = al(kRegions * 8) * 2 + al((kRegions + 1) * 8) + al((kRegions + 1) * 4) + al(kMaxWindow * 8),
                b_fhist = al(((size_t)w.ncoarse * 256 + 1) * 8), b_fbase = al(((size_t)w.nfine + 1) * 8),
                b_ffill = al((size_t)w.nfine * 8),
                b_sst = al((size_t)kStatShards * kMaxWindow * kStatFields * 8),
                b_rlcnt = al((size_t)w.nfine * 4) + al(((size_t)w.nfine + 2) * 4),
-               b_tsum = al((size_t)w.ncoarse * kMaxWindow * 8) + al(((size_t)w.ncoarse + 1) * 8);
+               b_tsum = al(ntile * kMaxWindow * 8) + al((ntile + 1) * 8);
   const size_t total = b_fc + 2 * b_units + b_small + b_fhist + b_fbase + b_ffill + b_sst + b_rlcnt + b_tsum;
   if (dev_malloc(&c->wn.d_win, total) != hipSuccess)
     return fail(c, GS_ENOMEM, "cannot allocate window-engine buffers");
@@ -121,7 +124,7 @@
   if (dev_malloc(&c->wn.d_flist, flist) != hipSuccess)
     return fail(c, GS_ENOMEM, "cannot allocate " + std::to_string(flist >> 20) + " MiB of fire lists");
   char* q = (char*)c->wn.d_win;
-  w.fcount = (uint32_t*)q; q += b_fc;
+  w.fcount = (uint16_t*)q; q += b_fc;
   w.usize = (unsigned long long*)q; q += b_units;
   w.unit_off = (unsigned long long*)q; q += b_units;
   w.chist = (unsigned long long*)q; q += al(kRegions * 8);
@@ -136,8 +139,8 @@
   w.sstats = (unsigned long long*)q; q += b_sst;
   w.rlcnt = (uint32_t*)q; q += al((size_t)w.nfine * 4);
   w.lgl = (uint32_t*)q; q += al(((size_t)w.nfine + 2) * 4);
-  w.tsum = (unsigned long long*)q; q += al((size_t)w.ncoarse * kMaxWindow * 8);
-  w.toff = (unsigned long long*)q; q += al(((size_t)w.ncoarse + 1) * 8);
+  w.tsum = (unsigned long long*)q; q += al(ntile * kMaxWindow * 8);
+  w.toff = (unsigned long long*)q; q += al((ntile + 1) * 8);
   if (dev_malloc(&c->wn.d_rlmsg, (size_t)w.nfine * kRolledCap * 4) != hipSuccess)
     return fail(c, GS_ENOMEM, "cannot allocate the rolled-receipt lists");
   w.rlmsg = (uint32_t*)c->wn.d_rlmsg;
@@ -145,7 +148,7 @@
   if (getenv("GS_STAMPS") && dev_malloc(&w.dbg, kDbgWords * 8) == hipSuccess)
     (void)hipMemset(w.dbg, 0, kDbgWords * 8);
   w.flist = (uint16_t*)c->wn.d_flist;
-  c->wn.fcount_bytes = (size_t)w.R * w.nfine * 4;
+  c->wn.fcount_bytes = (size_t)w.R * nsub * sizeof *w.fcount;
   if (hipMemsetAsync(c->wn.d_win, 0, total, c->stream) != hipSuccess)
     return fail(c, GS_EDEVICE, "memset of window buffers failed");
   c->wn.misc_words = std::max<size_t>(4096, (size_t)c->G * kMaxWindow + 64);
diff --git a/gossip_simulator_amd/csrc/gs_internal.h b/gossip_simulator_amd/csrc/gs_internal.h
--- a/gossip_simulator_amd/csrc/gs_internal.h
+++ b/gossip_simulator_amd/csrc/gs_internal.h
@@ -67,6 +67,13 @@
 
 constexpr uint32_t kFineLog = 14;
 constexpr uint32_t kFineNodes = 1u << kFineLog;
+#ifndef GS_FIRE_SUB
+#define GS_FIRE_SUB 1
+#endif
+constexpr uint32_t kFireSub = GS_FIRE_SUB;
+constexpr uint32_t kFireSubLog = kFireSub == 4 ? 2 : kFireSub == 2 ? 1 : 0;
+static_assert(kFireSub == 1u << kFireSubLog && kFireSub <= 4, "kFireSub is 1, 2 or 4");
+constexpr uint32_t kSubNodes = kFineNodes / kFireSub;
 constexpr uint32_t kCoarseShift = kFineLog + 8;
 constexpr uint32_t kMaxWindow = 16;
 constexpr uint32_t kCoarseSub = 8;
@@ -106,8 +113,9 @@
   uint32_t* lgl;
   unsigned long long* stats;
   uint32_t* err;
-  uint32_t* fcount;
+  uint16_t* fcount;
   uint16_t* flist;
+  uint32_t fshift;
   unsigned long long* usize;
   unsigned long long* unit_off;
   unsigned long long* tfires;
@@ -215,6 +223,7 @@
   uint32_t nfine_max;
   uint32_t ncoarse_max;
   uint32_t slots_max;
+  uint32_t ring_max;
 };
 hipError_t win_units_g(const WinGroup& g, uint32_t L, hipStream_t s);
 hipError_t win_cut_g(const WinGroup& g, unsigned long long budget, hipStream_t s);
diff --git a/gossip_simulator_amd/csrc/gs_shards.cpp b/gossip_simulator_amd/csrc/gs_shards.cpp
--- a/gossip_simulator_amd/csrc/gs_shards.cpp
+++ b/gossip_simulator_amd/csrc/gs_shards.cpp
@@ -751,6 +751,7 @@
       grp.nfine_max = std::max(grp.nfine_max, ws[i].nfine);
       grp.ncoarse_max = std::max(grp.ncoarse_max, ws[i].ncoarse);
       grp.slots_max = std::max(grp.slots_max, ws[i].slots);
+      grp.ring_max = std::max(grp.ring_max, ws[i].R);
     }
   }
   auto bsize = [&](uint32_t s, uint32_t d) {
diff --git a/gossip_simulator_amd/csrc/gs_win_dev.h b/gossip_simulator_amd/csrc/gs_win_dev.h
--- a/gossip_simulator_amd/csrc/gs_win_dev.h
+++ b/gossip_simulator_amd/csrc/gs_win_dev.h
@@ -116,5 +116,29 @@
 __device__ __forceinline__ uint32_t msg_loc(uint32_t m) { return m & (kFineNodes - 1); }
 __device__ __forceinline__ uint32_t msg_tick(uint32_t m) { return (m >> kFineLog) & (kMaxWindow - 1); }
 
+__host__ __device__ __forceinline__ uint32_t win_nsub(const WinState& w) { return w.nfine * kFireSub; }
+__host__ __device__ __forceinline__ uint32_t win_ntile(const WinState& w) { return (win_nsub(w) + 255) / 256; }
+__device__ __forceinline__ uint16_t* fc_at(const WinState& w, uint32_t s, uint32_t f, uint32_t j) {
+  return &w.fcount[((size_t)s * w.nfine + f) * kFireSub + j];
+}
+__device__ __forceinline__ uint16_t* flist_at(const WinState& w, uint32_t s, uint32_t f) {
+  return &w.flist[((size_t)s * w.nfine + f) * kFineNodes];
+}
+constexpr uint32_t kFcWords = kFireSub > 1 ? kFireSub / 2 : 1;
+__device__ __forceinline__ uint32_t fc_word(const WinState& w, uint32_t f, uint32_t i) {
+  if (kFireSub == 1) return *fc_at(w, i, f, 0);
+  return *reinterpret_cast<const uint32_t*>(fc_at(w, i / kFcWords, f, 2 * (i % kFcWords)));
+}
+__device__ __forceinline__ void fc_word_store(const WinState& w, uint32_t f, uint32_t i, uint32_t word) {
+  if (kFireSub == 1) *fc_at(w, i, f, 0) = (uint16_t)word;
+  else *reinterpret_cast<uint32_t*>(fc_at(w, i / kFcWords, f, 2 * (i % kFcWords))) = word;
+}
+__device__ __forceinline__ uint32_t fc_append(const WinState& w, uint32_t* fc, uint32_t slot, uint32_t loc) {
+  if (kFireSub == 1) return atomicAdd(&fc[slot], 1u);
+  const uint32_t j = loc >> w.fshift, sh = 16 * (j & 1);
+  const uint32_t old = atomicAdd(&fc[slot * kFcWords + (j >> 1)], 1u << sh);
+  return j * kSubNodes + ((old >> sh) & 0xFFFFu);
+}
+
 }
 }
diff --git a/gossip_simulator_amd/csrc/gs_win_expand.hip b/gossip_simulator_amd/csrc/gs_win_expand.hip
--- a/gossip_simulator_amd/csrc/gs_win_expand.hip
+++ b/gossip_simulator_amd/csrc/gs_win_expand.hip
@@ -194,7 +194,7 @@
     Tn = w.ctl->Tn;
     Ls = w.lstride;
   }
-  const uint32_t units = Ls * w.nfine;
+  const uint32_t units = Ls * win_nsub(w);
   constexpr uint32_t per_round = B * NPT;
   if (tid < kMaxWindow * 2) (&sm.acc[0][0])[tid] = 0;
   static_assert(B % 256 == 0, "thread b < 256 owns coarse bin b");
@@ -230,10 +230,10 @@
       if (g0 < Tn) {
         const uint32_t u = unit_of_wave(w, g0, g < Tn ? g : Tn - 1, Tn, units);
         if (g < Tn) {
-        const uint32_t f = u / Ls, k = u - f * Ls;
+        const uint32_t fj = u / Ls, k = u - fj * Ls, f = fj >> kFireSubLog, j = fj & (kFireSub - 1);
         const uint32_t s = (t0 + k) % w.R;
         const uint32_t i = (uint32_t)(g - w.unit_off[u]);
-        vv[q] = (f << kFineLog) + w.flist[((size_t)s * w.nfine + f) * kFineNodes + i];
+        vv[q] = (f << kFineLog) + flist_at(w, s, f)[j * kSubNodes + i];
         kk[q] = k;
         }
       }
diff --git a/gossip_simulator_amd/csrc/gs_win_resolve.hip b/gossip_simulator_amd/csrc/gs_win_resolve.hip
--- a/gossip_simulator_amd/csrc/gs_win_resolve.hip
+++ b/gossip_simulator_amd/csrc/gs_win_resolve.hip
@@ -31,7 +31,7 @@
       uint32_t ncrash[kBitWords];
     };
   };
-  uint32_t fc[kWinMaxRing];
+  uint32_t fc[kWinMaxRing * kFcWords];
   uint32_t st[kMaxWindow][4];
   uint32_t dead[kMaxWindow];
   uint32_t blist[kResolveMaxBuckets];
@@ -82,8 +82,7 @@
     const uint32_t off = fire_offset(w.delay_low, w.delay_span,
                                      philox(u, t, 0, c3delay, w.key.k0, w.key.k1).x);
     const uint32_t s = (t + off) % w.R;
-    const uint32_t at = atomicAdd(&sm.fc[s], 1u);
-    w.flist[((size_t)s * w.nfine + f) * kFineNodes + at] = (uint16_t)loc;
+    flist_at(w, s, f)[fc_append(w, sm.fc, s, loc)] = (uint16_t)loc;
     ++cs;
   }
   if (pos <= kk) {
@@ -155,7 +154,7 @@
   L = win_live(w, t0, L);
   if (!L) return;
   static_assert(kBitWords == kResolveBlock, "one bit word per thread");
-  static_assert(kWinMaxRing <= kResolveBlock, "one ring slot per thread");
+  static_assert(kWinMaxRing * kFcWords <= kResolveBlock, "one staged fire-list word per thread");
   if (tid < kMaxWindow * 4) (&sm.st[0][0])[tid] = 0;
   if (tid == 0) { sm.nb = 0; sm.cls = 0; }
   if (tid < 2 * kStampPhases) (&sm.stamp[0][0])[tid] = 0;
@@ -203,7 +202,7 @@
     p_recv0 = rwg[wc];
     p_crash0 = cwg[wc];
     p_roll0 = w.rollw[wc];
-    p_fcv = w.fcount[(size_t)(tid < w.R ? tid : 0u) * w.nfine + f];
+    p_fcv = fc_word(w, f, tid < w.R * kFcWords ? tid : 0u);
     ld(w.fmsg + mb, M, 0, pm);
   };
   if (nb > 0) prefetch(fB, MB, mbB);
@@ -217,7 +216,7 @@
     const uint32_t c3delay = (c3order & 0xFFFFFFu) | (K_DELAY << 24);
     const bool in = wi < w.W * 2;
     const uint32_t recv0 = p_in ? p_recv0 : 0u, crash0 = p_in ? p_crash0 : 0u, roll0 = p_in ? p_roll0 : 0u;
-    const uint32_t fcv = tid < w.R ? p_fcv : 0u;
+    const uint32_t fcv = p_fcv;
     if (i + 1 < nb) next_bucket(i + 1);
     if (roll0) w.rollw[wi] = 0u;
     const uint32_t rollw = roll0 & ~crash0;
@@ -225,7 +224,7 @@
     for (uint32_t k = 0; k < kBitTicks; ++k)
       if (k < L) sm.b1[k][tid] = 0;
     sm.cr0[tid] = make_uint2(crash0, rollw);
-    if (tid < w.R) sm.fc[tid] = fcv;
+    if (tid < w.R * kFcWords) sm.fc[tid] = fcv;
     if (tid < kMaxWindow) sm.dead[tid] = 0;
     if (tid == 0) { sm.ndup = 0; sm.ninf = 0; sm.err = M >= (1u << 28) ? 3 : 0; sm.cls = M >= 1024 ? 1 : 0; }
     __syncthreads();
@@ -330,8 +329,7 @@
         const uint32_t off = fire_offset(w.delay_low, w.delay_span,
                                          philox(knode0 + loc, t, 0, c3delay, w.key.k0, w.key.k1).x);
         const uint32_t slot = (t + off) % w.R;
-        const uint32_t pos = atomicAdd(&sm.fc[slot], 1u);
-        w.flist[((size_t)slot * w.nfine + f) * kFineNodes + pos] = (uint16_t)loc;
+        flist_at(w, slot, f)[fc_append(w, sm.fc, slot, loc)] = (uint16_t)loc;
       };
       uint32_t* inf = &sm.cnt[0];
       {
@@ -374,7 +372,7 @@
       if (rw != recv0) rwg[wi] = rw;
       if (cw != crash0) cwg[wi] = cw;
     }
-    if (tid < w.R) w.fcount[(size_t)tid * w.nfine + f] = sm.fc[tid];
+    if (tid < w.R * kFcWords) fc_word_store(w, f, tid, sm.fc[tid]);
     stamp(w, sm, 9);
     if (w.dbg && tid == 0) sm.stamp[sm.cls][0] += 1;
     if (w.tstat) flush_counts(w, sm, acc_ni, L, (uint32_t)(((uint64_t)w.base + node0) >> w.tlog));
@@ -398,7 +396,7 @@
     uint2 cr0[kBitWords];
     uint32_t inf[kInfCap];
   };
-  uint32_t fc[kWinMaxRing];
+  uint32_t fc[kWinMaxRing * kFcWords];
   uint32_t st[kMaxWindow][4];
   uint32_t dead[kMaxWindow];
   uint32_t blist[kResolveMaxBuckets];
@@ -463,7 +461,7 @@
     p_recv0 = rwg[wc];
     p_crash0 = cwg[wc];
     p_roll0 = w.rollw[wc];
-    p_fcv = w.fcount[(size_t)(tid < w.R ? tid : 0u) * w.nfine + f];
+    p_fcv = fc_word(w, f, tid < w.R * kFcWords ? tid : 0u);
     ld(w.fmsg + sm.bstart[j], sm.bcnt[j], 0, pm);
   };
   if (nb > 0) prefetch(0);
@@ -483,7 +481,7 @@
     for (uint32_t k = 0; k < kBitTicks; ++k)
       if (k < L) sm.b1[k][tid] = 0;
     sm.cr0[tid] = make_uint2(crash0, rollw);
-    if (tid < w.R) sm.fc[tid] = p_fcv;
+    if (tid < w.R * kFcWords) sm.fc[tid] = p_fcv;
     if (tid < kMaxWindow) sm.dead[tid] = 0;
     if (tid == 0) { sm.ndup = 0; sm.ninf = 0; sm.err = M >= (1u << 28) ? 3 : 0; sm.cls = M >= 1024 ? 1 : 0; }
     __syncthreads();
@@ -599,8 +597,7 @@
           const uint32_t off = fire_offset(w.delay_low, w.delay_span,
                                            philox(knode0 + loc, t, 0, c3delay, w.key.k0, w.key.k1).x);
           const uint32_t slot = (t + off) % w.R;
-          const uint32_t pos = atomicAdd(&sm.fc[slot], 1u);
-          w.flist[((size_t)slot * w.nfine + f) * kFineNodes + pos] = (uint16_t)loc;
+          flist_at(w, slot, f)[fc_append(w, sm.fc, slot, loc)] = (uint16_t)loc;
         }
         if (left <= kInfCap) break;
         __syncthreads();
@@ -608,7 +605,7 @@
     }
     __syncthreads();
     stamp(w, sm, 8);
-    if (!large && tid < w.R) w.fcount[(size_t)tid * w.nfine + f] = sm.fc[tid];
+    if (!large && tid < w.R * kFcWords) fc_word_store(w, f, tid, sm.fc[tid]);
     stamp(w, sm, 9);
     if (w.dbg && tid == 0) sm.stamp[sm.cls][0] += 1;
     if (w.tstat) flush_counts(w, sm, acc_ni, L, (uint32_t)(((uint64_t)w.base + node0) >> w.tlog));
@@ -648,7 +645,7 @@
       for (uint32_t q = tid; q < kFineNodes / 4; q += kResolveBlock) c4[q] = make_uint4(0, 0, 0, 0);
       sm.recv[tid] = recv0;
       sm.crash[tid] = crash0;
-      if (tid < w.R) sm.fc[tid] = w.fcount[(size_t)tid * w.nfine + f];
+      if (tid < w.R * kFcWords) sm.fc[tid] = fc_word(w, f, tid);
       if (tid == 0) sm.err = 0;
       __syncthreads();
       for (uint32_t k = 0; k < L; ++k) resolve_tick(w, sm, f, gm, 0, M, k, t0 + k);
@@ -657,7 +654,7 @@
         if (rw != recv0) rwg[wi] = rw;
         if (cw != crash0) cwg[wi] = cw;
       }
-      if (tid < w.R) w.fcount[(size_t)tid * w.nfine + f] = sm.fc[tid];
+      if (tid < w.R * kFcWords) fc_word_store(w, f, tid, sm.fc[tid]);
       if (tid == 0 && sm.err == 1) atomicOr(w.err, kErrArrivals);
       if (w.tstat) flush_counts(w, sm, acc_ni, L, (uint32_t)(((uint64_t)w.base + node0) >> w.tlog));
       else __syncthreads();
@@ -687,8 +684,8 @@
   {
     const bool consume = !ROLLED && w.ctl;
     const uint32_t s0 = t0 % w.R;
-    for (uint32_t s = lane; s < w.R; s += 64)
-      fcw[s] = consume && (s + w.R - s0) % w.R < L ? 0u : w.fcount[(size_t)s * w.nfine + f];
+    for (uint32_t i = lane; i < w.R * kFcWords; i += 64)
+      fcw[i] = consume && (i / kFcWords + w.R - s0) % w.R < L ? 0u : fc_word(w, f, i);
     uint32_t knode0, c3order;
     node_key(w.tlog, w.tmask, w.key, (uint64_t)w.base + (f << kFineLog), K_ORDER, knode0, c3order);
     const uint32_t c3delay = (c3order & 0xFFFFFFu) | (K_DELAY << 24);
@@ -779,15 +776,14 @@
         const uint32_t off = fire_offset(w.delay_low, w.delay_span,
                                          philox(u, tinf, 0, c3delay, w.key.k0, w.key.k1).x);
         const uint32_t slot = (tinf + off) % w.R;
-        const uint32_t pos = atomicAdd(&fcw[slot], 1u);
-        w.flist[((size_t)slot * w.nfine + f) * kFineNodes + pos] = (uint16_t)loc;
+        flist_at(w, slot, f)[fc_append(w, fcw, slot, loc)] = (uint16_t)loc;
       }
     }
     wave_lds_sync();
     if (__ballot(any_inf)) {
-      for (uint32_t s = lane; s < w.R; s += 64) w.fcount[(size_t)s * w.nfine + f] = fcw[s];
-    } else if (consume && lane < L) {
-      w.fcount[(size_t)((t0 + lane) % w.R) * w.nfine + f] = 0;
+      for (uint32_t i = lane; i < w.R * kFcWords; i += 64) fc_word_store(w, f, i, fcw[i]);
+    } else if (consume && lane < L * kFireSub) {
+      *fc_at(w, (t0 + lane / kFireSub) % w.R, f, lane % kFireSub) = 0;
     }
     if (w.tstat) {
       wave_lds_sync();
@@ -807,7 +803,9 @@
   constexpr uint32_t kEmax = ROLLED ? 16 : 4;
   __shared__ uint32_t st[kWaves][kMaxWindow][4];
   __shared__ uint32_t sk[kWaves][64 * kEmax];
-  __shared__ uint32_t fcw[kWaves][kWinMaxRing];
+  extern __shared__ uint32_t fcw_all[];
+  uint32_t* const fcw = fcw_all + (threadIdx.x >> 6) * w.R * kFcWords;
+  static_assert(kBitTicks * kFireSub <= 64, "a lane per (window slot, sub-list) to consume");
   const uint32_t tid = threadIdx.x, wv = tid >> 6;
   static_assert(kWaves * kMaxWindow * 4 == kWaves * 64, "one counter per thread");
   static_assert(kRolledCap == 64 * 16, "the rolled bodies cover 1..kRolledCap");
@@ -827,15 +825,15 @@
   if (!L) return;
   (&st[0][0][0])[tid] = 0;
   __syncthreads();
-  if (M > 0 && M <= 64) resolve_small_bucket<1, ROLLED>(w, t0, L, f, gm, M, st, sk[wv], fcw[wv]);
-  else if (M > 64 && M <= 256) resolve_small_bucket<4, ROLLED>(w, t0, L, f, gm, M, st, sk[wv], fcw[wv]);
+  if (M > 0 && M <= 64) resolve_small_bucket<1, ROLLED>(w, t0, L, f, gm, M, st, sk[wv], fcw);
+  else if (M > 64 && M <= 256) resolve_small_bucket<4, ROLLED>(w, t0, L, f, gm, M, st, sk[wv], fcw);
   else if (ROLLED && M > 256 && M <= 512)
-    resolve_small_bucket<ROLLED ? 8 : 1, ROLLED>(w, t0, L, f, gm, M, st, sk[wv], fcw[wv]);
+    resolve_small_bucket<ROLLED ? 8 : 1, ROLLED>(w, t0, L, f, gm, M, st, sk[wv], fcw);
   else if (ROLLED && M > 512 && M <= kRolledCap)
-    resolve_small_bucket<ROLLED ? 16 : 1, ROLLED>(w, t0, L, f, gm, M, st, sk[wv], fcw[wv]);
+    resolve_small_bucket<ROLLED ? 16 : 1, ROLLED>(w, t0, L, f, gm, M, st, sk[wv], fcw);
   if (ROLLED && M && (threadIdx.x & 63) == 0) w.rlcnt[f] = 0;
-  if (!ROLLED && w.ctl && !(M > 0 && M <= 256) && f < w.nfine && (threadIdx.x & 63) < L)
-    w.fcount[(size_t)((t0 + (threadIdx.x & 63)) % w.R) * w.nfine + f] = 0;
+  if (!ROLLED && w.ctl && !(M > 0 && M <= 256) && f < w.nfine && (threadIdx.x & 63) < L * kFireSub)
+    *fc_at(w, (t0 + (threadIdx.x & 63) / kFireSub) % w.R, f, (threadIdx.x & 63) % kFireSub) = 0;
   __syncthreads();
   if (tid < L * 3) {
     const uint32_t k = tid / 3, fld = tid - k * 3;
@@ -863,6 +861,8 @@
 
 }
 
+static uint32_t small_fcw_bytes(uint32_t block, uint32_t R) { return block / 64 * R * kFcWords * 4; }
+
 static bool resolve_occ3() {
   static const bool on = [] { const char* e = getenv("GS_RESOLVE_OCC3"); return !e || atoi(e) != 0; }();
   return on;
@@ -881,7 +881,7 @@
   uint32_t G = std::min<uint32_t>(w.nfine, resolve_grid_env() ? resolve_grid_env() : per_cu * cus);
   G = std::max<uint32_t>(G, (w.nfine + kResolveMaxBuckets - 1) / kResolveMaxBuckets);
   const uint32_t gs = (w.nfine + kSmallBlock / 64 - 1) / (kSmallBlock / 64);
-  hipLaunchKernelGGL(k_resolve_small<false>, dim3(gs), dim3(kSmallBlock), 0, s, w, t0, L);
+  hipLaunchKernelGGL(k_resolve_small<false>, dim3(gs), dim3(kSmallBlock), small_fcw_bytes(kSmallBlock, w.R), s, w, t0, L);
   static_assert(kSmallMax == 64 * 4, "the two bodies cover 1..kSmallMax");
   if (occ3) {
     hipLaunchKernelGGL(k_resolve, dim3(G), dim3(kResolveBlock), 0, s, w, t0, L);
@@ -890,7 +890,7 @@
     hipLaunchKernelGGL(k_resolve2, dim3(G), dim3(kResolveBlock), 0, s, w, t0, L);
   }
   hipLaunchKernelGGL(k_resolve_small<true>, dim3((w.nfine + kRolledBlock / 64 - 1) / (kRolledBlock / 64)),
-                     dim3(kRolledBlock), 0, s, w, t0, L);
+                     dim3(kRolledBlock), small_fcw_bytes(kRolledBlock, w.R), s, w, t0, L);
   return hipGetLastError();
 }
 
@@ -901,7 +901,8 @@
                                   resolve_grid_env() ? resolve_grid_env() : ((occ3 ? 3 : 2) * cus + g.M - 1) / g.M);
   G = std::max<uint32_t>(G, (g.nfine_max + kResolveMaxBuckets - 1) / kResolveMaxBuckets);
   const uint32_t gs = (g.nfine_max + kSmallBlock / 64 - 1) / (kSmallBlock / 64);
-  hipLaunchKernelGGL(k_resolve_small_m<false>, dim3(gs, g.M), dim3(kSmallBlock), 0, s, g.wr, L);
+  hipLaunchKernelGGL(k_resolve_small_m<false>, dim3(gs, g.M), dim3(kSmallBlock), small_fcw_bytes(kSmallBlock, g.ring_max),
+                     s, g.wr, L);
   if (occ3) {
     hipLaunchKernelGGL(k_resolve_m, dim3(G, g.M), dim3(kResolveBlock), 0, s, g.wr, L);
     hipLaunchKernelGGL(k_resolve_large_m, dim3(std::min<uint32_t>(g.nfine_max, (cus + g.M - 1) / g.M), g.M),
@@ -910,7 +911,7 @@
     hipLaunchKernelGGL(k_resolve2_m, dim3(G, g.M), dim3(kResolveBlock), 0, s, g.wr, L);
   }
   hipLaunchKernelGGL(k_resolve_small_m<true>, dim3((g.nfine_max + kRolledBlock / 64 - 1) / (kRolledBlock / 64), g.M),
-                     dim3(kRolledBlock), 0, s, g.wr, L);
+                     dim3(kRolledBlock), small_fcw_bytes(kRolledBlock, g.ring_max), s, g.wr, L);
   return hipGetLastError();
 }
 
diff --git a/gossip_simulator_amd/csrc/gs_win_shard.hip b/gossip_simulator_amd/csrc/gs_win_shard.hip
--- a/gossip_simulator_amd/csrc/gs_win_shard.hip
+++ b/gossip_simulator_amd/csrc/gs_win_shard.hip
@@ -16,9 +16,10 @@
 }
 
 __global__ void k_consume_sh(const WinState w, uint32_t t0, uint32_t L) {
-  for (uint32_t i = blockIdx.x * blockDim.x + threadIdx.x; i < L * w.nfine; i += gridDim.x * blockDim.x) {
-    const uint32_t k = i / w.nfine, f = i - k * w.nfine;
-    w.fcount[(size_t)((t0 + k) % w.R) * w.nfine + f] = 0;
+  const uint32_t nsub = win_nsub(w);
+  for (uint32_t i = blockIdx.x * blockDim.x + threadIdx.x; i < L * nsub; i += gridDim.x * blockDim.x) {
+    const uint32_t k = i / nsub, f = i - k * nsub;
+    w.fcount[(size_t)((t0 + k) % w.R) * nsub + f] = 0;
   }
 }
 
@@ -251,7 +252,7 @@
 }
 
 hipError_t win_consume_sh(const WinState& w, uint32_t t0, uint32_t L, hipStream_t s) {
-  const uint32_t blocks = std::min<uint32_t>((L * w.nfine + 255) / 256, 2048);
+  const uint32_t blocks = std::min<uint32_t>((L * win_nsub(w) + 255) / 256, 2048);
   hipLaunchKernelGGL(k_consume_sh, dim3(blocks ? blocks : 1), dim3(256), 0, s, w, t0, L);
   return hipGetLastError();
 }
diff --git a/gossip_simulator_amd/csrc/gs_win_units.hip b/gossip_simulator_amd/csrc/gs_win_units.hip
--- a/gossip_simulator_amd/csrc/gs_win_units.hip
+++ b/gossip_simulator_amd/csrc/gs_win_units.hip
@@ -13,7 +13,7 @@
     if (!L) return;
     Ls = w.lstride;
   }
-  const uint32_t units = Ls * w.nfine;
+  const uint32_t nsub = win_nsub(w), units = Ls * nsub;
   const uint32_t tid = blockIdx.x * blockDim.x + threadIdx.x, nth = gridDim.x * blockDim.x;
   __shared__ uint32_t s_tile[256 * (kMaxWindow + 1)];
   uint32_t acc[kMaxWindow];
@@ -26,13 +26,13 @@
   uint32_t slot[kMaxWindow];
 #pragma unroll
   for (uint32_t k = 0; k < kMaxWindow; ++k) slot[k] = k < L ? (t0 + k) % w.R : 0u;
-  for (uint32_t f0 = blockIdx.x * 256; f0 < w.nfine; f0 += gridDim.x * 256) {
+  for (uint32_t f0 = blockIdx.x * 256; f0 < nsub; f0 += gridDim.x * 256) {
     const uint32_t f = f0 + threadIdx.x;
     if (threadIdx.x < kMaxWindow) s_ts[threadIdx.x] = 0;
     uint32_t cv[kMaxWindow];
 #pragma unroll
     for (uint32_t k = 0; k < kMaxWindow; ++k)
-      cv[k] = k < L && k < Ls && f < w.nfine ? w.fcount[(size_t)slot[k] * w.nfine + f] : 0u;
+      cv[k] = k < L && k < Ls && f < nsub ? w.fcount[(size_t)slot[k] * nsub + f] : 0u;
 #pragma unroll
     for (uint32_t k = 0; k < kMaxWindow; ++k) {
       if (k < Ls) {
@@ -50,7 +50,7 @@
     }
     __syncthreads();
     if (threadIdx.x < Ls) w.tsum[(size_t)(f0 >> 8) * kMaxWindow + threadIdx.x] = s_ts[threadIdx.x];
-    const uint32_t nb = min(256u, w.nfine - f0), base = f0 * Ls;
+    const uint32_t nb = min(256u, nsub - f0), base = f0 * Ls;
     for (uint32_t i = threadIdx.x; i < nb * Ls; i += 256) {
       const uint32_t b = i / Ls, k = i - b * Ls;
       w.usize[base + i] = s_tile[b * (kMaxWindow + 1) + k];
@@ -105,7 +105,7 @@
   for (uint32_t j = 0; j < 4; ++j)
 #pragma unroll
     for (uint32_t k = 0; k < kMaxWindow; ++k)
-      ts[j][k] = Lw && b * 4 + j < w.ncoarse ? w.tsum[(size_t)(b * 4 + j) * kMaxWindow + k] : 0ull;
+      ts[j][k] = Lw && b * 4 + j < win_ntile(w) ? w.tsum[(size_t)(b * 4 + j) * kMaxWindow + k] : 0ull;
   __syncthreads();
   if (b == 0) {
     s_go = Lw != 0;
@@ -134,7 +134,8 @@
   __syncthreads();
   if (!s_go) return;
   {
-    const uint32_t L = s_L, nt = w.ncoarse;
+    static_assert(256 * kFireSub <= 1024, "k_cut scans four tiles per thread");
+    const uint32_t L = s_L, nt = win_ntile(w);
     unsigned long long v[4], sum = 0;
 #pragma unroll
     for (uint32_t j = 0; j < 4; ++j) {
@@ -196,7 +197,8 @@
 
 __device__ __forceinline__ void unitscan_body(const WinState& w) {
   __shared__ unsigned long long s_x[4];
-  if (blockIdx.x >= w.ncoarse) return;
+  const uint32_t nsub = win_nsub(w);
+  if (blockIdx.x >= win_ntile(w)) return;
   uint32_t t0;
   const uint32_t L = win_live(w, t0, 0);
   if (!L) return;
@@ -205,12 +207,12 @@
   unsigned long long sz[kMaxWindow], sum = 0;
 #pragma unroll
   for (uint32_t k = 0; k < kMaxWindow; ++k)
-    sz[k] = k < L && f < w.nfine ? w.usize[(size_t)f * Ls + k] : 0ull;
+    sz[k] = k < L && f < nsub ? w.usize[(size_t)f * Ls + k] : 0ull;
 #pragma unroll
   for (uint32_t k = 0; k < kMaxWindow; ++k) sum += sz[k];
   unsigned long long tot;
   unsigned long long a = w.toff[tile] + block_exscan_u64<4>(sum, s_x, &tot);
-  if (f >= w.nfine) return;
+  if (f >= nsub) return;
 #pragma unroll
   for (uint32_t k = 0; k < kMaxWindow; ++k) {
     if (k >= Ls) break;
@@ -220,7 +222,7 @@
     for (unsigned long long q = (a + 63) >> 6; (q << 6) < b; ++q) w.gmap[q] = u;
     a = b;
   }
-  if (f == w.nfine - 1) w.unit_off[(size_t)w.nfine * Ls] = a;
+  if (f == nsub - 1) w.unit_off[(size_t)nsub * Ls] = a;
 }
 __global__ __launch_bounds__(256) void k_unitscan(const WinState w) { unitscan_body(w); }
 __global__ __launch_bounds__(256) void k_unitscan_m(const WinState* __restrict__ ws) { unitscan_body(ws[blockIdx.y]); }
@@ -231,7 +233,7 @@
     if (!win_live(w, t0, 0)) return;
     L = w.lstride;
   }
-  const uint32_t units = L * w.nfine;
+  const uint32_t units = L * win_nsub(w);
   for (uint32_t u = blockIdx.x * blockDim.x + threadIdx.x; u < units; u += gridDim.x * blockDim.x) {
     const unsigned long long a = w.unit_off[u], b = w.unit_off[u + 1];
     for (unsigned long long q = (a + 63) >> 6; (q << 6) < b; ++q) w.gmap[q] = u;
@@ -306,15 +308,17 @@
   node_key(w.tlog, w.tmask, w.key, (uint64_t)w.base + local, K_DELAY, kn, c3);
   const uint32_t off = fire_offset(w.delay_low, w.delay_span, philox(kn, t, 0, c3, w.key.k0, w.key.k1).x);
   const uint32_t s = (t + off) % w.R;
-  const uint32_t f = local >> kFineLog;
-  const uint32_t pos = atomicAdd(&w.fcount[(size_t)s * w.nfine + f], 1u);
-  w.flist[((size_t)s * w.nfine + f) * kFineNodes + pos] = (uint16_t)(local & (kFineNodes - 1));
+  const uint32_t f = local >> kFineLog, loc = local & (kFineNodes - 1), j = loc >> w.fshift;
+  uint16_t* const len = fc_at(w, s, f, j);
+  const uint32_t sh = 8 * (uint32_t)((uintptr_t)len & 2);
+  const uint32_t pos = (atomicAdd(reinterpret_cast<uint32_t*>((uintptr_t)len & ~(uintptr_t)3), 1u << sh) >> sh) & 0xFFFFu;
+  flist_at(w, s, f)[j * kSubNodes + pos] = (uint16_t)loc;
 }
 
 }
 
 hipError_t win_units_g(const WinGroup& g, uint32_t L, hipStream_t s) {
-  const uint32_t blocks = std::max<uint32_t>(std::min<uint32_t>((g.nfine_max + 255) / 256, 4096), 1);
+  const uint32_t blocks = std::max<uint32_t>(std::min<uint32_t>((g.nfine_max * kFireSub + 255) / 256, 4096), 1);
   hipLaunchKernelGGL(k_units_m, dim3(blocks, g.M), dim3(256), 0, s, g.ws, 0u, L);
   return hipGetLastError();
 }
@@ -325,13 +329,14 @@
 }
 
 hipError_t win_unitscan_g(const WinGroup& g, hipStream_t s) {
-  hipLaunchKernelGGL(k_unitscan_m, dim3(std::max<uint32_t>(g.ncoarse_max, 1), g.M), dim3(256), 0, s, g.ws);
+  hipLaunchKernelGGL(k_unitscan_m, dim3(std::max<uint32_t>((g.nfine_max * kFireSub + 255) / 256, 1), g.M), dim3(256), 0, s,
+                     g.ws);
   return hipGetLastError();
 }
 
 hipError_t win_units(const WinState& w, uint32_t t0, uint32_t L, hipStream_t s) {
   (void)L;
-  const uint32_t blocks = std::max<uint32_t>(std::min<uint32_t>((w.nfine + 255) / 256, 4096), 1);
+  const uint32_t blocks = std::max<uint32_t>(std::min<uint32_t>(win_ntile(w), 4096), 1);
   hipLaunchKernelGGL(k_units, dim3(blocks), dim3(256), 0, s, w, t0, L);
   return hipGetLastError();
 }
@@ -342,7 +347,7 @@
 }
 
 hipError_t win_unitscan(const WinState& w, hipStream_t s) {
-  hipLaunchKernelGGL(k_unitscan, dim3(w.ncoarse), dim3(256), 0, s, w);
+  hipLaunchKernelGGL(k_unitscan, dim3(win_ntile(w)), dim3(256), 0, s, w);
   return hipGetLastError();
 }
 
@@ -353,11 +358,11 @@
 
 hipError_t win_scan_units(const WinState& w, uint32_t L, void* tmp, size_t& tmp_bytes, hipStream_t s) {
   return hipcub::DeviceScan::ExclusiveSum(tmp, tmp_bytes, (const unsigned long long*)w.usize,
-                                          w.unit_off, (int)(L * w.nfine + 1), s);
+                                          w.unit_off, (int)(L * win_nsub(w) + 1), s);
 }
 
 hipError_t win_groupmap(const WinState& w, uint32_t L, hipStream_t s) {
-  const uint32_t units = L * w.nfine;
+  const uint32_t units = L * win_nsub(w);
   const uint32_t blocks = std::min<uint32_t>((units + 255) / 256, 4096);
   hipLaunchKernelGGL(k_groupmap, dim3(blocks ? blocks : 1), dim3(256), 0, s, w, L);
   return hipGetLastError();
diff --git a/gossip_simulator_amd/csrc/gs_windows.cpp b/gossip_simulator_amd/csrc/gs_windows.cpp
--- a/gossip_simulator_amd/csrc/gs_windows.cpp
+++ b/gossip_simulator_amd/csrc/gs_windows.cpp
@@ -70,7 +70,7 @@
       CK(c, win_scan_units(w, Lu, c->wn.tmp.p, need, c->stream));
       CK(c, hipMemcpyAsync(c->wn.h_misc, w.tfires, kMaxWindow * 8, hipMemcpyDeviceToHost, c->stream));
       if (trial_plan)
-        CK(c, hipMemcpy2DAsync(c->wn.h_misc + kMaxWindow, 8, w.unit_off, (size_t)256 * Lu * 8, 8, w.ncoarse,
+        CK(c, hipMemcpy2DAsync(c->wn.h_misc + kMaxWindow, 8, w.unit_off, (size_t)256 * kFireSub * Lu * 8, 8, w.ncoarse,
                                hipMemcpyDeviceToHost, c->stream));
       CK(c, hipStreamSynchronize(c->stream));
       return GS_OK;
@@ -147,8 +147,9 @@
     }
     const uint32_t s0 = t % w.R;
     const uint32_t first = std::min(L, w.R - s0);
-    CK(c, hipMemsetAsync(w.fcount + (size_t)s0 * w.nfine, 0, (size_t)first * w.nfine * 4, c->stream));
-    if (first < L) CK(c, hipMemsetAsync(w.fcount, 0, (size_t)(L - first) * w.nfine * 4, c->stream));
+    const size_t nsub = (size_t)w.nfine * kFireSub;
+    CK(c, hipMemsetAsync(w.fcount + (size_t)s0 * nsub, 0, (size_t)first * nsub * sizeof *w.fcount, c->stream));
+    if (first < L) CK(c, hipMemsetAsync(w.fcount, 0, (size_t)(L - first) * nsub * sizeof *w.fcount, c->stream));
     if (e) CK(c, hipEventRecord(e[3], c->stream));
     if (T) CK(c, win_resolve(w, t, L, c->stream));
     if (T) CK(c, win_stats_reduce(w, t, L, c->stream));
```

New measurement: 86.21 billion. Within noise of the previous version (-0.6%).
